# RenYurui/Global-Flow-Local-Attention

Measured on AMD Instinct MI355X. Metric: images/sec (fwd+bwd) PoseGenerator 256x176 attn_layer=2,3 -- feature-warping hot path, higher is better.
Workload: dtype f32 (FC products: 2-term f16 splits exact to 2^-24 on f16 MFMA, f32 accumulate)

## Files before the change

global_flow_local_attention_amd/_lib.py:

```python
import ctypes
import os
import subprocess

import torch

_PKG = os.path.dirname(os.path.abspath(__file__))
LIB_PATH = os.environ.get("GFLA_HIP_LIBRARY") or os.path.join(_PKG, "libgfla_hip.so")
_lib = None

_i64, _int, _ptr = ctypes.c_int64, ctypes.c_int, ctypes.c_void_p

_SIGNATURES = {
    "gfla_block_extractor_fwd": [_ptr] * 3 + [_i64] * 6 + [_int, _ptr],
    "gfla_block_extractor_bwd": [_ptr] * 5 + [_i64] * 6 + [_int, _ptr],
    "gfla_block_extractor_unfold_fwd": [_ptr] * 3 + [_i64] * 6 + [_int, _int, _ptr],
    "gfla_block_extractor_unfold_bwd": [_ptr] * 5 + [_i64] * 6 + [_int, _int, _ptr],
    "gfla_local_attn_reshape_fwd": [_ptr] * 2 + [_i64] * 3 + [_int, _ptr],
    "gfla_local_attn_reshape_bwd": [_ptr] * 2 + [_i64] * 3 + [_int, _ptr],
    "gfla_resample2d_fwd": [_ptr] * 3 + [_i64] * 6 + [_int, _int, _ptr],
    "gfla_resample2d_bwd": [_ptr] * 5 + [_i64] * 6 + [_int, _int, _int, _ptr],
    "gfla_local_attn_aggregate_fwd": [_ptr] * 5 + [_i64] * 6 + [_int, _int, _ptr],
    "gfla_local_attn_aggregate_bwd": [_ptr] * 7 + [_i64] * 6 + [_int, _int, _ptr],
    "gfla_local_attn_source_bwd": [_ptr] * 7 + [_i64] * 6 + [_int, _int, _ptr],
    "gfla_flow_warp_fwd": [_ptr] * 3 + [_i64] * 6 + [ctypes.c_double] * 4 + [_ptr],
    "gfla_flow_warp_bwd": [_ptr] * 5 + [_i64] * 6 + [ctypes.c_double] * 4 + [_ptr],
}
_SINGLE = {
    "gfla_max_cosine_fwd_f32": [_ptr] * 5 + [_i64] * 4 + [ctypes.c_double, _ptr],
    "gfla_max_cosine_fwd_f16": [_ptr] * 5 + [_i64] * 4 + [ctypes.c_double, _ptr],
    "gfla_max_cosine_fwd_bf16": [_ptr] * 5 + [_i64] * 4 + [ctypes.c_double, _ptr],
    "gfla_max_cosine_workspace_bytes": [_i64] * 3,
    "gfla_fc_tail_fwd_f32": [_ptr, _i64, _i64] + [_ptr] * 5 + [_i64] * 3 + [_int, ctypes.c_double, _ptr],
    "gfla_fc_tail_fwd_f64": [_ptr, _i64, _i64] + [_ptr] * 5 + [_i64] * 3 + [_int, ctypes.c_double, _ptr],
    "gfla_fc_tail_bwd_f32": [_ptr, _i64, _i64] + [_ptr] * 8 + [_i64] * 3 + [_int, ctypes.c_double, _ptr],
    "gfla_fc_tail_bwd_f64": [_ptr, _i64, _i64] + [_ptr] * 8 + [_i64] * 3 + [_int, ctypes.c_double, _ptr],
    "gfla_replicate_pad_bwd_f32": [_ptr] * 2 + [_i64] * 3 + [_int] * 4 + [_ptr],
    "gfla_replicate_pad_bwd_f64": [_ptr] * 2 + [_i64] * 3 + [_int] * 4 + [_ptr],
    "gfla_correctness_map_fwd_f32": [_ptr] * 5 + [_i64] * 3 + [ctypes.c_double] * 2 + [_ptr],
    "gfla_correctness_map_bwd_f32": [_ptr] * 9 + [_i64] * 3 + [ctypes.c_double] * 2 + [_ptr],
    "gfla_correctness_map_fwd_f16": [_ptr] * 5 + [_i64] * 3 + [ctypes.c_double] * 2 + [_ptr],
    "gfla_correctness_map_bwd_f16": [_ptr] * 9 + [_i64] * 3 + [ctypes.c_double] * 2 + [_ptr],
    "gfla_correctness_map_fwd_bf16": [_ptr] * 5 + [_i64] * 3 + [ctypes.c_double] * 2 + [_ptr],
    "gfla_correctness_map_bwd_bf16": [_ptr] * 9 + [_i64] * 3 + [ctypes.c_double] * 2 + [_ptr],
    "gfla_fc_supported": [_i64] * 3 + [_int, _int],
    "gfla_fc_workspace_bytes": [_i64] * 4 + [_int] * 3,
    "gfla_fc_forward_f32": [_ptr] * 9 + [_i64] * 4 + [_int, ctypes.c_double, _int, _ptr],
    "gfla_fc_backward_f32": [_ptr] * 12 + [_i64] * 4 + [_int, ctypes.c_double, _int, _int, _ptr],
    "gfla_fc_geometry": [_i64, _i64, _int, _int, _ptr],
    "gfla_fc_conv_fwd_f32": [_ptr, _ptr, _int, _ptr, _ptr] + [_i64] * 4 + [_int, _int, _ptr],
    "gfla_fc_conv_bwd_f32": [_ptr, _int, _ptr, _ptr, _ptr, _ptr] + [_i64] * 4 + [_int, _int, _ptr],
    "gfla_fc_tr_probe": [_ptr, _int, _ptr, _ptr, _ptr],
    "gfla_fc_wino_debug_buffer": [_ptr],
    "gfla_fc_kernel_f32": [_int, _ptr, _ptr] + [_i64] * 4 + [_int, _int, _ptr],
    "gfla_scatter_workspace_bytes": [_i64] * 3 + [_int],
    "gfla_aggregate_fwd_workspace_bytes": [_i64] * 3 + [_int],
    "gfla_aggregate_fwd_geometry": [_i64] * 6 + [_int, _ptr],
    "gfla_aggregate_bwd_supported": [_i64, _i64, _int],
    "gfla_big_plane_geometry": [_int] + [_i64] * 6 + [_int, _int, _ptr],
    "gfla_xcd_swizzle": [_i64, _i64],
    "gfla_local_attn_aggregate_fwd_ws_f32": [_ptr] * 6 + [_i64] * 6 + [_int, _int, _ptr],
    "gfla_local_attn_aggregate_fwd_ws_bf16": [_ptr] * 6 + [_i64] * 6 + [_int, _int, _ptr],
    "gfla_local_attn_aggregate_fwd_ws_f16": [_ptr] * 6 + [_i64] * 6 + [_int, _int, _ptr],
    "gfla_local_attn_aggregate_bwd_ws_f32": [_ptr] * 8 + [_i64] * 6 + [_int, _int, _ptr],
    "gfla_resample2d_bwd_ws_f32": [_ptr] * 6 + [_i64] * 6 + [_int, _int, _int, _ptr],
    "gfla_convert_multi": [_ptr, _ptr, _i64] * 4 + [_int, _ptr],
    "gfla_mask_blend_fwd_f32": [_ptr] * 6 + [_i64] * 3 + [_ptr],
    "gfla_mask_blend_fwd_bf16": [_ptr] * 6 + [_i64] * 3 + [_ptr],
    "gfla_mask_blend_bwd_f32": [_ptr] * 11 + [_i64] * 3 + [_ptr],
    "gfla_mask_blend_bwd_bf16": [_ptr] * 11 + [_i64] * 3 + [_ptr],
    "gfla_mask_blend_fwd_f16": [_ptr] * 6 + [_i64] * 3 + [_ptr],
    "gfla_mask_blend_bwd_f16": [_ptr] * 11 + [_i64] * 3 + [_ptr],
    "gfla_fc_forward_f16": [_ptr] * 9 + [_i64] * 4 + [_int, ctypes.c_double, _ptr],
    "gfla_gemm_f64_workspace_bytes": [_i64] * 3 + [_int],
    "gfla_gemm_f64": [_ptr] * 6 + [_i64] * 3 + [_int, _int, _ptr, _ptr],
    "gfla_affine_reg_workspace_bytes": [_i64] * 3 + [_int],
    "gfla_affine_reg_fwd_f32": [_ptr] * 3 + [_i64] * 3 + [_int, _ptr],
    "gfla_affine_reg_fwd_f64": [_ptr] * 3 + [_i64] * 3 + [_int, _ptr],
    "gfla_affine_reg_fwd_f16": [_ptr] * 3 + [_i64] * 3 + [_int, _ptr],
    "gfla_affine_reg_fwd_bf16": [_ptr] * 3 + [_i64] * 3 + [_int, _ptr],
    "gfla_affine_reg_bwd_f32": [_ptr] * 4 + [_i64] * 3 + [_int, _ptr],
    "gfla_affine_reg_bwd_f64": [_ptr] * 4 + [_i64] * 3 + [_int, _ptr],
    "gfla_affine_reg_bwd_f16": [_ptr] * 4 + [_i64] * 3 + [_int, _ptr],
    "gfla_affine_reg_bwd_bf16": [_ptr] * 4 + [_i64] * 3 + [_int, _ptr],
    "gfla_gram_l1_workspace_bytes": [_i64] * 3,
    "gfla_gram_l1_fwd_f32": [_ptr] * 5 + [_i64] * 3 + [_ptr],
    "gfla_gram_l1_fwd_f16": [_ptr] * 5 + [_i64] * 3 + [_ptr],
    "gfla_gram_l1_fwd_bf16": [_ptr] * 5 + [_i64] * 3 + [_ptr],
    "gfla_gram_l1_bwd_f32": [_ptr] * 4 + [_i64] * 3 + [_int, _ptr],
    "gfla_gram_l1_bwd_f16": [_ptr] * 4 + [_i64] * 3 + [_int, _ptr],
    "gfla_gram_l1_bwd_bf16": [_ptr] * 4 + [_i64] * 3 + [_int, _ptr],
}
_FWD_ONLY_BF16 = set()


def exported_symbols():
    names = ["gfla_abi_version", "gfla_status_string", "gfla_set_tuning", "gfla_path_count", "gfla_unfold_supported"]
    for base in _SIGNATURES:
        for sfx in ("f32", "f64", "bf16", "f16"):
            if sfx == "bf16" and base in _FWD_ONLY_BF16:
                continue
            names.append("%s_%s" % (base, sfx))
    return names + list(_SINGLE)


def build(force=False):
    cmd = ["make", "-C", os.path.join(_PKG, "csrc"), "-j8"]
    if force:
        cmd.append("-B")
    subprocess.check_call(cmd, stdout=subprocess.DEVNULL)
    return LIB_PATH


def lib():
    global _lib
    if _lib is None:
        if not os.path.exists(LIB_PATH):
            raise RuntimeError(
                "libgfla_hip.so is not built (%s). Run `python -c 'import __graft_entry__ as g; g.build()'` "
                "or `make -C global_flow_local_attention_amd/csrc`. There is no fallback path." % LIB_PATH)
        handle = ctypes.CDLL(LIB_PATH)
        handle.gfla_status_string.restype = ctypes.c_char_p
        handle.gfla_status_string.argtypes = [_int]
        handle.gfla_set_tuning.argtypes = [_int, _int]
        handle.gfla_path_count.argtypes = [_int]
        handle.gfla_path_count.restype = _i64
        handle.gfla_unfold_supported.argtypes = [_i64, _i64, _int, _int]
        for base, args in _SIGNATURES.items():
            for sfx in ("f32", "f64", "bf16", "f16"):
                if sfx == "bf16" and base in _FWD_ONLY_BF16:
                    continue
                fn = getattr(handle, "%s_%s" % (base, sfx))
                fn.argtypes = args
                fn.restype = _int
        for name, args in _SINGLE.items():
            fn = getattr(handle, name)
            fn.argtypes = args
            fn.restype = _i64 if (name.endswith("_bytes") or name == "gfla_xcd_swizzle") else _int
        _lib = handle
    return _lib


_SUFFIX = {torch.float32: "f32", torch.float64: "f64", torch.bfloat16: "bf16", torch.float16: "f16"}
HALF_TYPES = (torch.bfloat16, torch.float16)


def suffix(t, what, allow_bf16=True):
    try:
        sfx = _SUFFIX[t.dtype]
    except KeyError:
        raise TypeError("%s: unsupported dtype %s (float32, float64, bfloat16, float16)" % (what, t.dtype))
    if sfx == "bf16" and not allow_bf16:
        raise TypeError("%s: bfloat16 is forward-only in this library (use float32 for training)" % what)
    return sfx


def reduction_like(t):
    return torch.zeros(t.shape, dtype=torch.float32 if t.dtype in HALF_TYPES else t.dtype, device=t.device)


def scatter_workspace(ref_tensor, B, H, W, entries):
    n = lib().gfla_scatter_workspace_bytes(int(B), int(H), int(W), int(entries))
    return torch.empty(max(int(n), 16), dtype=torch.uint8, device=ref_tensor.device)


def aggregate_fwd(source, flow, logits, out, attn, k, apply_softmax):
    b, c, hs, ws = source.shape
    h, w = flow.shape[2], flow.shape[3]
    sfx = suffix(source, "local_attn_aggregate")
    tail = (b, c, hs, ws, h, w, int(k), 1 if apply_softmax else 0)
    if sfx in ("f32", "bf16", "f16"):
        n = lib().gfla_aggregate_fwd_workspace_bytes(int(b), int(h), int(w), int(k))
        scratch = torch.empty(max(int(n), 16), dtype=torch.uint8, device=source.device)
        call("gfla_local_attn_aggregate_fwd_ws_" + sfx, source, ptr(source), ptr(flow), ptr(logits), ptr(out), ptr(attn),
             ptr(scratch), *tail)
    else:
        call("gfla_local_attn_aggregate_fwd_" + sfx, source, ptr(source), ptr(flow), ptr(logits), ptr(out), ptr(attn), *tail)


def require_gpu(*tensors):
    for t in tensors:
        if t is not None and not t.is_cuda:
            raise NotImplementedError("GFLA ops run on the GPU only (got a %s tensor); there is no CPU path"
                                      % t.device.type)


def ptr(t):
    return None if t is None else ctypes.c_void_p(t.data_ptr())


class Unsupported(RuntimeError):
    """GFLA_ERR_UNSUPPORTED (-3): the arguments are valid but outside what this entry point's kernels take (nothing was
    launched).  Callers that have another way to the same result catch exactly this."""


def call(name, ref_tensor, *args):
    fn = getattr(lib(), name)
    with torch.cuda.device(ref_tensor.device):
        stream = ctypes.c_void_p(torch.cuda.current_stream(ref_tensor.device).cuda_stream)
        status = fn(*args, stream)
    if status != 0:
        err = Unsupported if status == -3 else RuntimeError
        raise err("%s failed: %s (status %d)" % (name, lib().gfla_status_string(status).decode(), status))


_CONVERT_FLAG = {(torch.bfloat16, torch.float32): 0, (torch.float32, torch.bfloat16): 1,
                 (torch.float16, torch.float32): 2, (torch.float32, torch.float16): 3}


def convert_many(tensors, dtype):
    out = list(tensors)
    todo = [i for i, t in enumerate(out) if t is not None and t.dtype != dtype]
    pair_ok = all(out[i].is_cuda and (out[i].dtype, dtype) in _CONVERT_FLAG for i in todo)
    if not todo or not pair_ok or len({out[i].dtype for i in todo}) != 1:
        return [None if t is None else t.to(dtype) for t in out]
    flag = _CONVERT_FLAG[(out[todo[0]].dtype, dtype)]
    for at in range(0, len(todo), 4):
        grp = todo[at:at + 4]
        srcs = [out[i].contiguous() for i in grp]
        dsts = [torch.empty(t.shape, dtype=dtype, device=t.device) for t in srcs]
        args = []
        for j in range(4):
            args += [ptr(srcs[j]), ptr(dsts[j]), srcs[j].numel()] if j < len(grp) else [None, None, 0]
        call("gfla_convert_multi", srcs[0], *args, flag)
        for i, d in zip(grp, dsts):
            out[i] = d
    return out


def unfold_supported(Hs, Ws, k, elem_size):
    return bool(lib().gfla_unfold_supported(int(Hs), int(Ws), int(k), int(elem_size)))


def set_tuning(key, value):
    return lib().gfla_set_tuning(int(key), int(value))


ABI_VERSION = 8
PATH_BE_BWD_LDS, PATH_BE_BWD_GLOBAL, PATH_FC_FWD_MODE0, PATH_FC_BWD_MODE0, PATH_BE_FWD_PIX = 0, 1, 2, 7, 12
PATH_BE_FWD_GPIX, PATH_BE_BWD_TILE, PATH_RS_FWD_BIG, PATH_RS_BWD1_TILE, PATH_RS_BWD2_BIG = 13, 14, 15, 16, 17
PATH_FC_FWD_MODE5, PATH_FC_BWD_MODE5 = 18, 19
PATH_GEMM_F64 = 20
PATH_FC_PACK_F16, PATH_COUNT = 21, 22


def fc_path(mode, backward=False):
    if int(mode) == 5:
        return PATH_FC_BWD_MODE5 if backward else PATH_FC_FWD_MODE5
    return (PATH_FC_BWD_MODE0 if backward else PATH_FC_FWD_MODE0) + int(mode)


def path_count(path):
    return int(lib().gfla_path_count(int(path)))
```

global_flow_local_attention_amd/csrc/fc_block.hip:

```cpp
#include "fc_gemm.h"

namespace gfla {

static int64_t align256(int64_t v) { return (v + 255) & ~(int64_t)255; }

enum { kAmaxSrc = 0, kAmaxTgt = 1, kAmaxW = 2, kAmaxZs = 3, kAmaxZt = 4, kAmaxSlots = 8 };

enum FcConv {
  kConvDirect,
  kConvDirect16,
  kConvWino32,
  kConvWino16,
};
enum FcWgrad {
  kWgradDirect32,
  kWgradDirect16,
  kWgradWino32,
  kWgradWino16,
};
static bool fc_wgrad_wino(FcWgrad w) { return w == kWgradWino32 || w == kWgradWino16; }

struct FcPlan {
  int split;
  bool scaled;
  FcConv fwd, dgrad;
  bool pack_wf, pack_wd;
  int pack_split;
  bool pack_uf, pack_ud;
  bool dgrads_together;
  FcWgrad wgrad;
  FcWgrad wgrad_both;
  bool wgrads_together;
  bool wgrad_x32;
  bool own_scatter;
};

static FcPlan fc_plan(int64_t B, int C, int H, int W, int k, int mode) {
  (void)C;
  FcPlan P;
  P.split = fc_base_mode(mode);
  P.scaled = P.split != 0 || mode == 5;
  P.fwd = mode == 4 ? kConvWino32 : mode == 5 ? (k == 5 ? kConvDirect16 : kConvWino16) : kConvDirect;
  P.dgrad = mode == 4 ? kConvWino32 : mode == 5 ? kConvDirect16 : kConvDirect;
  P.pack_wf = P.fwd == kConvDirect || P.fwd == kConvDirect16;
  P.pack_wd = P.dgrad == kConvDirect || P.dgrad == kConvDirect16;
  P.pack_split = P.dgrad == kConvDirect16 ? 2 : P.split;
  P.pack_uf = P.fwd == kConvWino32 || P.fwd == kConvWino16;
  P.pack_ud = P.dgrad == kConvWino32;
  P.dgrads_together = fc_is_wino(mode);
  P.wgrad_x32 = mode == 1 && k == 5;
  P.wgrad = fc_is_wino(mode) || P.wgrad_x32 ? (mode == 5 && k == 5 ? kWgradWino16 : kWgradWino32)
                                            : (P.split ? kWgradDirect16 : kWgradDirect32);
  P.wgrad_both = P.wgrad_x32 ? kWgradWino16 : P.wgrad;
  P.wgrads_together = tuning(21) != 2;
  const FcHalf hs = fc_half(H, W, k, true);
  P.own_scatter = tuning(46) != 1 && fc_scatter_own_rows(B, hs.Ho, hs.Wo) >= 1;
  return P;
}

struct FcLayout {
  FcPlan plan;
  FcHalf hs, ht;
  int nch_c, cpad, nt_d, KK, dw1_tiles;
  int64_t amax, xs, xt, gs, hid, wd_t, wd_s, gt, wf_t, wf_s, wu_ft, wu_fs, wu_dt, wu_ds, fwd_total;
  int64_t dzs, dzt, dw_s, dw_t, zero_bytes, zs_pk, zt_pk, dxs, dxt, b0p, dw1p, red, red_tmp, dwp, dwp2, x32, x32b, bwd_total;
};

static FcLayout fc_layout(int64_t B, int C, int H, int W, int k, int mode) {
  const bool wino = fc_is_wino(mode);
  FcLayout L;
  L.plan = fc_plan(B, C, H, W, k, mode);
  const FcPlan &P = L.plan;
  L.hs = fc_half(H, W, k, true);
  L.ht = fc_half(H, W, k, false);
  L.nch_c = (int)ceil_div(C, kFcChunk);
  L.cpad = L.nch_c * kFcChunk;
  L.nt_d = (int)ceil_div(C, kFcTN);
  L.KK = k * k;
  const int nch_h = kFcHidden / kFcChunk;
  int64_t o = 0;
  auto take = [&](int64_t bytes) {
    const int64_t at = o;
    o += align256(bytes);
    return at;
  };
  L.amax = take(kAmaxSlots * 4);
  L.xs = take(fc_packed_bytes(B, L.nch_c, L.hs.Sx, P.split));
  L.xt = take(fc_packed_bytes(B, L.nch_c, L.ht.Sx, P.split));
  L.gs = take(B * L.hs.Mg * kFcHidden * 4);
  L.hid = take(B * (int64_t)H * W * kFcHidden * 4);
  L.wd_t = take(P.pack_wd ? fc_wpack_bytes(L.nt_d, nch_h, k, P.pack_split) : 0);
  L.wd_s = take(P.pack_wd ? fc_wpack_bytes(L.nt_d, nch_h, k, P.pack_split) : 0);
  L.gt = take(B * L.ht.Mg * kFcHidden * 4);
  L.wf_t = take(P.pack_wd ? fc_wpack_bytes(1, L.nch_c, k, P.pack_split) : 0);
  L.wf_s = take(P.pack_wd ? fc_wpack_bytes(1, L.nch_c, k, P.pack_split) : 0);
  L.wu_ft = take(wino ? fc_wino_wpack_bytes(C, kFcHidden) : 0);
  L.wu_fs = take(wino ? fc_wino_wpack_bytes(C, kFcHidden) : 0);
  L.wu_dt = take(wino ? fc_wino_wpack_bytes(kFcHidden, C) : 0);
  L.wu_ds = take(wino ? fc_wino_wpack_bytes(kFcHidden, C) : 0);
  L.fwd_total = o;

  o = 0;
  L.dzs = take(B * L.hs.Sz * kFcHidden * 4);
  L.dzt = take(B * L.ht.Sz * kFcHidden * 4);
  L.dw_s = take((int64_t)L.KK * L.cpad * kFcHidden * 4);
  L.dw_t = take((int64_t)L.KK * L.cpad * kFcHidden * 4);
  L.zero_bytes = o;
  L.zs_pk = take(P.split ? fc_packed_bytes(B, nch_h, L.hs.Sz, P.split) : 0);
  L.zt_pk = take(P.split ? fc_packed_bytes(B, nch_h, L.ht.Sz, P.split) : 0);
  L.dxs = take(B * L.hs.Mdg * (int64_t)C * 4);
  L.dxt = take(B * L.ht.Mdg * (int64_t)C * 4);
  const int64_t tiles = ceil_div((int64_t)H * W, 64);
  L.b0p = take(B * tiles * kFcHidden * 4);
  int t = 1;
  while (B * t < 2 * kNumCU && t * 128 < H * W) t *= 2;
  L.dw1_tiles = t;
  L.dw1p = take(B * t * (32 * kFcHidden + 32) * 4);
  L.red = take((32 * kFcHidden + 32 + kFcHidden) * 4);
  L.red_tmp = take((int64_t)kFcRedTmpFloats * 4);
  const int64_t sp_s = fc_wgrad_splits(B, L.hs.M, L.cpad), sp_t = fc_wgrad_splits(B, L.ht.M, L.cpad);
  int64_t dwp = P.split == 0 ? (sp_s > sp_t ? sp_s : sp_t) * L.KK * L.cpad * kFcHidden * 4 : 0;
  if (fc_wgrad_wino(P.wgrad)) {
    const int64_t ws_s = fc_wino_wgrad_splits(B, L.hs.Ho, L.hs.Wo, L.cpad, k), ws_t = fc_wino_wgrad_splits(B, L.ht.Ho, L.ht.Wo, L.cpad, k);
    const int64_t w = (ws_s > ws_t ? ws_s : ws_t) * 36 * L.cpad * kFcHidden * 4;
    if (w > dwp) dwp = w;
  }
  L.dwp = take(dwp);
  L.dwp2 = take(dwp);
  const int64_t x32_s = fc_packed_bytes(B, L.nch_c, L.hs.Sx, 0), x32_t = fc_packed_bytes(B, L.nch_c, L.ht.Sx, 0);
  L.x32 = take(P.wgrad_x32 ? (x32_s > x32_t ? x32_s : x32_t) : 0);
  L.x32b = take(P.wgrad_x32 ? x32_t : 0);
  L.bwd_total = o;
  return L;
}

static int fc_args_ok(int64_t B, int64_t C, int64_t H, int64_t W, int k, int mode) {
  if (B < 0 || C <= 0 || H <= 0 || W <= 0 || k < 1) return GFLA_ERR_BAD_SHAPE;
  if (!fc_mode_ok(mode) || (k != 3 && k != 5)) return GFLA_ERR_UNSUPPORTED;
  if (B > 65535 || C > 4096 || H > 2048 || W > 2048) return GFLA_ERR_UNSUPPORTED;
  const FcHalf hs = fc_half((int)H, (int)W, k, true), ht = fc_half((int)H, (int)W, k, false);
  const int direct = mode == 5 ? 2 : mode;
  if (mode == 4) {
    if (!fc_wino_fits(hs.Mv, hs.Wo, hs.Wp, k) || !fc_wino_fits(hs.Md, hs.Wp, hs.Wp, k) ||
        !fc_wino_fits(ht.Mv, ht.Wo, ht.Wp, k) || !fc_wino_fits(ht.Md, ht.Wp, ht.Wp, k))
      return GFLA_ERR_UNSUPPORTED;
  } else if (mode == 5) {
    if (!fc_wino16_fits(hs.Mv, hs.Wo, hs.Wp, k) || !fc_wino16_fits(hs.Md, hs.Wp, hs.Wp, k) ||
        !fc_wino16_fits(ht.Mv, ht.Wo, ht.Wp, k) || !fc_wino16_fits(ht.Md, ht.Wp, ht.Wp, k))
      return GFLA_ERR_UNSUPPORTED;
  }
  if (mode != 4 && (!fc_conv_fits(hs.Wo, hs.Wp, k, direct) || !fc_conv_fits(hs.Wp, hs.Wp, k, direct) ||
                    !fc_conv_fits(ht.Wo, ht.Wp, k, direct) || !fc_conv_fits(ht.Wp, ht.Wp, k, direct)))
    return GFLA_ERR_UNSUPPORTED;
  if ((int64_t)64 * (W + 1) * 4 > 64 * 1024) return GFLA_ERR_UNSUPPORTED;
  return GFLA_OK;
}

#define GFLA_TRY(expr)           \
  do {                           \
    const int rc_ = (expr);      \
    if (rc_ != GFLA_OK) return rc_; \
  } while (0)

static int fc_pack_weight_sets(const FcLayout &L, const float *w0, unsigned char *ws, int C, int k, hipStream_t stream) {
  const FcPlan &P = L.plan;
  const uint32_t *a_w = reinterpret_cast<const uint32_t *>(ws + L.amax) + kAmaxW;
  if (P.pack_wf || P.pack_wd)
    GFLA_TRY(fc_pack_weights(w0, P.pack_split ? a_w : nullptr, P.pack_wf ? ws + L.wf_t : nullptr, P.pack_wf ? ws + L.wf_s : nullptr,
                             P.pack_wd ? ws + L.wd_t : nullptr, P.pack_wd ? ws + L.wd_s : nullptr, C, k, P.pack_split, stream));
  float *u_ft = reinterpret_cast<float *>(ws + L.wu_ft), *u_fs = reinterpret_cast<float *>(ws + L.wu_fs);
  if (P.fwd == kConvWino16) return fc_wino16_pack_weights(w0, a_w, u_ft, u_fs, C, k, stream);
  if (P.pack_uf || P.pack_ud)
    return fc_wino_pack_weights(w0, P.pack_uf ? u_ft : nullptr, P.pack_uf ? u_fs : nullptr,
                                P.pack_ud ? reinterpret_cast<float *>(ws + L.wu_dt) : nullptr,
                                P.pack_ud ? reinterpret_cast<float *>(ws + L.wu_ds) : nullptr, C, k, stream);
  return GFLA_OK;
}

static int fc_wino_jobs(const WnConvJob *jobs, int njobs, const uint32_t *const *amax, const uint32_t *amax_w, bool w16, int64_t B,
                        int nch, int k, hipStream_t stream) {
  if (!w16) return fc_wino_conv_jobs(jobs, njobs, B, nch, k, stream);
  Wn16ConvJob j16[2];
  for (int j = 0; j < njobs && j < 2; ++j)
    j16[j] = Wn16ConvJob{jobs[j].X, reinterpret_cast<const uint32_t *>(jobs[j].U), amax[j], jobs[j].out, jobs[j].out_bs, jobs[j].ldo,
                         jobs[j].n_valid, jobs[j].M, jobs[j].Wv, jobs[j].Wp, jobs[j].S};
  return fc_wino16_conv_jobs(j16, njobs, B, nch, k, amax_w, stream);
}

static int fc_fwd_convs(const FcLayout &L, const unsigned char *ws, float *out_s, float *out_t, int64_t B, int k,
                        hipStream_t stream) {
  const FcPlan &P = L.plan;
  const uint32_t *amax = reinterpret_cast<const uint32_t *>(ws + L.amax);
  WnConvJob jobs[2];
  const uint32_t *am[2];
  int n = 0;
  for (int h = 0; h < 2; ++h) {
    const bool src = h == 0;
    float *out = src ? out_s : out_t;
    if (!out) continue;
    const FcHalf &g = src ? L.hs : L.ht;
    const PackedDesc X = fc_desc_packed(ws + (src ? L.xs : L.xt), B, L.nch_c, g.Sx, P.split);
    const uint32_t *a_x = amax + (src ? kAmaxSrc : kAmaxTgt);
    const unsigned char *wf = ws + (src ? L.wf_s : L.wf_t);
    if (P.fwd == kConvDirect16) {
      GFLA_TRY(fc_conv_f32src(X, wf, fc_wpack_bytes(1, L.nch_c, k, 2) / 2, out, g.Mg * kFcHidden, kFcHidden, kFcHidden, B, L.nch_c,
                              g.Mv, g.Wo, g.Wp, k, a_x, amax + kAmaxW, stream));
    } else if (P.fwd == kConvDirect) {
      GFLA_TRY(fc_conv(X, wf, fc_wpack_bytes(1, L.nch_c, k, P.split) / fc_nsplit(P.split), out, g.Mg * kFcHidden, kFcHidden,
                       kFcHidden, B, L.nch_c, g.Mv, g.Wo, g.Wp, k, P.split, P.split ? a_x : nullptr,
                       P.split ? amax + kAmaxW : nullptr, stream));
    } else {
      jobs[n] = WnConvJob{X, reinterpret_cast<const float *>(ws + (src ? L.wu_fs : L.wu_ft)), out, g.Mg * kFcHidden, kFcHidden,
                          kFcHidden, g.Mv, g.Wo, g.Wp, g.Sx};
      am[n++] = a_x;
    }
  }
  return n ? fc_wino_jobs(jobs, n, am, amax + kAmaxW, P.fwd == kConvWino16, B, L.nch_c, k, stream) : GFLA_OK;
}

static int fc_dgrad_convs(const FcLayout &L, const unsigned char *ws, unsigned char *sc, bool want_s, bool want_t, int64_t B, int C,
                          int k, hipStream_t stream) {
  const FcPlan &P = L.plan;
  const uint32_t *amax = reinterpret_cast<const uint32_t *>(ws + L.amax);
  const int nch_h = kFcHidden / kFcChunk;
  WnConvJob jobs[2];
  int n = 0;
  for (int h = 0; h < 2; ++h) {
    const bool src = h == 0;
    if (!(src ? want_s : want_t)) continue;
    const FcHalf &g = src ? L.hs : L.ht;
    const float *dz = reinterpret_cast<const float *>(sc + (src ? L.dzs : L.dzt));
    float *dx = reinterpret_cast<float *>(sc + (src ? L.dxs : L.dxt));
    const uint32_t *a_z = amax + (src ? kAmaxZs : kAmaxZt);
    const unsigned char *wd = ws + (src ? L.wd_s : L.wd_t);
    if (P.dgrad == kConvDirect16) {
      GFLA_TRY(fc_conv_f32src(fc_desc_nhwc(dz, g.Sz, kFcHidden), wd, fc_wpack_bytes(L.nt_d, nch_h, k, 2) / 2, dx, g.Mdg * (int64_t)C,
                              C, C, B, nch_h, g.Md, g.Wp, g.Wp, k, a_z, amax + kAmaxW, stream));
    } else if (P.dgrad == kConvDirect) {
      const PackedDesc Z = P.split ? fc_desc_packed(sc + (src ? L.zs_pk : L.zt_pk), B, nch_h, g.Sz, P.split)
                                   : fc_desc_nhwc(dz, g.Sz, kFcHidden);
      GFLA_TRY(fc_conv(Z, wd, fc_wpack_bytes(L.nt_d, nch_h, k, P.split) / fc_nsplit(P.split), dx, g.Mdg * (int64_t)C, C, C, B,
                       nch_h, g.Md, g.Wp, g.Wp, k, P.split, P.split ? a_z : nullptr, P.split ? amax + kAmaxW : nullptr, stream));
    } else {
      jobs[n++] = WnConvJob{fc_desc_nhwc(dz, g.Sz, kFcHidden), reinterpret_cast<const float *>(ws + (src ? L.wu_ds : L.wu_dt)), dx,
                            g.Mdg * (int64_t)C, C, C, g.Md, g.Wp, g.Wp, g.Sz};
    }
  }
  return n ? fc_wino_conv_jobs(jobs, n, B, nch_h, k, stream) : GFLA_OK;
}

static PackedDesc fc_wgrad_x(const FcLayout &L, const unsigned char *ws, const unsigned char *sc, bool src, int64_t B) {
  const FcHalf &g = src ? L.hs : L.ht;
  if (L.plan.wgrad_x32) return fc_desc_packed(sc + (src ? L.x32 : L.x32b), B, L.nch_c, g.Sx, 0);
  return fc_desc_packed(ws + (src ? L.xs : L.xt), B, L.nch_c, g.Sx, L.plan.split);
}

static int fc_wgrad_half(const FcLayout &L, bool src, const unsigned char *ws, unsigned char *sc, int64_t B, int k,
                         hipStream_t stream) {
  const FcPlan &P = L.plan;
  const FcHalf &g = src ? L.hs : L.ht;
  const uint32_t *amax = reinterpret_cast<const uint32_t *>(ws + L.amax);
  const PackedDesc X = fc_wgrad_x(L, ws, sc, src, B);
  const float *dz = reinterpret_cast<const float *>(sc + (src ? L.dzs : L.dzt));
  float *part = reinterpret_cast<float *>(sc + (src ? L.dwp : L.dwp2));
  switch (P.wgrad) {
    case kWgradWino16: {
      const WwJob job{X, dz, part, g.Sz * kFcHidden, g.lead, g.Sx, g.Ho, g.Wo, g.Wp};
      const uint32_t *const ax[1] = {amax + (src ? kAmaxSrc : kAmaxTgt)}, *const az[1] = {amax + (src ? kAmaxZs : kAmaxZt)};
      return fc_wino16_wgrad_jobs(&job, 1, L.cpad, B, k, ax, az, stream);
    }
    case kWgradWino32:
      return fc_wino_wgrad(X, dz, g.Sz * kFcHidden, g.lead, part, L.cpad, B, g.Ho, g.Wo, g.Wp, g.Sx, k, stream);
    case kWgradDirect32:
      return fc_wgrad_f32(X, fc_desc_nhwc(dz, g.Sz, kFcHidden), g.lead, part, L.cpad, B, g.M, g.Wp, k, stream);
    default:
      return fc_wgrad(X, fc_desc_packed(sc + (src ? L.zs_pk : L.zt_pk), B, kFcHidden / kFcChunk, g.Sz, P.split), g.lead,
                      reinterpret_cast<float *>(sc + (src ? L.dw_s : L.dw_t)), L.cpad, B, g.M, g.Wp, k, P.split, stream);
  }
}

static int fc_wgrad_both(const FcLayout &L, const unsigned char *ws, unsigned char *sc, int64_t B, int k, hipStream_t stream) {
  const uint32_t *amax = reinterpret_cast<const uint32_t *>(ws + L.amax);
  const WwJob jobs[2] = {
      {fc_wgrad_x(L, ws, sc, true, B), reinterpret_cast<const float *>(sc + L.dzs), reinterpret_cast<float *>(sc + L.dwp),
       L.hs.Sz * kFcHidden, L.hs.lead, L.hs.Sx, L.hs.Ho, L.hs.Wo, L.hs.Wp},
      {fc_wgrad_x(L, ws, sc, false, B), reinterpret_cast<const float *>(sc + L.dzt), reinterpret_cast<float *>(sc + L.dwp2),
       L.ht.Sz * kFcHidden, L.ht.lead, L.ht.Sx, L.ht.Ho, L.ht.Wo, L.ht.Wp}};
  if (L.plan.wgrad_both == kWgradWino16) {
    const uint32_t *const ax[2] = {amax + kAmaxSrc, amax + kAmaxTgt}, *const az[2] = {amax + kAmaxZs, amax + kAmaxZt};
    return fc_wino16_wgrad_jobs(jobs, 2, L.cpad, B, k, ax, az, stream);
  }
  return fc_wino_wgrad_jobs(jobs, 2, L.cpad, B, k, stream);
}

static int fc_forward(const float *source, const float *target, const float *flow, const float *w0, const float *b0,
                      const float *w1, const float *b1, void *ws_, float *logits, int64_t B, int C, int H, int W,
                      int k, float slope, int mode_, hipStream_t stream, const uint16_t *source16 = nullptr,
                      const uint16_t *target16 = nullptr) {
  const bool f16 = source16 != nullptr;
  if (f16 ? !target16 : (!source || !target)) return GFLA_ERR_NULL_POINTER;
  if (!flow || !w0 || !w1 || !ws_ || !logits) return GFLA_ERR_NULL_POINTER;
  if (f16 && mode_ != 1) return GFLA_ERR_UNSUPPORTED;
  GFLA_TRY(fc_args_ok(B, C, H, W, k, mode_));
  if (B == 0) return GFLA_OK;
  note_path(mode_ == 5 ? GFLA_PATH_FC_FWD_MODE5 : GFLA_PATH_FC_FWD_MODE0 + mode_);
  const FcLayout L = fc_layout(B, C, H, W, k, mode_);
  const FcPlan &P = L.plan;
  unsigned char *ws = static_cast<unsigned char *>(ws_);
  uint32_t *amax = reinterpret_cast<uint32_t *>(ws + L.amax);
  if (P.scaled) {
    if (hipMemsetAsync(amax, 0, kAmaxSlots * 4, stream) != hipSuccess) return GFLA_ERR_LAUNCH;
    if (f16)
      GFLA_TRY(fc_maxabs(w0, (int64_t)kFcHidden * 2 * C * k * k, amax + kAmaxW, stream));
    else
      GFLA_TRY(fc_maxabs_multi(source, B * (int64_t)C * H * W, amax + kAmaxSrc, target, B * (int64_t)C * H * W, amax + kAmaxTgt,
                               w0, (int64_t)kFcHidden * 2 * C * k * k, amax + kAmaxW, stream));
  }
  GFLA_TRY(fc_pack_weight_sets(L, w0, ws, C, k, stream));
  if (f16)
    GFLA_TRY(fc_pack_act2_f16(source16, ws + L.xs, L.hs, target16, ws + L.xt, L.ht, B, C, H, W, stream));
  else
    GFLA_TRY(fc_pack_act2(source, P.split ? amax + kAmaxSrc : nullptr, ws + L.xs, L.hs, target, P.split ? amax + kAmaxTgt : nullptr,
                          ws + L.xt, L.ht, B, C, H, W, P.split, stream));
  float *gs = reinterpret_cast<float *>(ws + L.gs), *gt = reinterpret_cast<float *>(ws + L.gt);
  GFLA_TRY(fc_fwd_convs(L, ws, gs, gt, B, k, stream));
  return fc_sample_tail_fwd(gs, gt, flow, b0, w1, b1, reinterpret_cast<float *>(ws + L.hid), logits, B, H, W, k,
                            L.hs.Mg * kFcHidden, L.ht.Mg * kFcHidden, L.hs.Wo, L.ht.Wo, slope, stream);
}

struct FcHalfCall {
  int acc_x = 0;
  bool z_ready = false;
  bool dgrad_done = false;
  bool fold_later = false;
  bool wgrad_later = false;
  bool reduce = true;
};

static int fc_half_backward(const FcLayout &L, bool source, unsigned char *ws, unsigned char *sc, float *g_x, float *g_w0,
                            int64_t B, int C, int H, int W, int k, const FcHalfCall &call, hipStream_t stream) {
  const FcPlan &P = L.plan;
  const FcHalf &g = source ? L.hs : L.ht;
  uint32_t *amax = reinterpret_cast<uint32_t *>(ws + L.amax);
  uint32_t *a_z = amax + (source ? kAmaxZs : kAmaxZt);
  float *dz = reinterpret_cast<float *>(sc + (source ? L.dzs : L.dzt));
  if (P.split && !call.z_ready) {
    GFLA_TRY(fc_maxabs(dz, B * g.Sz * kFcHidden, a_z, stream));
    GFLA_TRY(fc_pack_z(dz, a_z, sc + (source ? L.zs_pk : L.zt_pk), B, g.Sz, kFcHidden, P.split, stream));
  }
  if (g_x && !call.dgrad_done) {
    if (P.dgrad == kConvDirect16) GFLA_TRY(fc_maxabs(dz, B * g.Sz * kFcHidden, a_z, stream));
    GFLA_TRY(fc_dgrad_convs(L, ws, sc, source, !source, B, C, k, stream));
    if (!call.fold_later)
      GFLA_TRY(fc_fold(reinterpret_cast<const float *>(sc + (source ? L.dxs : L.dxt)), g_x, B, C, H, W, g, g.Mdg * (int64_t)C,
                       call.acc_x, stream));
  }
  if (!g_w0) return GFLA_OK;
  if (P.wgrad_x32)
    GFLA_TRY(fc_unpack_act(ws + (source ? L.xs : L.xt), amax + (source ? kAmaxSrc : kAmaxTgt),
                           reinterpret_cast<float *>(sc + (source ? L.x32 : L.x32b)), B, L.nch_c, g.Sx, stream));
  if (!call.wgrad_later) {
    if (P.wgrad == kWgradWino16) GFLA_TRY(fc_maxabs(dz, B * g.Sz * kFcHidden, a_z, stream));
    GFLA_TRY(fc_wgrad_half(L, source, ws, sc, B, k, stream));
  }
  if (!call.reduce) return GFLA_OK;
  float *part = reinterpret_cast<float *>(sc + (source ? L.dwp : L.dwp2));
  if (fc_wgrad_wino(P.wgrad))
    return fc_wino_wgrad_reduce(part, fc_wino_wgrad_splits(B, g.Ho, g.Wo, L.cpad, k), g_w0, C, source ? C : 0, L.cpad, k, stream);
  if (P.wgrad == kWgradDirect32)
    return fc_wgrad_reduce(part, fc_wgrad_splits(B, g.M, L.cpad), g_w0, C, source ? C : 0, L.cpad, k, stream);
  return GFLA_OK;
}

static int fc_fold_both(const FcLayout &L, const unsigned char *sc, float *g_source, float *g_target, int acc_s, int64_t B, int C,
                        int H, int W, hipStream_t stream) {
  return fc_fold2(reinterpret_cast<const float *>(sc + L.dxs), g_source, L.hs, L.hs.Mdg * (int64_t)C, acc_s,
                  reinterpret_cast<const float *>(sc + L.dxt), g_target, L.ht, L.ht.Mdg * (int64_t)C, 0, B, C, H, W, stream);
}

static int fc_unpack_wgrad_both(const FcLayout &L, const unsigned char *ws, unsigned char *sc, float *g_w0, int C, int k,
                                hipStream_t stream) {
  const uint32_t *a = reinterpret_cast<const uint32_t *>(ws + L.amax);
  return fc_unpack_wgrad(reinterpret_cast<float *>(sc + L.dw_t), reinterpret_cast<float *>(sc + L.dw_s), a + kAmaxTgt, a + kAmaxSrc,
                         a + kAmaxZt, a + kAmaxZs, g_w0, C, L.cpad, k, stream);
}

static int fc_backward(void *ws_, const float *flow, const float *w1, const float *g_logits, void *scratch_,
                       float *g_source, float *g_target, float *g_flow, float *g_w0, float *g_b0, float *g_w1,
                       float *g_b1, int64_t B, int C, int H, int W, int k, float slope, int mode_, int flags,
                       hipStream_t stream) {
  if (!ws_ || !flow || !w1 || !g_logits || !scratch_) return GFLA_ERR_NULL_POINTER;
  GFLA_TRY(fc_args_ok(B, C, H, W, k, mode_));
  if (B == 0) return GFLA_OK;
  note_path(mode_ == 5 ? GFLA_PATH_FC_BWD_MODE5 : GFLA_PATH_FC_BWD_MODE0 + mode_);
  const FcLayout L = fc_layout(B, C, H, W, k, mode_);
  const FcPlan &P = L.plan;
  unsigned char *ws = static_cast<unsigned char *>(ws_), *sc = static_cast<unsigned char *>(scratch_);
  uint32_t *amax = reinterpret_cast<uint32_t *>(ws + L.amax);
  const float *hid = reinterpret_cast<const float *>(ws + L.hid);
  float *red_tmp = reinterpret_cast<float *>(sc + L.red_tmp);
  const float *gs = reinterpret_cast<const float *>(ws + L.gs);
  const bool need_s = g_source || g_w0, need_t = g_target || g_w0;
  float *dzs = need_s ? reinterpret_cast<float *>(sc + L.dzs) : nullptr;
  float *dzt = need_t ? reinterpret_cast<float *>(sc + L.dzt) : nullptr;
  float *b0p = g_b0 ? reinterpret_cast<float *>(sc + L.b0p) : nullptr;
  const int64_t tiles = ceil_div((int64_t)H * W, 64);
  const bool own = need_s && need_t && P.own_scatter;
  if (hipMemsetAsync(sc + (own ? L.dzt : 0), 0, L.zero_bytes - (own ? L.dzt : 0), stream) != hipSuccess) return GFLA_ERR_LAUNCH;
  if ((P.scaled || own) && hipMemsetAsync(amax + kAmaxZs, 0, 8, stream) != hipSuccess) return GFLA_ERR_LAUNCH;
  GFLA_TRY(fc_sample_tail_bwd(gs, flow, hid, w1, g_logits, own ? nullptr : dzs, dzt, g_flow, b0p, B, H, W, k, L.hs.Mg * kFcHidden,
                              L.hs.Wo, L.hs.Wp, L.ht.Wp, L.hs.Sz * kFcHidden, L.ht.Sz * kFcHidden, L.hs.lead, L.ht.lead, slope,
                              flags & GFLA_FC_ACCUMULATE_FLOW, stream, own ? amax + kAmaxZt : nullptr));
  if (own)
    GFLA_TRY(fc_sample_scatter_own(flow, dzt, dzs, amax + kAmaxZt, amax + kAmaxZs, B, H, W, k, L.hs.Ho, L.hs.Wo, L.hs.Wp, L.ht.Wp,
                                   L.hs.Sz * kFcHidden, L.ht.Sz * kFcHidden, L.hs.lead, L.ht.lead, L.hs.Sz, stream));
  const float *dw1p = nullptr;
  if (g_w1 || g_b1) {
    float *part = reinterpret_cast<float *>(sc + L.dw1p);
    GFLA_TRY(fc_dw1(hid, g_logits, part, B, H * W, L.KK, L.dw1_tiles, slope, stream));
    dw1p = part;
  }
  GFLA_TRY(fc_reduce_bias_w1(b0p, B * tiles, g_b0, dw1p, B * L.dw1_tiles, g_w1, g_b1, L.KK, red_tmp, stream));
  const int acc_s = (flags & GFLA_FC_ACCUMULATE_SOURCE) ? 1 : 0;
  const bool both_x = g_source && g_target;
  const bool dgrads_done = P.dgrads_together && both_x;
  if (dgrads_done) {
    if (P.dgrad == kConvDirect16 && !own)
      GFLA_TRY(fc_maxabs_multi(dzs, B * L.hs.Sz * kFcHidden, amax + kAmaxZs, dzt, B * L.ht.Sz * kFcHidden, amax + kAmaxZt, nullptr,
                               0, nullptr, stream));
    GFLA_TRY(fc_dgrad_convs(L, ws, sc, true, true, B, C, k, stream));
    GFLA_TRY(fc_fold_both(L, sc, g_source, g_target, acc_s, B, C, H, W, stream));
  }
  const bool defer = g_w0 && P.wgrad != kWgradDirect16;
  const bool wgrads_done = defer && fc_wgrad_wino(P.wgrad) && both_x && P.wgrads_together;
  const bool z_both = P.split != 0 && need_s && need_t;
  if (z_both) {
    if (!own)
      GFLA_TRY(fc_maxabs_multi(dzs, B * L.hs.Sz * kFcHidden, amax + kAmaxZs, dzt, B * L.ht.Sz * kFcHidden, amax + kAmaxZt, nullptr,
                               0, nullptr, stream));
    GFLA_TRY(fc_pack_z2(dzs, amax + kAmaxZs, sc + L.zs_pk, L.hs.Sz, dzt, amax + kAmaxZt, sc + L.zt_pk, L.ht.Sz, B, kFcHidden,
                        P.split, stream));
  }
  FcHalfCall call;
  call.z_ready = z_both;
  call.dgrad_done = dgrads_done;
  call.fold_later = both_x;
  call.wgrad_later = wgrads_done;
  call.reduce = !defer;
  if (need_s) {
    call.acc_x = acc_s;
    GFLA_TRY(fc_half_backward(L, true, ws, sc, g_source, g_w0, B, C, H, W, k, call, stream));
  }
  if (need_t) {
    call.acc_x = 0;
    GFLA_TRY(fc_half_backward(L, false, ws, sc, g_target, g_w0, B, C, H, W, k, call, stream));
  }
  if (both_x && !dgrads_done) GFLA_TRY(fc_fold_both(L, sc, g_source, g_target, acc_s, B, C, H, W, stream));
  if (wgrads_done) GFLA_TRY(fc_wgrad_both(L, ws, sc, B, k, stream));
  if (defer) {
    float *part_s = reinterpret_cast<float *>(sc + L.dwp), *part_t = reinterpret_cast<float *>(sc + L.dwp2);
    if (fc_wgrad_wino(P.wgrad))
      GFLA_TRY(fc_wino_wgrad_reduce2(part_s, fc_wino_wgrad_splits(B, L.hs.Ho, L.hs.Wo, L.cpad, k), part_t,
                                     fc_wino_wgrad_splits(B, L.ht.Ho, L.ht.Wo, L.cpad, k), g_w0, C, L.cpad, k, stream));
    else
      GFLA_TRY(fc_wgrad_reduce2(part_s, fc_wgrad_splits(B, L.hs.M, L.cpad), part_t, fc_wgrad_splits(B, L.ht.M, L.cpad), g_w0, C,
                                L.cpad, k, stream));
  }
  if (g_w0 && P.wgrad == kWgradDirect16) GFLA_TRY(fc_unpack_wgrad_both(L, ws, sc, g_w0, C, k, stream));
  return GFLA_OK;
}

}

extern "C" {
using namespace gfla;

int gfla_fc_supported(int64_t C, int64_t H, int64_t W, int kernel_size, int mode) {
  return fc_args_ok(1, C, H, W, kernel_size, mode) == GFLA_OK ? 1 : 0;
}

int64_t gfla_fc_workspace_bytes(int64_t B, int64_t C, int64_t H, int64_t W, int kernel_size, int mode, int which) {
  if (fc_args_ok(B, C, H, W, kernel_size, mode) != GFLA_OK) return -1;
  const FcLayout L = fc_layout(B, (int)C, (int)H, (int)W, kernel_size, mode);
  return which == 0 ? L.fwd_total : L.bwd_total;
}

int gfla_fc_forward_f32(const float *source, const float *target, const float *flow, const float *w0,
                        const float *b0, const float *w1, const float *b1, void *workspace, float *logits, int64_t B,
                        int64_t C, int64_t H, int64_t W, int kernel_size, double slope, int mode,
                        gfla_stream_t stream) {
  return fc_forward(source, target, flow, w0, b0, w1, b1, workspace, logits, B, (int)C, (int)H, (int)W, kernel_size,
                    (float)slope, mode, static_cast<hipStream_t>(stream));
}

int gfla_fc_forward_f16(const uint16_t *source, const uint16_t *target, const float *flow, const float *w0,
                        const float *b0, const float *w1, const float *b1, void *workspace, float *logits, int64_t B,
                        int64_t C, int64_t H, int64_t W, int kernel_size, double slope, gfla_stream_t stream) {
  return fc_forward(nullptr, nullptr, flow, w0, b0, w1, b1, workspace, logits, B, (int)C, (int)H, (int)W, kernel_size,
                    (float)slope, 1, static_cast<hipStream_t>(stream), source, target);
}

int gfla_fc_backward_f32(void *workspace, const float *flow, const float *w1, const float *grad_logits,
                         void *scratch, float *grad_source, float *grad_target, float *grad_flow, float *grad_w0,
                         float *grad_b0, float *grad_w1, float *grad_b1, int64_t B, int64_t C, int64_t H, int64_t W,
                         int kernel_size, double slope, int mode, int flags, gfla_stream_t stream) {
  return fc_backward(workspace, flow, w1, grad_logits, scratch, grad_source, grad_target, grad_flow, grad_w0, grad_b0,
                     grad_w1, grad_b1, B, (int)C, (int)H, (int)W, kernel_size, (float)slope, mode, flags,
                     static_cast<hipStream_t>(stream));
}


int gfla_fc_geometry(int64_t H, int64_t W, int kernel_size, int is_source, int64_t *out) {
  if (!out) return GFLA_ERR_NULL_POINTER;
  if (H <= 0 || W <= 0 || kernel_size < 1) return GFLA_ERR_BAD_SHAPE;
  const FcHalf g = fc_half((int)H, (int)W, kernel_size, is_source != 0);
  const int64_t v[13] = {g.Hp, g.Wp, g.Ho, g.Wo, g.pad_t, g.pad_l, g.M, g.Md, g.lead, g.Sx, g.Sz, g.Mg, g.Mdg};
  for (int i = 0; i < 13; ++i) out[i] = v[i];
  return GFLA_OK;
}

int gfla_fc_conv_fwd_f32(const float *x, const float *w0, int is_source, void *workspace, float *out, int64_t B,
                         int64_t C_, int64_t H_, int64_t W_, int kernel_size, int mode, gfla_stream_t stream_) {
  if (!x || !w0 || !workspace || !out) return GFLA_ERR_NULL_POINTER;
  const int C = (int)C_, H = (int)H_, W = (int)W_, k = kernel_size;
  GFLA_TRY(fc_args_ok(B, C, H, W, k, mode));
  if (B == 0) return GFLA_OK;
  hipStream_t stream = static_cast<hipStream_t>(stream_);
  const FcLayout L = fc_layout(B, C, H, W, k, mode);
  const FcPlan &P = L.plan;
  const FcHalf &g = is_source ? L.hs : L.ht;
  unsigned char *ws = static_cast<unsigned char *>(workspace);
  uint32_t *amax = reinterpret_cast<uint32_t *>(ws + L.amax);
  uint32_t *a_x = amax + (is_source ? kAmaxSrc : kAmaxTgt);
  if (hipMemsetAsync(amax, 0, kAmaxSlots * 4, stream) != hipSuccess) return GFLA_ERR_LAUNCH;
  if (P.scaled) {
    GFLA_TRY(fc_maxabs(x, B * (int64_t)C * H * W, a_x, stream));
    GFLA_TRY(fc_maxabs(w0, (int64_t)kFcHidden * 2 * C * k * k, amax + kAmaxW, stream));
  }
  GFLA_TRY(fc_pack_act(x, P.split ? a_x : nullptr, ws + (is_source ? L.xs : L.xt), B, C, H, W, g, P.split, stream));
  GFLA_TRY(fc_pack_weight_sets(L, w0, ws, C, k, stream));
  return fc_fwd_convs(L, ws, is_source ? out : nullptr, is_source ? nullptr : out, B, k, stream);
}

int gfla_fc_conv_bwd_f32(const float *z, int is_source, void *workspace, void *scratch, float *grad_x, float *grad_w0,
                         int64_t B, int64_t C_, int64_t H_, int64_t W_, int kernel_size, int mode,
                         gfla_stream_t stream_) {
  if (!z || !workspace || !scratch) return GFLA_ERR_NULL_POINTER;
  const int C = (int)C_, H = (int)H_, W = (int)W_, k = kernel_size;
  GFLA_TRY(fc_args_ok(B, C, H, W, k, mode));
  if (B == 0) return GFLA_OK;
  hipStream_t stream = static_cast<hipStream_t>(stream_);
  const FcLayout L = fc_layout(B, C, H, W, k, mode);
  const FcHalf &g = is_source ? L.hs : L.ht;
  unsigned char *ws = static_cast<unsigned char *>(workspace), *sc = static_cast<unsigned char *>(scratch);
  uint32_t *amax = reinterpret_cast<uint32_t *>(ws + L.amax);
  if (hipMemsetAsync(sc, 0, L.zero_bytes, stream) != hipSuccess) return GFLA_ERR_LAUNCH;
  if (hipMemsetAsync(amax + kAmaxZs, 0, 8, stream) != hipSuccess) return GFLA_ERR_LAUNCH;
  if (hipMemcpyAsync(sc + (is_source ? L.dzs : L.dzt), z, (size_t)(B * g.Sz * kFcHidden * 4), hipMemcpyDeviceToDevice,
                     stream) != hipSuccess)
    return GFLA_ERR_LAUNCH;
  const bool unpack = L.plan.wgrad == kWgradDirect16;
  if (grad_w0 && !unpack &&
      hipMemsetAsync(grad_w0, 0, (size_t)kFcHidden * 2 * C * k * k * 4, stream) != hipSuccess)
    return GFLA_ERR_LAUNCH;
  GFLA_TRY(fc_half_backward(L, is_source != 0, ws, sc, grad_x, grad_w0, B, C, H, W, k, FcHalfCall(), stream));
  if (grad_w0 && unpack) GFLA_TRY(fc_unpack_wgrad_both(L, ws, sc, grad_w0, C, k, stream));
  return GFLA_OK;
}

int gfla_fc_kernel_f32(int which, void *workspace, void *scratch, int64_t B, int64_t C_, int64_t H_, int64_t W_,
                       int kernel_size, int mode, gfla_stream_t stream_) {
  if (!workspace || !scratch) return GFLA_ERR_NULL_POINTER;
  if (which < 0 || which > 8 || (which > 5 && !fc_is_wino(mode))) return GFLA_ERR_BAD_SHAPE;
  const int C = (int)C_, H = (int)H_, W = (int)W_, k = kernel_size;
  GFLA_TRY(fc_args_ok(B, C, H, W, k, mode));
  if (B == 0) return GFLA_OK;
  hipStream_t stream = static_cast<hipStream_t>(stream_);
  const FcLayout L = fc_layout(B, C, H, W, k, mode);
  unsigned char *ws = static_cast<unsigned char *>(workspace), *sc = static_cast<unsigned char *>(scratch);
  const bool src = which == 6 || which == 7 || (which & 1) == 0, tgt = which > 5 || (which & 1) == 1;
  float *gs = reinterpret_cast<float *>(ws + L.gs), *gt = reinterpret_cast<float *>(ws + L.gt);
  switch (which) {
    case 0: case 1: case 6: return fc_fwd_convs(L, ws, src ? gs : nullptr, tgt ? gt : nullptr, B, k, stream);
    case 2: case 3: case 7: return fc_dgrad_convs(L, ws, sc, src, tgt, B, C, k, stream);
    case 4: case 5: return fc_wgrad_half(L, src, ws, sc, B, k, stream);
    default: return fc_wgrad_wino(L.plan.wgrad_both) ? fc_wgrad_both(L, ws, sc, B, k, stream) : GFLA_ERR_UNSUPPORTED;
  }
}

int gfla_fc_tr_probe(const int16_t *image, int n_halves, const int32_t *offsets, int16_t *out, gfla_stream_t stream) {
  if (!image || !offsets || !out) return GFLA_ERR_NULL_POINTER;
  return fc_tr_probe(image, n_halves, offsets, out, static_cast<hipStream_t>(stream));
}
}
```

global_flow_local_attention_amd/csrc/fc_conv.hip:

```cpp
#include "fc_conv_impl.h"

namespace gfla {

bool fc_conv_fits(int Wv, int Wp, int k, int mode) {
  return (int64_t)fc_nsplit(mode) * fc_conv_tile_pixels(kFcMinRowBlocks, Wv, Wp, k) * (mode ? 48 : 80) <= 156 * 1024;
}

int fc_conv(const PackedDesc &X, const void *wk, int64_t w_split_stride, float *out, int64_t out_bs, int ldo,
            int n_valid, int64_t B, int nch, int M, int Wv, int Wp, int k, int mode, const uint32_t *amax_x,
            const uint32_t *amax_w, hipStream_t stream) {
  if (!fc_mode_ok(mode) || (k != 3 && k != 5)) return GFLA_ERR_UNSUPPORTED;
  if (B > 65535 || B <= 0 || M <= 0) return B == 0 ? GFLA_OK : GFLA_ERR_UNSUPPORTED;
  if (Wv <= 0 || Wv > Wp || !fc_conv_fits(Wv, Wp, k, mode)) return GFLA_ERR_UNSUPPORTED;
  if (mode == 0)
    return fc_conv_mode<0>(X, wk, w_split_stride, out, out_bs, ldo, n_valid, B, nch, M, Wv, Wp, k, amax_x, amax_w, stream);
  if (mode == 1)
    return fc_conv_mode<1>(X, wk, w_split_stride, out, out_bs, ldo, n_valid, B, nch, M, Wv, Wp, k, amax_x, amax_w, stream);
  if (mode == 2)
    return fc_conv_mode<2>(X, wk, w_split_stride, out, out_bs, ldo, n_valid, B, nch, M, Wv, Wp, k, amax_x, amax_w, stream);
  return fc_conv_mode<3>(X, wk, w_split_stride, out, out_bs, ldo, n_valid, B, nch, M, Wv, Wp, k, amax_x, amax_w, stream);
}

}
```

global_flow_local_attention_amd/csrc/fc_conv_impl.h:

```cpp
#pragma once

#include "fc_mma.h"

namespace gfla {

constexpr int kFcMinRowBlocks = 2, kFcMaxRowBlocks = 8;
constexpr int kFcPrefetch = 8;

template <int MODE>
__device__ __forceinline__ void load_b_frags(Frag<MODE> (&fb)[Fc<MODE>::KB], const unsigned char *p, int64_t split_stride) {
  if constexpr (MODE == 0) {
    fb[0].v = *reinterpret_cast<const float4 *>(p);
    fb[1].v = *reinterpret_cast<const float4 *>(p + 32);
  } else {
#pragma unroll
    for (int sp = 0; sp < Fc<MODE>::NS; ++sp) fb[0].s[sp] = *reinterpret_cast<const f16x8 *>(p + sp * split_stride);
  }
}

typedef unsigned int u32x4 __attribute__((ext_vector_type(4)));

__device__ __forceinline__ void fc_prefetch_pieces(u32x4 (&pf)[kFcPrefetch], const unsigned char *src, int x_ps, int pix0,
                                                   int tmh) {
#pragma unroll
  for (int q = 0; q < kFcPrefetch; ++q)
    pf[q] = *reinterpret_cast<const u32x4 *>(src + (int64_t)min(pix0 + 64 * q, tmh - 1) * x_ps);
}

struct ConvTiling {
  int T, base, rem, heavy, per_ntile;
};

template <int MODE, int KS, int NMB, bool SRC32 = false>
__global__ __launch_bounds__(256, 2) void fc_conv_kernel(PackedDesc X, const unsigned char *__restrict__ Wk,
                                                        int64_t w_split_stride, float *__restrict__ out,
                                                        int64_t out_bs, int ldo, int n_valid, int M, int Wv, int Wp,
                                                        int nch, int tmh, ConvTiling tl,
                                                        const uint32_t *__restrict__ amax_x,
                                                        const uint32_t *__restrict__ amax_w) {
  using F = Fc<MODE>;
  constexpr int KK = KS * KS, PITCH = F::PITCH, STEPS = F::KB * NMB;
  extern __shared__ __attribute__((aligned(16))) unsigned char gfla_smem[];
  unsigned char *xs = gfla_smem;
  const int t = threadIdx.x, lane = t & 63, wave = t >> 6, l31 = lane & 31, kh = lane >> 5;
  int wid = blockIdx.x;
  const int ntile = wid / tl.per_ntile;
  wid -= ntile * tl.per_ntile;
  if (tl.per_ntile <= 2 * kNumCU && wid >= kNumCU) wid = tl.per_ntile - 1 - (wid - kNumCU);
  else if (tl.per_ntile <= kNumCU && (ntile & 1)) wid = tl.per_ntile - 1 - wid;
  int64_t b;
  int first, nblk;
  if (wid < tl.heavy) {
    b = wid / tl.rem;
    first = (wid - (int)b * tl.rem) * (tl.base + 1);
    nblk = tl.base + 1;
  } else {
    const int u = wid - tl.heavy, per = tl.T - tl.rem;
    b = u / per;
    first = tl.rem * (tl.base + 1) + (u - (int)b * per) * tl.base;
    nblk = tl.base;
  }
  const int m0 = first * 32;
  const int y0 = m0 / Wv, p0 = y0 * Wp + (m0 - y0 * Wv);
  const int64_t x_ss = X.split_stride, x_cs = X.chunk_stride;
  const int x_ps = X.pix_stride;
  const unsigned char *xg = X.base + b * X.batch_stride + (int64_t)p0 * x_ps;
  constexpr int64_t kWTile = (int64_t)kFcTN * F::REC;
  const unsigned char *wg = Wk + (int64_t)ntile * nch * KK * kWTile + (wave * 32 + l31) * F::REC + kh * 16;

  int a_off[NMB];
#pragma unroll
  for (int mb = 0; mb < NMB; ++mb) {
    const int r = min(m0 + mb * 32 + l31, M - 1);
    const int y = r / Wv;
    a_off[mb] = (y * Wp + (r - y * Wv) - p0) * PITCH;
  }

  f32x16 acc[NMB];
#pragma unroll
  for (int mb = 0; mb < NMB; ++mb)
#pragma unroll
    for (int r = 0; r < 16; ++r) acc[mb][r] = 0.f;

  static_assert(!SRC32 || MODE == 2, "float32 source: mode 2 arithmetic only");
  const int per = tmh * (SRC32 ? 4 : F::PIECES);
  const int x_total = SRC32 ? per : per * F::NS;
  const int xplane = tmh * PITCH;

  constexpr int PF = kFcPrefetch;
  constexpr bool kPrefetch = MODE == 0 || SRC32;
  const float sx32 = SRC32 ? fc_scale(amax_x) : 1.f;
  auto store_split = [&](unsigned char *dst8, u32x4 v) {
    uint32_t h01, l01, h23, l23;
    fc_split_pair(__uint_as_float(v[0]) * sx32, __uint_as_float(v[1]) * sx32, h01, l01);
    fc_split_pair(__uint_as_float(v[2]) * sx32, __uint_as_float(v[3]) * sx32, h23, l23);
    *reinterpret_cast<uint2 *>(dst8) = make_uint2(h01, h23);
    *reinterpret_cast<uint2 *>(dst8 + xplane) = make_uint2(l01, l23);
  };
  u32x4 pf[PF];
  const int pix0 = t >> 2;
  const unsigned char *pf_src = xg + (t & 3) * 16;
  unsigned char *pf_dst = xs + (size_t)pix0 * PITCH + (t & 3) * (SRC32 ? 8 : 16);
  const int x_first = kPrefetch ? min(x_total, 256 * PF) : 0;

  Frag<MODE> cur[F::KB], nxt[F::KB];
  load_b_frags<MODE>(cur, wg, w_split_stride);
  if constexpr (kPrefetch) fc_prefetch_pieces(pf, pf_src, x_ps, pix0, tmh);
  for (int cc = 0; cc < nch; ++cc) {
    __syncthreads();
    if constexpr (kPrefetch) {
#pragma unroll
      for (int q = 0; q < PF; ++q)
        if (pix0 + 64 * q < tmh) {
          if constexpr (SRC32) store_split(pf_dst + (size_t)q * 64 * PITCH, pf[q]);
          else *reinterpret_cast<u32x4 *>(pf_dst + (size_t)q * 64 * PITCH) = pf[q];
        }
    }
    if constexpr (SRC32) {
      const unsigned char *src = xg + (int64_t)cc * x_cs + (t & 3) * 16;
      for (int pix = pix0 + 64 * PF; pix < tmh; pix += 64)
        store_split(xs + (size_t)pix * PITCH + (t & 3) * 8, *reinterpret_cast<const u32x4 *>(src + (int64_t)pix * x_ps));
    } else if (x_first < x_total) {
      const unsigned char *src = xg + (int64_t)cc * x_cs;
      for (int base = x_first + t; base < x_total; base += 256 * 4) {
        uint4 v0 = make_uint4(0, 0, 0, 0), v1 = v0, v2 = v0, v3 = v0;
#define GFLA_X_SP(idx_) (((idx_) >= per) + ((idx_) >= 2 * per))
#define GFLA_X_REM(idx_) ((idx_)-GFLA_X_SP(idx_) * per)
#define GFLA_X_SRC(idx_) \
  (src + GFLA_X_SP(idx_) * x_ss + (int64_t)(GFLA_X_REM(idx_) / F::PIECES) * x_ps + (GFLA_X_REM(idx_) % F::PIECES) * 16)
#define GFLA_X_DST(idx_) \
  (xs + ((size_t)GFLA_X_SP(idx_) * tmh + GFLA_X_REM(idx_) / F::PIECES) * PITCH + (GFLA_X_REM(idx_) % F::PIECES) * 16)
        if (base < x_total) v0 = *reinterpret_cast<const uint4 *>(GFLA_X_SRC(base));
        if (base + 256 < x_total) v1 = *reinterpret_cast<const uint4 *>(GFLA_X_SRC(base + 256));
        if (base + 512 < x_total) v2 = *reinterpret_cast<const uint4 *>(GFLA_X_SRC(base + 512));
        if (base + 768 < x_total) v3 = *reinterpret_cast<const uint4 *>(GFLA_X_SRC(base + 768));
        if (base < x_total) *reinterpret_cast<uint4 *>(GFLA_X_DST(base)) = v0;
        if (base + 256 < x_total) *reinterpret_cast<uint4 *>(GFLA_X_DST(base + 256)) = v1;
        if (base + 512 < x_total) *reinterpret_cast<uint4 *>(GFLA_X_DST(base + 512)) = v2;
        if (base + 768 < x_total) *reinterpret_cast<uint4 *>(GFLA_X_DST(base + 768)) = v3;
#undef GFLA_X_SRC
#undef GFLA_X_DST
#undef GFLA_X_SP
#undef GFLA_X_REM
      }
    }
    __syncthreads();
    Frag<MODE> fa = load_frag<MODE>(xs + a_off[0], xplane, 0, kh);
#pragma unroll 1
    for (int tap = 0; tap < KK; ++tap) {
      {
        const int lin = cc * KK + tap + 1;
#pragma unroll
        for (int q = 0; q < F::KB; ++q) nxt[q] = cur[q];
        if (lin < nch * KK) load_b_frags<MODE>(nxt, wg + (int64_t)lin * kWTile, w_split_stride);
        if constexpr (kPrefetch)
          if (tap == 0 && cc + 1 < nch)
            fc_prefetch_pieces(pf, pf_src + (int64_t)(cc + 1) * x_cs, x_ps, pix0, tmh);
      }
      const int i = tap / KS, j = tap - i * KS;
      const unsigned char *xa = xs + (size_t)(i * Wp + j) * PITCH;
      const int tn = tap + 1 < KK ? tap + 1 : 0;
      const int in = tn / KS, jn = tn - in * KS;
      const unsigned char *xa_next = xs + (size_t)(in * Wp + jn) * PITCH;
#pragma unroll
      for (int st = 0; st < STEPS; ++st) {
        const int kb = st / NMB, mb = st % NMB;
        const Frag<MODE> fc = fa;
        if (st + 1 < STEPS)
          fa = load_frag<MODE>(xa + a_off[(st + 1) % NMB], xplane, (st + 1) / NMB, kh);
        else
          fa = load_frag<MODE>(xa_next + a_off[0], xplane, 0, kh);
        __builtin_amdgcn_sched_barrier(0);
        if (mb + 1 < NMB || nblk == NMB)
          acc[mb] = mma<MODE>(fc, cur[kb], acc[mb]);
      }
#pragma unroll
      for (int q = 0; q < F::KB; ++q) cur[q] = nxt[q];
    }
  }

  const float inv = MODE == 0 ? 1.f : fc_inv_scale(amax_x) * fc_inv_scale(amax_w);
  float *ob = out + b * out_bs;
  const int col = ntile * kFcTN + wave * 32 + l31;
  if (col < n_valid) {
#pragma unroll
    for (int mb = 0; mb < NMB; ++mb) {
      if (mb >= nblk) continue;
#pragma unroll
      for (int r = 0; r < 16; ++r) {
        const int m = m0 + mb * 32 + (r & 3) + 8 * (r >> 2) + 4 * kh;
        if (m < M) ob[(int64_t)m * ldo + col] = acc[mb][r] * inv;
      }
    }
  }
}



inline int fc_conv_tile_pixels(int mb, int Wv, int Wp, int k) {
  const int tm = 32 * mb;
  return tm + ((tm - 1) / Wv + 1) * (Wp - Wv) + (k - 1) * (Wp + 1);
}

inline int pick_conv_tiling(int M, int64_t B, int ntiles_n, int Wv, int Wp, int k, int mode, ConvTiling *tl) {
  const int ns = fc_nsplit(mode), pitch = mode ? 48 : 80;
  const int nb = (int)ceil_div(M, 32);
  const int forced = tuning(11);
  int64_t T = (2 * kNumCU) / (B * ntiles_n);
  if (T < 1) T = 1;
  if (T > nb) T = nb;
  if (ceil_div(nb, T) > kFcMaxRowBlocks) T = ceil_div(nb, kFcMaxRowBlocks);
  if (forced >= kFcMinRowBlocks && forced <= kFcMaxRowBlocks) T = ceil_div(nb, forced);
  for (;; ++T) {
    const int nmb = (int)ceil_div(nb, T);
    const int64_t lds = (int64_t)ns * fc_conv_tile_pixels(nmb < kFcMinRowBlocks ? kFcMinRowBlocks : nmb, Wv, Wp, k) * pitch;
    if (lds <= 156 * 1024) break;
    if (nmb <= kFcMinRowBlocks) return 0;
  }
  tl->T = (int)T;
  tl->base = nb / (int)T;
  tl->rem = nb % (int)T;
  tl->heavy = (int)B * tl->rem;
  tl->per_ntile = (int)(B * T);
  int nmb = tl->base + (tl->rem ? 1 : 0);
  if (nmb < kFcMinRowBlocks) {
    nmb = kFcMinRowBlocks;
  }
  return nmb;
}

template <int MODE, int KS, int NMB, bool SRC32 = false>
static int launch_conv(const PackedDesc &X, const void *wk, int64_t w_split_stride, float *out, int64_t out_bs,
                       int ldo, int n_valid, int64_t B, int nch, int M, int Wv, int Wp, const ConvTiling &tl,
                       const uint32_t *amax_x, const uint32_t *amax_w, hipStream_t stream) {
  using F = Fc<MODE>;
  const int tmh = fc_conv_tile_pixels(NMB, Wv, Wp, KS);
  const unsigned lds = (unsigned)(F::NS * tmh * F::PITCH);
  const int64_t wgs = (int64_t)tl.per_ntile * ceil_div(n_valid, kFcTN);
  if (wgs > 0x7fffffffLL) return GFLA_ERR_UNSUPPORTED;
  auto kern = fc_conv_kernel<MODE, KS, NMB, SRC32>;
  if (lds > 64 * 1024)
    (void)hipFuncSetAttribute(reinterpret_cast<const void *>(kern), hipFuncAttributeMaxDynamicSharedMemorySize, (int)lds);
  kern<<<dim3((unsigned)wgs), 256, lds, stream>>>(X, static_cast<const unsigned char *>(wk), w_split_stride, out, out_bs,
                                                  ldo, n_valid, M, Wv, Wp, nch, tmh, tl, amax_x, amax_w);
  return launch_status();
}

template <int MODE, int KS, bool SRC32 = false>
static int dispatch_conv(int nmb, const PackedDesc &X, const void *wk, int64_t wss, float *out, int64_t out_bs, int ldo,
                         int n_valid, int64_t B, int nch, int M, int Wv, int Wp, const ConvTiling &tl, const uint32_t *ax,
                         const uint32_t *aw, hipStream_t s) {
  switch (nmb) {
#define GFLA_CASE(N_) \
  case N_: return launch_conv<MODE, KS, N_, SRC32>(X, wk, wss, out, out_bs, ldo, n_valid, B, nch, M, Wv, Wp, tl, ax, aw, s)
    GFLA_CASE(2);
    GFLA_CASE(3);
    GFLA_CASE(4);
    GFLA_CASE(5);
    GFLA_CASE(6);
    GFLA_CASE(7);
    GFLA_CASE(8);
#undef GFLA_CASE
  }
  return GFLA_ERR_UNSUPPORTED;
}

template <int MODE>
int fc_conv_mode(const PackedDesc &X, const void *wk, int64_t w_split_stride, float *out, int64_t out_bs, int ldo,
                 int n_valid, int64_t B, int nch, int M, int Wv, int Wp, int k, const uint32_t *amax_x,
                 const uint32_t *amax_w, hipStream_t stream);

#define GFLA_DEFINE_FC_CONV_MODE(MODE_)                                                                               \
  template <>                                                                                                         \
  int fc_conv_mode<MODE_>(const PackedDesc &X, const void *wk, int64_t w_split_stride, float *out, int64_t out_bs,    \
                          int ldo, int n_valid, int64_t B, int nch, int M, int Wv, int Wp, int k,                     \
                          const uint32_t *amax_x, const uint32_t *amax_w, hipStream_t stream) {                       \
    ConvTiling tl;                                                                                                    \
    const int nmb = pick_conv_tiling(M, B, (int)ceil_div(n_valid, kFcTN), Wv, Wp, k, MODE_, &tl);                      \
    if (nmb == 0) return GFLA_ERR_UNSUPPORTED;                                                                        \
    if (k == 3)                                                                                                       \
      return dispatch_conv<MODE_, 3>(nmb, X, wk, w_split_stride, out, out_bs, ldo, n_valid, B, nch, M, Wv, Wp, tl,     \
                                     amax_x, amax_w, stream);                                                         \
    return dispatch_conv<MODE_, 5>(nmb, X, wk, w_split_stride, out, out_bs, ldo, n_valid, B, nch, M, Wv, Wp, tl,       \
                                   amax_x, amax_w, stream);                                                           \
  }

}
```

global_flow_local_attention_amd/csrc/fc_conv_m2.hip:

```cpp
#include "fc_conv_impl.h"

namespace gfla {
GFLA_DEFINE_FC_CONV_MODE(2)

int fc_conv_f32src(const PackedDesc &X32, const void *wk, int64_t w_split_stride, float *out, int64_t out_bs, int ldo,
                   int n_valid, int64_t B, int nch, int M, int Wv, int Wp, int k, const uint32_t *amax_x,
                   const uint32_t *amax_w, hipStream_t stream) {
  if ((k != 3 && k != 5) || !amax_x || !amax_w || X32.pix_stride < 64) return GFLA_ERR_UNSUPPORTED;
  if (B > 65535 || B <= 0 || M <= 0) return B == 0 ? GFLA_OK : GFLA_ERR_UNSUPPORTED;
  if (Wv <= 0 || Wv > Wp || !fc_conv_fits(Wv, Wp, k, 2)) return GFLA_ERR_UNSUPPORTED;
  ConvTiling tl;
  const int nmb = pick_conv_tiling(M, B, (int)ceil_div(n_valid, kFcTN), Wv, Wp, k, 2, &tl);
  if (nmb == 0) return GFLA_ERR_UNSUPPORTED;
  if (k == 3)
    return dispatch_conv<2, 3, true>(nmb, X32, wk, w_split_stride, out, out_bs, ldo, n_valid, B, nch, M, Wv, Wp, tl, amax_x, amax_w,
                                     stream);
  return dispatch_conv<2, 5, true>(nmb, X32, wk, w_split_stride, out, out_bs, ldo, n_valid, B, nch, M, Wv, Wp, tl, amax_x, amax_w,
                                   stream);
}
}
```

global_flow_local_attention_amd/csrc/fc_gemm.h:

```cpp
#pragma once

#include "gfla_common.h"

namespace gfla {

typedef float f32x16 __attribute__((ext_vector_type(16)));
typedef _Float16 f16x8 __attribute__((ext_vector_type(8)));
typedef short s16x4 __attribute__((ext_vector_type(4)));
typedef short s16x8 __attribute__((ext_vector_type(8)));

constexpr int kFcChunk = 16;
constexpr int kFcTN = 128;
constexpr int kFcHidden = 128;

template <int MODE>
struct Fc;
template <>
struct Fc<0> {
  static constexpr int NS = 1, ESZ = 4, REC = 64, PIECES = 4, PITCH = 80, KB = 2;
};
template <>
struct Fc<1> {
  static constexpr int NS = 1, ESZ = 2, REC = 32, PIECES = 2, PITCH = 48, KB = 1;
};
template <>
struct Fc<2> {
  static constexpr int NS = 2, ESZ = 2, REC = 32, PIECES = 2, PITCH = 48, KB = 1;
};
template <>
struct Fc<3> {
  static constexpr int NS = 3, ESZ = 2, REC = 32, PIECES = 2, PITCH = 48, KB = 1;
};

inline bool fc_is_wino(int mode) { return mode == 4 || mode == 5; }
inline int fc_base_mode(int mode) { return fc_is_wino(mode) ? 0 : mode; }
inline int fc_nsplit(int mode) { return mode == 0 ? 1 : mode; }
inline int fc_esz(int mode) { return mode == 0 ? 4 : 2; }
inline bool fc_mode_ok(int mode) { return mode >= 0 && mode <= 5; }

struct PackedDesc {
  const unsigned char *base;
  int64_t split_stride;
  int64_t batch_stride;
  int64_t chunk_stride;
  int pix_stride;
};

__host__ __device__ __forceinline__ int fc_scale_exp(uint32_t amax_bits) {
  const int eb = (int)((amax_bits >> 23) & 0xffu);
  if (eb == 0 || eb == 255) return 127;
  int se = 268 - eb;
  return se < 2 ? 2 : (se > 252 ? 252 : se);
}
__device__ __forceinline__ float fc_scale(const uint32_t *amax) {
  return amax ? __uint_as_float((uint32_t)fc_scale_exp(*amax) << 23) : 1.f;
}
__device__ __forceinline__ float fc_inv_scale(const uint32_t *amax) {
  return amax ? __uint_as_float((uint32_t)(254 - fc_scale_exp(*amax)) << 23) : 1.f;
}

typedef _Float16 fc_f16x2 __attribute__((ext_vector_type(2)));
typedef float fc_f32x2 __attribute__((ext_vector_type(2)));
__device__ __forceinline__ void fc_split_pair(float v0, float v1, uint32_t &hi, uint32_t &lo) {
  asm("" : "+v"(v0));
  asm("" : "+v"(v1));
  hi = __builtin_bit_cast(uint32_t, __builtin_convertvector(fc_f32x2{v0, v1}, fc_f16x2));
  float r0, r1;
  asm("v_fma_mix_f32 %0, %1, 1.0, -%2 op_sel_hi:[0,0,1]" : "=v"(r0) : "v"(v0), "v"(hi));
  asm("v_fma_mix_f32 %0, %1, 1.0, -%2 op_sel:[0,0,1] op_sel_hi:[0,0,1]" : "=v"(r1) : "v"(v1), "v"(hi));
  lo = __builtin_bit_cast(uint32_t, __builtin_convertvector(fc_f32x2{r0, r1}, fc_f16x2));
}

struct FcHalf {
  int Hp, Wp;
  int Ho, Wo;
  int pad_t, pad_l, pad_b, pad_r;
  int M;
  int Mv;
  int Md;
  int lead;
  int64_t Sx;
  int64_t Sz;
  int64_t Mg;
  int64_t Mdg;
};

inline int64_t round_up(int64_t v, int64_t m) { return (v + m - 1) / m * m; }

inline FcHalf fc_half(int H, int W, int k, bool source) {
  FcHalf g;
  const int lo = k / 2, hi = k - 1 - lo;
  if (source) {
    g.pad_t = g.pad_l = g.pad_b = g.pad_r = k - 1;
  } else {
    g.pad_t = g.pad_l = lo;
    g.pad_b = g.pad_r = hi;
  }
  g.Hp = H + g.pad_t + g.pad_b;
  g.Wp = W + g.pad_l + g.pad_r;
  g.Ho = g.Hp - k + 1;
  g.Wo = g.Wp - k + 1;
  g.M = g.Ho * g.Wp;
  g.Mv = g.Ho * g.Wo;
  g.Md = g.Hp * g.Wp;
  g.lead = (k - 1) * (g.Wp + 1);
  g.Mg = round_up(g.Mv, 16);
  g.Mdg = round_up(g.Md, 16);
  g.Sx = round_up((int64_t)g.Md + 256 + (255 / g.Wo + 1) * (k - 1) + 16, 16);
  const int64_t need_w = g.lead + round_up(g.M, 64) + 64;
  const int64_t need_d = (int64_t)g.Md + 256 + g.lead;
  g.Sz = round_up((need_w > need_d ? need_w : need_d) + 16, 16);
  return g;
}

int fc_maxabs(const float *x, int64_t n, uint32_t *slot, hipStream_t stream);
int fc_maxabs_multi(const float *x0, int64_t n0, uint32_t *slot0, const float *x1, int64_t n1, uint32_t *slot1,
                    const float *x2, int64_t n2, uint32_t *slot2, hipStream_t stream);
int fc_pack_act(const float *src, const uint32_t *amax, void *out, int64_t B, int C, int H, int W, const FcHalf &g,
                int mode, hipStream_t stream);
int fc_pack_act2(const float *src_s, const uint32_t *amax_s, void *out_s, const FcHalf &gs, const float *src_t,
                 const uint32_t *amax_t, void *out_t, const FcHalf &gt, int64_t B, int C, int H, int W, int mode,
                 hipStream_t stream);
int fc_pack_z(const float *z, const uint32_t *amax, void *out, int64_t B, int64_t S, int Cz, int mode,
              hipStream_t stream);
int fc_pack_z2(const float *z_s, const uint32_t *amax_s, void *out_s, int64_t S_s, const float *z_t, const uint32_t *amax_t,
               void *out_t, int64_t S_t, int64_t B, int Cz, int mode, hipStream_t stream);
int fc_pack_act2_f16(const uint16_t *src_s, void *out_s, const FcHalf &gs, const uint16_t *src_t, void *out_t,
                     const FcHalf &gt, int64_t B, int C, int H, int W, hipStream_t stream);
int fc_unpack_act(const void *x16, const uint32_t *amax, float *x32, int64_t B, int nch, int64_t S, hipStream_t stream);
int fc_pack_weights(const float *w0, const uint32_t *amax, void *wf_t, void *wf_s, void *wd_t, void *wd_s, int C,
                    int k, int mode, hipStream_t stream);
int fc_conv(const PackedDesc &X, const void *wk, int64_t w_split_stride, float *out, int64_t out_bs, int ldo,
            int n_valid, int64_t B, int nch, int M, int Wv, int Wp, int k, int mode, const uint32_t *amax_x,
            const uint32_t *amax_w, hipStream_t stream);
int fc_conv_f32src(const PackedDesc &X32, const void *wk, int64_t w_split_stride, float *out, int64_t out_bs, int ldo,
                   int n_valid, int64_t B, int nch, int M, int Wv, int Wp, int k, const uint32_t *amax_x,
                   const uint32_t *amax_w, hipStream_t stream);
bool fc_conv_fits(int Wv, int Wp, int k, int mode);
int fc_wgrad(const PackedDesc &X, const PackedDesc &Y, int64_t y_lead, float *dwacc, int cpad, int64_t B, int Mk,
             int Wp, int k, int mode, hipStream_t stream);
int fc_wgrad_splits(int64_t B, int Mk, int cpad);
int fc_wgrad_f32(const PackedDesc &X, const PackedDesc &Y, int64_t y_lead, float *part, int cpad, int64_t B, int Mk,
                 int Wp, int k, hipStream_t stream);
int fc_wgrad_reduce(const float *part, int nsplit, float *grad_w0, int C, int c_off, int cpad, int k,
                    hipStream_t stream);
int fc_wgrad_reduce2(const float *part_s, int nsplit_s, const float *part_t, int nsplit_t, float *grad_w0, int C, int cpad,
                     int k, hipStream_t stream);
int fc_unpack_wgrad(const float *dw_t, const float *dw_s, const uint32_t *amax_xt, const uint32_t *amax_xs,
                    const uint32_t *amax_zt, const uint32_t *amax_zs, float *grad_w0, int C, int cpad, int k,
                    hipStream_t stream);
PackedDesc fc_desc_packed(const void *base, int64_t B, int nch, int64_t S, int mode);
PackedDesc fc_desc_nhwc(const float *base, int64_t S, int Cz);
int64_t fc_packed_bytes(int64_t B, int nch, int64_t S, int mode);
int64_t fc_wpack_bytes(int ntiles, int nch, int k, int mode);
int fc_tr_probe(const short *image, int n_halves, const int *offsets, short *out, hipStream_t stream);

int64_t fc_wino_wpack_bytes(int n_in, int n_out);
int fc_wino_pack_weights(const float *w0, float *u_ft, float *u_fs, float *u_dt, float *u_ds, int C, int k,
                         hipStream_t stream);
bool fc_wino_fits(int M, int Wv, int Wp, int k);
struct WnConvJob {
  PackedDesc X;
  const float *U;
  float *out;
  int64_t out_bs;
  int ldo, n_valid, M, Wv, Wp;
  int64_t S;
};
int fc_wino_conv_jobs(const WnConvJob *jobs, int njobs, int64_t B, int nch, int k, hipStream_t stream);
int fc_wino_conv(const PackedDesc &X, const float *U, float *out, int64_t out_bs, int ldo, int n_valid, int64_t B, int nch,
                 int M, int Wv, int Wp, int64_t S, int k, hipStream_t stream);
int fc_wino_wgrad_splits(int64_t B, int Ho, int Wo, int cpad, int k);
struct WwJob {
  PackedDesc X;
  const float *Z;
  float *part;
  int64_t z_bs, z_lead, SX;
  int Ho, Wo, Wp;
};
int fc_wino_wgrad_jobs(const WwJob *jobs, int njobs, int cpad, int64_t B, int k, hipStream_t stream);
int fc_wino16_wgrad_jobs(const WwJob *jobs, int njobs, int cpad, int64_t B, int k, const uint32_t *const *amax_x,
                         const uint32_t *const *amax_z, hipStream_t stream);
int fc_wino_wgrad(const PackedDesc &X, const float *Z, int64_t z_bs, int64_t z_lead, float *part, int cpad, int64_t B, int Ho,
                  int Wo, int Wp, int64_t SX, int k, hipStream_t stream);
int fc_wino_wgrad_reduce(float *part, int nsplit, float *grad_w0, int C, int c_off, int cpad, int k, hipStream_t stream);
int fc_wino_wgrad_reduce2(float *part_s, int nsplit_s, float *part_t, int nsplit_t, float *grad_w0, int C, int cpad, int k,
                          hipStream_t stream);

struct Wn16ConvJob {
  PackedDesc X;
  const uint32_t *U;
  const uint32_t *amax_x;
  float *out;
  int64_t out_bs;
  int ldo, n_valid, M, Wv, Wp;
  int64_t S;
};
int fc_wino16_pack_weights(const float *w0, const uint32_t *amax_w, float *u_ft, float *u_fs, int C, int k, hipStream_t stream);
bool fc_wino16_fits(int M, int Wv, int Wp, int k);
int fc_wino16_conv_jobs(const Wn16ConvJob *jobs, int njobs, int64_t B, int nch, int k, const uint32_t *amax_w,
                        hipStream_t stream);

int fc_sample_tail_fwd(const float *gs, const float *gt, const float *flow, const float *b0, const float *w1,
                       const float *b1, float *hid, float *logits, int64_t B, int H, int W, int k, int64_t gs_bs,
                       int64_t gt_bs, int wps, int wpt, float slope, hipStream_t stream);
int fc_sample_tail_bwd(const float *gs, const float *flow, const float *hid, const float *w1, const float *g_logits,
                       float *dzs, float *dzt, float *gflow, float *b0_partials, int64_t B, int H, int W, int k,
                       int64_t gs_bs, int wps, int wpz, int wpt, int64_t zs_bs, int64_t zt_bs, int lead_s, int lead_t,
                       float slope, int acc_flow, hipStream_t stream, uint32_t *amax_d = nullptr);
int fc_scatter_own_rows(int64_t B, int Ho, int Wo);
int fc_sample_scatter_own(const float *flow, const float *dzt, float *dzs, const uint32_t *amax_d, uint32_t *amax_out,
                          int64_t B, int H, int W, int k, int Ho, int Wo, int wpz, int wpt, int64_t zs_bs, int64_t zt_bs,
                          int lead_s, int lead_t, int64_t Sz, hipStream_t stream);
int fc_dw1(const float *hid, const float *g_logits, float *partials, int64_t B, int HW, int KK, int tiles_per_sample,
           float slope, hipStream_t stream);
int fc_fold(const float *dxpad, float *grad, int64_t B, int C, int H, int W, const FcHalf &g, int64_t dx_bs,
            int accumulate, hipStream_t stream);
int fc_fold2(const float *dx_s, float *grad_s, const FcHalf &gs, int64_t dxs_bs, int acc_s, const float *dx_t, float *grad_t,
             const FcHalf &gt, int64_t dxt_bs, int acc_t, int64_t B, int C, int H, int W, hipStream_t stream);
constexpr int kFcRedTmpFloats = 32 * (32 * kFcHidden + 32 + kFcHidden);
int fc_reduce_rows(const float *partials, float *out, int64_t rows, int cols, float scale, float *tmp,
                   hipStream_t stream);
int fc_reduce_bias_w1(const float *b0_partials, int64_t rows_b0, float *g_b0, const float *dw1_partials, int64_t rows_w1,
                      float *g_w1, float *g_b1, int KK, float *tmp, hipStream_t stream);

}
```

global_flow_local_attention_amd/csrc/fc_wino16.hip:

```cpp
#include "fc_wino_shared.h"

namespace gfla {

__global__ __launch_bounds__(256) void fc_wino16_pack_w_kernel(const float *__restrict__ w0, WnPackJobs jobs, int C,
                                                               const uint32_t *__restrict__ amax_w) {
  constexpr int KS = 3;
  const WnPackJob jb = jobs.j[blockIdx.y];
  const int nch = (jb.n_in + kFcChunk - 1) / kFcChunk, ntn = (jb.n_out + kWnN - 1) / kWnN;
  const int64_t idx = (int64_t)blockIdx.x * 256 + threadIdx.x;
  if (!jb.U || idx >= (int64_t)ntn * kWnN * nch * kFcChunk) return;
  const float su = wn16_pow2(wn16_scale_exp(*amax_w, kWn16HeadW));
  const int co = (int)(idx % (ntn * kWnN)), ci = (int)(idx / (ntn * kWnN));
  float w[KS][KS];
#pragma unroll
  for (int i = 0; i < KS; ++i)
#pragma unroll
    for (int j = 0; j < KS; ++j) {
      float v = 0.f;
      if (ci < jb.n_in && co < jb.n_out) v = w0[(((int64_t)co * 2 * C + jb.c_off + ci) * KS + i) * KS + j];
      w[i][j] = v * su;
    }
  float t[6][KS];
#pragma unroll
  for (int j = 0; j < KS; ++j) {
    float col[KS], o[6];
#pragma unroll
    for (int i = 0; i < KS; ++i) col[i] = w[i][j];
    wn_g<KS>(col, o);
#pragma unroll
    for (int a = 0; a < 6; ++a) t[a][j] = o[a];
  }
  const int ntile = co / kWnN, n = co % kWnN;
  const int step = ci >> 3, g = (ci >> 2) & 1, c4 = ci & 3;
  uint32_t *dst = reinterpret_cast<uint32_t *>(jb.U) + ((((int64_t)ntile * 2 * nch + step) * kWnXi * 2 + g) * kWnN + n) * 4 + c4;
#pragma unroll
  for (int a = 0; a < 6; ++a) {
    float o[6];
    wn_g<KS>(t[a], o);
#pragma unroll
    for (int e = 0; e < 6; ++e) dst[(int64_t)(a * 6 + e) * 2 * kWnN * 4] = wn16_split(o[e]);
  }
}

int fc_wino16_pack_weights(const float *w0, const uint32_t *amax_w, float *u_ft, float *u_fs, int C, int k, hipStream_t stream) {
  if (k != 3) return GFLA_ERR_UNSUPPORTED;
  WnPackJobs jobs;
  jobs.j[0] = WnPackJob{u_ft, 0, 0, C, kFcHidden};
  jobs.j[1] = WnPackJob{u_fs, C, 0, C, kFcHidden};
  const dim3 grid((unsigned)ceil_div(ceil_div(kFcHidden, kWnN) * kWnN * ceil_div(C, kFcChunk) * kFcChunk, 256), 2);
  fc_wino16_pack_w_kernel<<<grid, 256, 0, stream>>>(w0, jobs, C, amax_w);
  return launch_status();
}

struct Wn16KArgs {
  PackedDesc X;
  const uint32_t *U;
  const uint32_t *amax_x;
  float *out;
  int64_t out_bs;
  int ldo, n_valid, Ho, Wv, Wp;
  WnGeo geo;
  int ntn;
  int64_t total_groups, S;
};

template <int M>
struct WnAT;
template <>
struct WnAT<2> {
  static constexpr float v[2][6] = {{1.f, 1.f, 1.f, 1.f, 1.f, 0.f}, {0.f, 1.f, -1.f, 2.f, -0.5f, 1.f}};
};
template <>
struct WnAT<4> {
  static constexpr float v[4][6] = {{1.f, 1.f, 1.f, 1.f, 1.f, 0.f},
                                    {0.f, 1.f, -1.f, 2.f, -0.5f, 0.f},
                                    {0.f, 1.f, 1.f, 4.f, 0.25f, 0.f},
                                    {0.f, 1.f, -1.f, 8.f, -0.125f, 1.f}};
};

template <int PG_>
struct PgTag { static constexpr int value = PG_; };

extern unsigned long long *g_wino_stamps;
template <int KS, bool DB = true, int DBG = 0>
__global__ __launch_bounds__(kWnThreads, 2) void fc_wino16_conv_kernel(Wn16KArgs a0, Wn16KArgs a1, unsigned n0, int nch,
                                                                      const uint32_t *__restrict__ amax_w,
                                                                      unsigned long long *stamps) {
  unsigned long long tk0 = 0, t_first = 0, t_second = 0, t_bar = 0, t_pro = 0, t_epi = 0;
  if constexpr (DBG & 16) tk0 = __builtin_amdgcn_s_memtime();
  auto stamp = [&](unsigned long long &slot) {
    if constexpr (DBG & 16) {
      __builtin_amdgcn_s_waitcnt(0);
      const unsigned long long n = __builtin_amdgcn_s_memtime();
      slot += n - tk0;
      tk0 = n;
    }
  };
  constexpr int M = Wn<KS>::M, PITCH = Wn<KS>::PITCH, NP = 9;
  const bool second = blockIdx.x >= n0;
#define GFLA_PICK(f) (second ? a1.f : a0.f)
  PackedDesc X;
  X.base = GFLA_PICK(X.base), X.split_stride = 0, X.batch_stride = GFLA_PICK(X.batch_stride);
  X.chunk_stride = GFLA_PICK(X.chunk_stride), X.pix_stride = GFLA_PICK(X.pix_stride);
  const uint32_t *__restrict__ U = GFLA_PICK(U);
  const uint32_t *__restrict__ amax_x = GFLA_PICK(amax_x);
  float *__restrict__ out = GFLA_PICK(out);
  const int64_t out_bs = GFLA_PICK(out_bs), total_groups = GFLA_PICK(total_groups), S = GFLA_PICK(S);
  const int ldo = GFLA_PICK(ldo), n_valid = GFLA_PICK(n_valid), Ho = GFLA_PICK(Ho), Wv = GFLA_PICK(Wv), Wp = GFLA_PICK(Wp);
  const int ntn = GFLA_PICK(ntn);
  WnGeo geo;
  geo.TH = GFLA_PICK(geo.TH), geo.TW = GFLA_PICK(geo.TW), geo.ngroups = GFLA_PICK(geo.ngroups), geo.span = GFLA_PICK(geo.span);
  geo.tpg = GFLA_PICK(geo.tpg);
#undef GFLA_PICK
  extern __shared__ __attribute__((aligned(16))) unsigned char gfla_smem[];
  uint32_t *vbuf = reinterpret_cast<uint32_t *>(gfla_smem);
  unsigned char *raw = gfla_smem + 2 * kWnVFloats * 4;
  const int raw_bytes = (geo.span * PITCH + 15) & ~15;
  const int t = threadIdx.x, lane = t & 63, wave = t >> 6, nblk = wave & 1, pg = (wave >> 1) & 3, xh = wave >> 2;
  const int g = lane >> 5, l31 = lane & 31;
  const int ex = wn16_scale_exp(*amax_x, kWn16HeadX), ew = wn16_scale_exp(*amax_w, kWn16HeadW);
  const float sx = wn16_pow2(ex), inv_x = wn16_pow2(254 - ex), inv_w = wn16_pow2(254 - ew);
  const int64_t x = blockIdx.x - (second ? n0 : 0u);
  const int xcd = (int)(x & 7);
  const int64_t slot = x >> 3;
  const int ntile = (int)(slot % ntn);
  const int64_t glin = (slot / ntn) * 8 + xcd;
  if (glin >= total_groups) return;
  const int64_t b = glin / geo.ngroups;
  const int grp = (int)(glin - b * geo.ngroups);
  const int ntiles = geo.TH * geo.TW;
  const int tile0 = grp * geo.tpg;
  const int ty_first = tile0 / geo.TW;
  const int p0 = M * ty_first * Wp;
  const int64_t avail = S - p0;

  const int tl = (t & 255) >> 3, c8 = t & 7;
  int toff;
  {
    const int tau = min(tile0 + min(tl, geo.tpg - 1), ntiles - 1);
    const int ty = tau / geo.TW, tx = tau - ty * geo.TW;
    toff = ((M * ty * Wp + M * tx) - p0) * PITCH + c8 * 4;
  }
  const int vpos = xh * 18 * 256 + (c8 >> 2) * 128 + tl * 4 + (c8 & 3);

  const unsigned char *xg = X.base + b * X.batch_stride + (int64_t)p0 * X.pix_stride;

  f32x16 acc[NP];
#pragma unroll
  for (int p = 0; p < NP; ++p)
#pragma unroll
    for (int i = 0; i < 16; ++i) acc[p][i] = 0.f;

  const int npieces = geo.span * 4;
  u32x4w pf[kWnPF];
  auto piece_off = [&](int q) -> unsigned {
    const int pix = q >> 2;
    return (unsigned)min((int64_t)pix, avail - 1) * (unsigned)X.pix_stride + (unsigned)(q & 3) * 16u;
  };
  auto piece_store = [&](int q, u32x4w v, int cc) {
    const int pix = q >> 2;
    float f[4];
#pragma unroll
    for (int e = 0; e < 4; ++e) f[e] = pix >= avail ? 0.f : __uint_as_float(v[e]) * sx;
    float2 *d = reinterpret_cast<float2 *>(raw + (DB ? (cc & 1) * raw_bytes : 0) + pix * PITCH + (q & 3) * 16);
    d[0] = make_float2(f[0], f[1]);
    d[1] = make_float2(f[2], f[3]);
  };
  auto prefetch = [&](int cc) {
    const unsigned char *base = xg + (int64_t)cc * X.chunk_stride;
#pragma unroll
    for (int i = 0; i < kWnPF; ++i) pf[i] = *reinterpret_cast<const u32x4w *>(base + piece_off(min(t + kWnThreads * i, npieces - 1)));
  };
  auto commit = [&](int cc) {
#pragma unroll
    for (int i = 0; i < kWnPF; ++i) {
      piece_store(min(t + kWnThreads * i, npieces - 1), pf[i], cc);
    }
    const unsigned char *base = xg + (int64_t)cc * X.chunk_stride;
    for (int q = t + kWnThreads * kWnPF; q < npieces; q += kWnThreads)
      piece_store(q, *reinterpret_cast<const u32x4w *>(base + piece_off(q)), cc);
  };

  const int nsteps = 2 * nch;
  const unsigned ub_wave = __builtin_amdgcn_readfirstlane((unsigned)((((unsigned)ntile * nsteps) * kWnXi + NP * pg) * 2 * kWnN + nblk * 32));
  const u32x4w *ub = reinterpret_cast<const u32x4w *>(U) + ub_wave + g * kWnN + l31;
  u32x4w bf[NP];
  auto load_b = [&](int step, int p) { return ub[((unsigned)step * kWnXi + p) * 2 * kWnN]; };

  auto transform = [&](auto half_tag, int step) {
    constexpr int HALF = decltype(half_tag)::value;
    const unsigned char *src = raw + (DB ? ((step >> 1) & 1) * raw_bytes : 0) + toff + (step & 1) * 32;
    uint32_t *dst = vbuf + (step & 1) * kWnVFloats + vpos;
    __builtin_amdgcn_s_setprio(3);
    float tm[3][6];
#pragma unroll
    for (int jp = 0; jp < 3; ++jp) {
      f32x2v d[6], o[3];
#pragma unroll
      for (int i = 0; i < 6; ++i)
        d[i] = f32x2v{*reinterpret_cast<const float *>(src + (i * Wp + 2 * jp) * PITCH),
                      *reinterpret_cast<const float *>(src + (i * Wp + 2 * jp + 1) * PITCH)};
      wn_bt3<HALF, f32x2v>(d, o);
#pragma unroll
      for (int r = 0; r < 3; ++r) tm[r][2 * jp] = o[r][0], tm[r][2 * jp + 1] = o[r][1];
    }
#pragma unroll
    for (int r = 0; r < 3; ++r) {
      float o[6];
      wn_bt_pk(tm[r], o);
#pragma unroll
      for (int e = 0; e < 6; ++e) dst[(r * 6 + e) * 256] = (DBG & 32) ? (uint32_t)__float_as_uint(o[e]) : wn16_split(o[e]);
    }
    __builtin_amdgcn_s_setprio(0);
  };

  auto multiply = [&](int s, int sn) {
    const u32x4w *va = reinterpret_cast<const u32x4w *>(vbuf + (s & 1) * kWnVFloats + (NP * pg) * 256 + g * 128 + l31 * 4);
    u32x4w ra[2][2];
    auto read_pair = [&](int p, int sl) {
      ra[sl][0] = va[p * 64];
      if (p + 1 < NP) ra[sl][1] = va[(p + 1) * 64];
    };
    auto swapped = [](u32x4w w) {
      u32x4w r;
#pragma unroll
      for (int e = 0; e < 4; ++e) r[e] = __builtin_amdgcn_alignbit(w[e], w[e], 16);
      return r;
    };
    read_pair(0, 0);
#pragma unroll
    for (int p = 0; p < NP; p += 2) {
      const int sl = (p >> 1) & 1;
      if (p + 2 < NP) read_pair(p + 2, sl ^ 1);
      __builtin_amdgcn_sched_barrier(0);
      const f16x8 a0v = __builtin_bit_cast(f16x8, ra[sl][0]);
      const f16x8 b0v = __builtin_bit_cast(f16x8, bf[p]), b0s = __builtin_bit_cast(f16x8, swapped(bf[p]));
      if (p + 1 < NP) {
        const f16x8 a1v = __builtin_bit_cast(f16x8, ra[sl][1]);
        const f16x8 b1v = __builtin_bit_cast(f16x8, bf[p + 1]), b1s = __builtin_bit_cast(f16x8, swapped(bf[p + 1]));
        acc[p] = __builtin_amdgcn_mfma_f32_32x32x16_f16(a0v, b0v, acc[p], 0, 0, 0);
        acc[p + 1] = __builtin_amdgcn_mfma_f32_32x32x16_f16(a1v, b1v, acc[p + 1], 0, 0, 0);
        acc[p] = __builtin_amdgcn_mfma_f32_32x32x16_f16(a0v, b0s, acc[p], 0, 0, 0);
        acc[p + 1] = __builtin_amdgcn_mfma_f32_32x32x16_f16(a1v, b1s, acc[p + 1], 0, 0, 0);
        if constexpr (!(DBG & 4)) {
          bf[p] = load_b(sn, p);
          bf[p + 1] = load_b(sn, p + 1);
        }
      } else {
        acc[p] = __builtin_amdgcn_mfma_f32_32x32x16_f16(a0v, b0v, acc[p], 0, 0, 0);
        acc[p] = __builtin_amdgcn_mfma_f32_32x32x16_f16(a0v, b0s, acc[p], 0, 0, 0);
        if constexpr (!(DBG & 4)) bf[p] = load_b(sn, p);
      }
      __builtin_amdgcn_sched_barrier(0);
    }
  };

  prefetch(0);
  commit(0);
#pragma unroll
  for (int p = 0; p < NP; ++p) bf[p] = load_b(0, p);
  __syncthreads();
  if (xh == 0) transform(Half0{}, 0);
  else transform(Half1{}, 0);
  __syncthreads();

  stamp(t_pro);
  for (int s = 0; s < nsteps; ++s) {
    const int cc = s >> 1;
    const int sn = min(s + 1, nsteps - 1);
    const bool stage_next = !(s & 1) && cc + 1 < nch;
    constexpr bool kT = !(DBG & 1), kM = !(DBG & 2), kS = !(DBG & 8);
    if (xh == 0) {
      if constexpr (kM) multiply(s, sn);
      __builtin_amdgcn_sched_barrier(0);
      stamp(t_first);
      if (kS && stage_next) {
        prefetch(cc + 1);
        if constexpr (kT) transform(Half0{}, s + 1);
        if constexpr (DB) commit(cc + 1);
      } else {
        if constexpr (kT) transform(Half0{}, s + 1);
      }
      stamp(t_second);
    } else {
      if (kS && stage_next) {
        prefetch(cc + 1);
        if constexpr (kT) transform(Half1{}, s + 1);
        if constexpr (DB) commit(cc + 1);
      } else {
        if constexpr (kT) transform(Half1{}, s + 1);
      }
      __builtin_amdgcn_sched_barrier(0);
      stamp(t_first);
      if constexpr (kM) multiply(s, sn);
      stamp(t_second);
    }
    __syncthreads();
    stamp(t_bar);
    if constexpr (!DB) {
      if (stage_next) {
        commit(cc + 1);
        __syncthreads();
      }
    }
  }

  float4 *xch = reinterpret_cast<float4 *>(gfla_smem);
  constexpr int MM4 = M * M / 4;
  const int col = ntile * kWnN + nblk * 32 + l31;
  float *ob = out + b * out_bs + col;
  auto partial = [&](auto pg_tag, int i, float (&part)[M * M]) {
    constexpr int PG = decltype(pg_tag)::value;
#pragma unroll
    for (int e = 0; e < M * M; ++e) part[e] = 0.f;
#pragma unroll
    for (int a = 0; a < 6; ++a) {
      constexpr int first = NP * PG, last = NP * PG + NP - 1;
      const int e0 = a * 6 > first ? 0 : first - a * 6, e1 = a * 6 + 5 < last ? 5 : last - a * 6;
      if (a * 6 + 5 < first || a * 6 > last) continue;
      float tj[M];
#pragma unroll
      for (int j = 0; j < M; ++j) {
        float sacc = 0.f;
#pragma unroll
        for (int e = 0; e < 6; ++e)
          if (e >= e0 && e <= e1 && WnAT<M>::v[j][e] != 0.f) sacc = fmaf(WnAT<M>::v[j][e], acc[a * 6 + e - first][i], sacc);
        tj[j] = sacc;
      }
#pragma unroll
      for (int ii = 0; ii < M; ++ii)
        if (WnAT<M>::v[ii][a] != 0.f) {
#pragma unroll
          for (int j = 0; j < M; ++j) part[ii * M + j] = fmaf(WnAT<M>::v[ii][a], tj[j], part[ii * M + j]);
        }
    }
  };
  constexpr int QPR = M == 2 ? 4 : 1;
  auto finish = [&](auto pg_tag) {
    constexpr int PG = decltype(pg_tag)::value;
#pragma unroll
    for (int q0 = 0; q0 < 4; q0 += QPR) {
      float part[QPR][4][M * M];
#pragma unroll
      for (int qq = 0; qq < QPR; ++qq)
#pragma unroll
        for (int r = 0; r < 4; ++r) partial(pg_tag, 4 * (q0 + qq) + r, part[qq][r]);
      if constexpr (!(DBG & 256)) __syncthreads();
#pragma unroll
      for (int qq = 0; qq < QPR; ++qq) {
        const int qd = q0 + qq;
        if (PG != qd && !(DBG & 256)) {
          const int w3 = (PG - qd - 1) & 3;
          float4 *dst = xch + (((qq * 3 + w3) * 2 + nblk) * 4 * MM4) * 64 + lane;
#pragma unroll
          for (int r = 0; r < 4; ++r)
#pragma unroll
            for (int c4 = 0; c4 < MM4; ++c4)
              dst[(r * MM4 + c4) * 64] = make_float4(part[qq][r][4 * c4], part[qq][r][4 * c4 + 1], part[qq][r][4 * c4 + 2],
                                                     part[qq][r][4 * c4 + 3]);
        }
      }
      if constexpr (!(DBG & 256)) __syncthreads();
#pragma unroll
      for (int qq = 0; qq < QPR; ++qq) {
        const int qd = q0 + qq;
        if (PG != qd) continue;
#pragma unroll
        for (int w3 = 0; w3 < ((DBG & 256) ? 0 : 3); ++w3) {
          const float4 *srcp = xch + (((qq * 3 + w3) * 2 + nblk) * 4 * MM4) * 64 + lane;
#pragma unroll
          for (int r = 0; r < 4; ++r)
#pragma unroll
            for (int c4 = 0; c4 < MM4; ++c4) {
              const float4 v = srcp[(r * MM4 + c4) * 64];
              part[qq][r][4 * c4] += v.x, part[qq][r][4 * c4 + 1] += v.y, part[qq][r][4 * c4 + 2] += v.z, part[qq][r][4 * c4 + 3] += v.w;
            }
        }
#pragma unroll
        for (int r = 0; r < 4; ++r) {
          const int slot_ = 8 * qd + 4 * g + r, tau = tile0 + slot_;
          if (slot_ >= geo.tpg || tau >= ntiles || col >= n_valid) continue;
          const int ty = tau / geo.TW, tx = tau - ty * geo.TW;
#pragma unroll
          for (int i = 0; i < M; ++i) {
            const int yo = M * ty + i;
            if (yo >= Ho) continue;
#pragma unroll
            for (int j = 0; j < M; ++j) {
              const int xo = M * tx + j;
              if (xo < Wv && (!(DBG & 128) || part[qq][r][i * M + j] == 1.2345f))
                ob[(int64_t)(yo * Wv + xo) * ldo] = (part[qq][r][i * M + j] * inv_x) * inv_w;
            }
          }
        }
      }
    }
  };
  if constexpr (DBG & 64) {
    float keep = 0.f;
#pragma unroll
    for (int p = 0; p < NP; ++p)
#pragma unroll
      for (int i = 0; i < 16; ++i) keep += acc[p][i];
    if (keep == 1.2345f) ob[0] = keep * inv_x * inv_w;
    return;
  }
  if (pg == 0) finish(PgTag<0>{});
  else if (pg == 1) finish(PgTag<1>{});
  else if (pg == 2) finish(PgTag<2>{});
  else finish(PgTag<3>{});
  if constexpr (DBG & 16) {
    stamp(t_epi);
    if (stamps && lane == 0) {
      unsigned long long *o = stamps + ((int64_t)blockIdx.x * 8 + wave) * 6;
      o[0] = t_pro, o[1] = t_first, o[2] = t_second, o[3] = t_bar, o[4] = t_epi, o[5] = (unsigned long long)xh;
    }
  }
}

static unsigned wn16_lds_bytes(int k, const WnGeo &g, bool double_raw) {
  const int m = k == 5 ? 2 : 4;
  const unsigned raw = k == 5 ? wn_raw_bytes<5>(g) : wn_raw_bytes<3>(g);
  const unsigned main_loop = (unsigned)(2 * kWnVFloats * 4) + (double_raw ? 2u : 1u) * raw;
  const unsigned exchange = (unsigned)(3 * 2 * 4 * m * m * 64 * 4) * (m == 2 ? 4u : 1u);
  return main_loop > exchange ? main_loop : exchange;
}

static int wn16_launch(const Wn16ConvJob *jobs, int njobs, int64_t B, int nch, const uint32_t *amax_w, hipStream_t stream) {
  Wn16KArgs a[2];
  int64_t wgs[2] = {0, 0};
  bool db = tuning(21) != 1;
  unsigned lds = 0;
  for (int j = 0; j < njobs; ++j) db = db && wn16_lds_bytes(3, wn_geometry<3>(jobs[j].M, jobs[j].Wv, jobs[j].Wp), true) <= kWnLdsLimit;
  for (int j = 0; j < 2; ++j) {
    const Wn16ConvJob &J = jobs[j < njobs ? j : 0];
    const WnGeo g = wn_geometry<3>(J.M, J.Wv, J.Wp);
    const int ntn = (int)ceil_div(J.n_valid, kWnN);
    const int64_t groups = B * g.ngroups;
    a[j] = Wn16KArgs{J.X, J.U, J.amax_x, J.out, J.out_bs, J.ldo, J.n_valid, J.M / J.Wv, J.Wv, J.Wp, g, ntn, groups, J.S};
    if (j < njobs) {
      wgs[j] = ceil_div(groups, 8) * 8 * ntn;
      lds = std::max(lds, wn16_lds_bytes(3, g, db));
    }
  }
  if (wgs[0] + wgs[1] > 0x7fffffffLL || lds > kWnLdsLimit) return GFLA_ERR_UNSUPPORTED;
  auto kern = db ? fc_wino16_conv_kernel<3, true> : fc_wino16_conv_kernel<3, false>;
  (void)hipFuncSetAttribute(reinterpret_cast<const void *>(kern), hipFuncAttributeMaxDynamicSharedMemorySize, (int)lds);
  kern<<<dim3((unsigned)(wgs[0] + wgs[1])), kWnThreads, lds, stream>>>(a[0], a[1], (unsigned)wgs[0], nch, amax_w,
                                                                         db ? g_wino_stamps : nullptr);
  return launch_status();
}

bool fc_wino16_fits(int M, int Wv, int Wp, int k) {
  if (!fc_wino_fits(M, Wv, Wp, k)) return false;
  const WnGeo g = k == 5 ? wn_geometry<5>(M, Wv, Wp) : wn_geometry<3>(M, Wv, Wp);
  return wn16_lds_bytes(k, g, false) <= kWnLdsLimit;
}

int fc_wino16_conv_jobs(const Wn16ConvJob *jobs, int njobs, int64_t B, int nch, int k, const uint32_t *amax_w, hipStream_t stream) {
  if (B <= 0 || njobs <= 0) return GFLA_OK;
  if (njobs > 2 || !amax_w || k != 3) return GFLA_ERR_UNSUPPORTED;
  for (int j = 0; j < njobs; ++j)
    if (!jobs[j].amax_x || !fc_wino16_fits(jobs[j].M, jobs[j].Wv, jobs[j].Wp, k)) return GFLA_ERR_UNSUPPORTED;
  if (njobs == 2 && tuning(21) == 2) {
    const int st = fc_wino16_conv_jobs(jobs, 1, B, nch, k, amax_w, stream);
    return st != GFLA_OK ? st : fc_wino16_conv_jobs(jobs + 1, 1, B, nch, k, amax_w, stream);
  }
  return wn16_launch(jobs, njobs, B, nch, amax_w, stream);
}

}
```

global_flow_local_attention_amd/fc_mfma.py:

```python
import ctypes

import torch
from torch.autograd import Function

from . import _lib

MODES = (0, 1, 2, 3, 4, 5)
DEFAULT_MODE = 5
MODE_NAMES = {0: "f32 MFMA, direct convolution", 1: "one f16 term per operand (exact for bf16 values), f32 accumulate",
              2: "two f16 terms per operand, f32 accumulate", 3: "three f16 terms per operand, f32 accumulate",
              4: "f32 MFMA, Winograd-domain convolutions F(2x2,5x5) / F(4x4,3x3)",
              5: "two f16 terms per operand on f16 MFMA, f32 accumulate: direct kernels (k5 convolutions, data gradients) + "
                 "Winograd domain F(2x2,5x5) / F(4x4,3x3) (k3 forward, k5 weight gradient)"}


def supported(C, H, W, k, mode=DEFAULT_MODE):
    return bool(_lib.lib().gfla_fc_supported(int(C), int(H), int(W), int(k), int(mode)))


def resolve_mode(C, H, W, k, mode=None):
    mode = DEFAULT_MODE if mode is None else int(mode)
    if mode not in MODES:
        return None
    if supported(C, H, W, k, mode):
        return mode
    if mode == 5 and supported(C, H, W, k, 4):
        return 4
    if mode in (4, 5) and supported(C, H, W, k, 0):
        return 0
    return None


def workspace_bytes(B, C, H, W, k, mode, which):
    n = _lib.lib().gfla_fc_workspace_bytes(int(B), int(C), int(H), int(W), int(k), int(mode), int(which))
    if n < 0:
        raise ValueError("fc_mfma: unsupported shape B=%d C=%d %dx%d k=%d mode=%d" % (B, C, H, W, k, mode))
    return n


def geometry(H, W, k, is_source):
    out = (ctypes.c_int64 * 13)()
    rc = _lib.lib().gfla_fc_geometry(int(H), int(W), int(k), 1 if is_source else 0, ctypes.cast(out, ctypes.c_void_p))
    if rc != 0:
        raise ValueError("gfla_fc_geometry: status %d" % rc)
    names = ("Hp", "Wp", "Ho", "Wo", "pad_t", "pad_l", "M", "Md", "lead", "Sx", "Sz", "Mg", "Mdg")
    return dict(zip(names, (int(v) for v in out)))


def _check(source, target, flow, w0, w1, k):
    _lib.require_gpu(source, target, flow, w0, w1)
    B, C, H, W = source.shape
    if tuple(target.shape) != (B, C, H, W) or tuple(flow.shape) != (B, 2, H, W):
        raise ValueError("fc_mfma: source %s, target %s and flow %s must share B, C (features) and H, W" %
                         (tuple(source.shape), tuple(target.shape), tuple(flow.shape)))
    if tuple(w0.shape) != (128, 2 * C, k, k) or tuple(w1.shape[:2]) != (k * k, 128):
        raise ValueError("fc_mfma: weights %s / %s do not belong to an ExtractorAttn(%d, %d)" %
                         (tuple(w0.shape), tuple(w1.shape), C, k))
    for t in (source, target, flow, w0, w1):
        if t.dtype != torch.float32:
            raise TypeError("fc_mfma: float32 only (got %s)" % t.dtype)


def _f32c(t):
    return None if t is None else t.detach().float().contiguous()


def forward_call(source, target, flow, w0, b0, w1, b1, k, slope, mode):
    B, C, H, W = source.shape
    w0c, w1c, b0c, b1c = _f32c(w0), _f32c(w1).reshape(k * k, 128), _f32c(b0), _f32c(b1)
    ws = torch.empty(workspace_bytes(B, C, H, W, k, mode, 0), dtype=torch.uint8, device=source.device)
    logits = torch.empty((B, k * k, H, W), dtype=torch.float32, device=source.device)
    P = _lib.ptr
    if source.dtype == torch.float16:
        assert mode == 1, "gfla_fc_forward_f16 feeds the mode-1 backward"
        _lib.call("gfla_fc_forward_f16", source, P(source), P(target), P(flow), P(w0c), P(b0c), P(w1c), P(b1c), P(ws), P(logits),
                  B, C, H, W, k, float(slope))
    else:
        _lib.call("gfla_fc_forward_f32", source, P(source), P(target), P(flow), P(w0c), P(b0c), P(w1c), P(b1c), P(ws), P(logits),
                  B, C, H, W, k, float(slope), mode)
    return logits, ws, w1c


def backward_call(ws, flow, w1c, g_logits, dims, w_shapes, need, flags=0, g_source=None, g_flow=None):
    B, C, H, W, k, slope, mode = dims
    w0_shape, w1_shape, has_b0, has_b1 = w_shapes
    dev = flow.device
    g_logits = g_logits.contiguous()

    def new(shape, wanted):
        return torch.empty(shape, dtype=torch.float32, device=dev) if wanted else None

    g = (new((B, C, H, W), need[0]) if g_source is None else g_source, new((B, C, H, W), need[1]),
         new((B, 2, H, W), need[2]) if g_flow is None else g_flow, new(w0_shape, need[3]), new((128,), need[4] and has_b0),
         new(w1_shape, need[5]), new((k * k,), need[6] and has_b1))
    scratch = torch.empty(workspace_bytes(B, C, H, W, k, mode, 1), dtype=torch.uint8, device=dev)
    _lib.call("gfla_fc_backward_f32", flow, _lib.ptr(ws), _lib.ptr(flow), _lib.ptr(w1c), _lib.ptr(g_logits),
              _lib.ptr(scratch), *[_lib.ptr(t) for t in g], B, C, H, W, k, slope, mode, flags)
    return g


def aggregate_backward_f32(source, flow, attn, g_out, g_source, g_flow, g_logits, k, apply_softmax=True):
    b, c, hs, ws = source.shape
    h, w = flow.shape[2:]
    table = _lib.scatter_workspace(source, b, h, w, (k + 1) ** 2) if g_source is not None else None
    _lib.call("gfla_local_attn_aggregate_bwd_ws_f32", source, _lib.ptr(source), _lib.ptr(flow), _lib.ptr(attn), _lib.ptr(g_out),
              _lib.ptr(g_source), _lib.ptr(g_flow), _lib.ptr(g_logits), _lib.ptr(table), b, c, hs, ws, h, w, k,
              1 if apply_softmax else 0)


class FcMfmaFunction(Function):
    @staticmethod
    def forward(ctx, source, target, flow, w0, b0, w1, b1, kernel_size, slope, mode):
        k, mode = int(kernel_size), int(mode)
        _check(source, target, flow, w0, w1, k)
        source, target, flow = source.contiguous(), target.contiguous(), flow.contiguous()
        logits, ws, w1c = forward_call(source, target, flow, w0, b0, w1, b1, k, slope, mode)
        ctx.save_for_backward(flow, w1c, ws)
        ctx.dims = tuple(source.shape) + (k, float(slope), mode)
        ctx.w_shapes = (w0.shape, w1.shape, b0 is not None, b1 is not None)
        return logits

    @staticmethod
    def backward(ctx, g_logits):
        flow, w1c, ws = ctx.saved_tensors
        return backward_call(ws, flow, w1c, g_logits, ctx.dims, ctx.w_shapes, ctx.needs_input_grad) + (None, None, None)
```

include/gfla_hip.h:

```cpp
#ifndef GFLA_HIP_H_
#define GFLA_HIP_H_

#include <stdint.h>

#ifdef __cplusplus
extern "C" {
#endif

typedef enum gfla_status {
  GFLA_OK = 0,
  GFLA_ERR_NULL_POINTER = -1,
  GFLA_ERR_BAD_SHAPE = -2,
  GFLA_ERR_UNSUPPORTED = -3,
  GFLA_ERR_LAUNCH = -4
} gfla_status;

typedef void *gfla_stream_t;

#define GFLA_ABI_VERSION 8
int gfla_abi_version(void);
const char *gfla_status_string(int status);

int gfla_set_tuning(int key, int value);

enum gfla_path {
  GFLA_PATH_BE_BWD_LDS = 0,
  GFLA_PATH_BE_BWD_GLOBAL = 1,
  GFLA_PATH_FC_FWD_MODE0 = 2,
  GFLA_PATH_FC_FWD_MODE1 = 3,
  GFLA_PATH_FC_FWD_MODE2 = 4,
  GFLA_PATH_FC_FWD_MODE3 = 5,
  GFLA_PATH_FC_FWD_MODE4 = 6,
  GFLA_PATH_FC_BWD_MODE0 = 7,
  GFLA_PATH_FC_BWD_MODE1 = 8,
  GFLA_PATH_FC_BWD_MODE2 = 9,
  GFLA_PATH_FC_BWD_MODE3 = 10,
  GFLA_PATH_FC_BWD_MODE4 = 11,
  GFLA_PATH_BE_FWD_PIX = 12,
  GFLA_PATH_BE_FWD_GPIX = 13,
  GFLA_PATH_BE_BWD_TILE = 14,
  GFLA_PATH_RS_FWD_BIG = 15,
  GFLA_PATH_RS_BWD1_TILE = 16,
  GFLA_PATH_RS_BWD2_BIG = 17,
  GFLA_PATH_FC_FWD_MODE5 = 18,
  GFLA_PATH_FC_BWD_MODE5 = 19,
  GFLA_PATH_GEMM_F64 = 20,
  GFLA_PATH_FC_PACK_F16 = 21,
  GFLA_PATH_COUNT = 22
};
int64_t gfla_path_count(int path);

int gfla_big_plane_geometry(int op, int64_t B, int64_t C, int64_t Hs, int64_t Ws, int64_t H, int64_t W, int span,
                            int elem_size, int64_t *out);
int64_t gfla_xcd_swizzle(int64_t block, int64_t nwg);

#define GFLA_DECL_BLOCK_EXTRACTOR(SFX, T)                                                          \
  int gfla_block_extractor_fwd_##SFX(const T *source, const T *flow, T *out, int64_t B, int64_t C, \
                                     int64_t Hs, int64_t Ws, int64_t Hf, int64_t Wf,               \
                                     int kernel_size, gfla_stream_t stream);
GFLA_DECL_BLOCK_EXTRACTOR(f32, float)
GFLA_DECL_BLOCK_EXTRACTOR(f64, double)
GFLA_DECL_BLOCK_EXTRACTOR(bf16, uint16_t)
GFLA_DECL_BLOCK_EXTRACTOR(f16, uint16_t)
#undef GFLA_DECL_BLOCK_EXTRACTOR

#define GFLA_DECL_BLOCK_EXTRACTOR_BWD(SFX, T)                                                      \
  int gfla_block_extractor_bwd_##SFX(const T *source, const T *flow, const T *grad_out,            \
                                     T *grad_source, T *grad_flow, int64_t B, int64_t C,           \
                                     int64_t Hs, int64_t Ws, int64_t Hf, int64_t Wf,               \
                                     int kernel_size, gfla_stream_t stream);
GFLA_DECL_BLOCK_EXTRACTOR_BWD(f32, float)
GFLA_DECL_BLOCK_EXTRACTOR_BWD(f64, double)
#undef GFLA_DECL_BLOCK_EXTRACTOR_BWD

int gfla_unfold_supported(int64_t Hs, int64_t Ws, int kernel_size, int elem_size);
#define GFLA_DECL_UNFOLD_FWD(SFX, T)                                                               \
  int gfla_block_extractor_unfold_fwd_##SFX(const T *source, const T *flow, T *out_unfold,         \
                                            int64_t B, int64_t C, int64_t Hs, int64_t Ws,          \
                                            int64_t Hf, int64_t Wf, int kernel_size, int layout,   \
                                            gfla_stream_t stream);
GFLA_DECL_UNFOLD_FWD(f32, float)
GFLA_DECL_UNFOLD_FWD(f64, double)
GFLA_DECL_UNFOLD_FWD(bf16, uint16_t)
GFLA_DECL_UNFOLD_FWD(f16, uint16_t)
#undef GFLA_DECL_UNFOLD_FWD

#define GFLA_DECL_UNFOLD_BWD(SFX, T)                                                               \
  int gfla_block_extractor_unfold_bwd_##SFX(const T *source, const T *flow, const T *grad_unfold,  \
                                            T *grad_source, T *grad_flow, int64_t B, int64_t C,    \
                                            int64_t Hs, int64_t Ws, int64_t Hf, int64_t Wf,        \
                                            int kernel_size, int layout, gfla_stream_t stream);
GFLA_DECL_UNFOLD_BWD(f32, float)
GFLA_DECL_UNFOLD_BWD(f64, double)
#undef GFLA_DECL_UNFOLD_BWD

#define GFLA_DECL_RESHAPE(SFX, T)                                                                  \
  int gfla_local_attn_reshape_fwd_##SFX(const T *in, T *out, int64_t B, int64_t H, int64_t W,      \
                                        int kernel_size, gfla_stream_t stream);                    \
  int gfla_local_attn_reshape_bwd_##SFX(const T *grad_out, T *grad_in, int64_t B, int64_t H,       \
                                        int64_t W, int kernel_size, gfla_stream_t stream);
GFLA_DECL_RESHAPE(f32, float)
GFLA_DECL_RESHAPE(f64, double)
GFLA_DECL_RESHAPE(bf16, uint16_t)
GFLA_DECL_RESHAPE(f16, uint16_t)
#undef GFLA_DECL_RESHAPE

#define GFLA_RESAMPLE_TRUNC_COMPAT 1
#define GFLA_RESAMPLE_OVERWRITE_IN1 2
#define GFLA_DECL_RESAMPLE_FWD(SFX, T)                                                             \
  int gfla_resample2d_fwd_##SFX(const T *in1, const T *in2, T *out, int64_t B, int64_t C,          \
                                int64_t Hi, int64_t Wi, int64_t H, int64_t W, int kernel_size,     \
                                int dilation, gfla_stream_t stream);
GFLA_DECL_RESAMPLE_FWD(f32, float)
GFLA_DECL_RESAMPLE_FWD(f64, double)
GFLA_DECL_RESAMPLE_FWD(bf16, uint16_t)
GFLA_DECL_RESAMPLE_FWD(f16, uint16_t)
#undef GFLA_DECL_RESAMPLE_FWD

#define GFLA_DECL_RESAMPLE_BWD(SFX, T)                                                             \
  int gfla_resample2d_bwd_##SFX(const T *in1, const T *in2, const T *grad_out, T *grad_in1,        \
                                T *grad_in2, int64_t B, int64_t C, int64_t Hi, int64_t Wi,         \
                                int64_t H, int64_t W, int kernel_size, int dilation,               \
                                int trunc_compat, gfla_stream_t stream);
GFLA_DECL_RESAMPLE_BWD(f32, float)
GFLA_DECL_RESAMPLE_BWD(f64, double)
#undef GFLA_DECL_RESAMPLE_BWD

#define GFLA_DECL_AGGREGATE_FWD(SFX, T)                                                            \
  int gfla_local_attn_aggregate_fwd_##SFX(const T *source, const T *flow, const T *logits, T *out, \
                                          T *attn_out, int64_t B, int64_t C, int64_t Hs,           \
                                          int64_t Ws, int64_t H, int64_t W, int kernel_size,       \
                                          int apply_softmax, gfla_stream_t stream);
GFLA_DECL_AGGREGATE_FWD(f32, float)
GFLA_DECL_AGGREGATE_FWD(f64, double)
GFLA_DECL_AGGREGATE_FWD(bf16, uint16_t)
GFLA_DECL_AGGREGATE_FWD(f16, uint16_t)
#undef GFLA_DECL_AGGREGATE_FWD

int64_t gfla_aggregate_fwd_workspace_bytes(int64_t B, int64_t H, int64_t W, int kernel_size);
int gfla_aggregate_bwd_supported(int64_t Hs, int64_t Ws, int elem_size);
int gfla_aggregate_fwd_geometry(int64_t B, int64_t C, int64_t Hs, int64_t Ws, int64_t H, int64_t W, int kernel_size,
                                int64_t *out);
int gfla_local_attn_aggregate_fwd_ws_f32(const float *source, const float *flow, const float *logits, float *out,
                                         float *attn_out, void *workspace, int64_t B, int64_t C, int64_t Hs,
                                         int64_t Ws, int64_t H, int64_t W, int kernel_size, int apply_softmax,
                                         gfla_stream_t stream);
int gfla_local_attn_aggregate_fwd_ws_bf16(const uint16_t *source, const uint16_t *flow, const uint16_t *logits,
                                          uint16_t *out, uint16_t *attn_out, void *workspace, int64_t B, int64_t C,
                                          int64_t Hs, int64_t Ws, int64_t H, int64_t W, int kernel_size,
                                          int apply_softmax, gfla_stream_t stream);
int gfla_local_attn_aggregate_fwd_ws_f16(const uint16_t *source, const uint16_t *flow, const uint16_t *logits,
                                         uint16_t *out, uint16_t *attn_out, void *workspace, int64_t B, int64_t C,
                                         int64_t Hs, int64_t Ws, int64_t H, int64_t W, int kernel_size,
                                         int apply_softmax, gfla_stream_t stream);

#define GFLA_DECL_AGGREGATE_BWD(SFX, T)                                                            \
  int gfla_local_attn_aggregate_bwd_##SFX(const T *source, const T *flow, const T *attn,           \
                                          const T *grad_out, T *grad_source, T *grad_flow,         \
                                          T *grad_logits, int64_t B, int64_t C, int64_t Hs,        \
                                          int64_t Ws, int64_t H, int64_t W, int kernel_size,       \
                                          int apply_softmax, gfla_stream_t stream);
GFLA_DECL_AGGREGATE_BWD(f32, float)
GFLA_DECL_AGGREGATE_BWD(f64, double)
#undef GFLA_DECL_AGGREGATE_BWD


int gfla_block_extractor_bwd_bf16(const uint16_t *source, const uint16_t *flow, const uint16_t *grad_out,
                                  uint16_t *grad_source, float *grad_flow, int64_t B, int64_t C, int64_t Hs, int64_t Ws,
                                  int64_t Hf, int64_t Wf, int kernel_size, gfla_stream_t stream);
int gfla_block_extractor_unfold_bwd_bf16(const uint16_t *source, const uint16_t *flow, const uint16_t *grad_unfold,
                                         uint16_t *grad_source, float *grad_flow, int64_t B, int64_t C, int64_t Hs,
                                         int64_t Ws, int64_t Hf, int64_t Wf, int kernel_size, int layout,
                                         gfla_stream_t stream);
int gfla_local_attn_aggregate_bwd_bf16(const uint16_t *source, const uint16_t *flow, const uint16_t *attn,
                                       const uint16_t *grad_out, uint16_t *grad_source, float *grad_flow,
                                       float *grad_logits, int64_t B, int64_t C, int64_t Hs, int64_t Ws, int64_t H,
                                       int64_t W, int kernel_size, int apply_softmax, gfla_stream_t stream);
int gfla_local_attn_source_bwd_bf16(const uint16_t *source, const uint16_t *flow, const uint16_t *grad_unfold,
                                    const uint16_t *attn, const uint16_t *grad_out, uint16_t *grad_source,
                                    float *grad_flow, int64_t B, int64_t C, int64_t Hs, int64_t Ws, int64_t H,
                                    int64_t W, int kernel_size, int layout, gfla_stream_t stream);
int gfla_resample2d_bwd_bf16(const uint16_t *in1, const uint16_t *in2, const uint16_t *grad_out, uint16_t *grad_in1,
                             float *grad_in2, int64_t B, int64_t C, int64_t Hi, int64_t Wi, int64_t H, int64_t W,
                             int kernel_size, int dilation, int trunc_compat, gfla_stream_t stream);

#define GFLA_DECL_BWD16(SFX, T)                                                                                        \
  int gfla_block_extractor_bwd_##SFX(const T *source, const T *flow, const T *grad_out, T *grad_source, float *grad_flow, \
                                     int64_t B, int64_t C, int64_t Hs, int64_t Ws, int64_t Hf, int64_t Wf,               \
                                     int kernel_size, gfla_stream_t stream);                                             \
  int gfla_block_extractor_unfold_bwd_##SFX(const T *source, const T *flow, const T *grad_unfold, T *grad_source,        \
                                            float *grad_flow, int64_t B, int64_t C, int64_t Hs, int64_t Ws, int64_t Hf,  \
                                            int64_t Wf, int kernel_size, int layout, gfla_stream_t stream);              \
  int gfla_local_attn_aggregate_bwd_##SFX(const T *source, const T *flow, const T *attn, const T *grad_out,             \
                                          T *grad_source, float *grad_flow, float *grad_logits, int64_t B, int64_t C,    \
                                          int64_t Hs, int64_t Ws, int64_t H, int64_t W, int kernel_size,                 \
                                          int apply_softmax, gfla_stream_t stream);                                      \
  int gfla_local_attn_source_bwd_##SFX(const T *source, const T *flow, const T *grad_unfold, const T *attn,             \
                                       const T *grad_out, T *grad_source, float *grad_flow, int64_t B, int64_t C,        \
                                       int64_t Hs, int64_t Ws, int64_t H, int64_t W, int kernel_size, int layout,        \
                                       gfla_stream_t stream);                                                            \
  int gfla_resample2d_bwd_##SFX(const T *in1, const T *in2, const T *grad_out, T *grad_in1, float *grad_in2, int64_t B, \
                                int64_t C, int64_t Hi, int64_t Wi, int64_t H, int64_t W, int kernel_size, int dilation,  \
                                int trunc_compat, gfla_stream_t stream);
GFLA_DECL_BWD16(f16, uint16_t)
#undef GFLA_DECL_BWD16

int64_t gfla_scatter_workspace_bytes(int64_t B, int64_t H, int64_t W, int patch_entries);
int gfla_local_attn_aggregate_bwd_ws_f32(const float *source, const float *flow, const float *attn,
                                         const float *grad_out, float *grad_source, float *grad_flow,
                                         float *grad_logits, void *workspace, int64_t B, int64_t C, int64_t Hs,
                                         int64_t Ws, int64_t H, int64_t W, int kernel_size, int apply_softmax,
                                         gfla_stream_t stream);
int gfla_resample2d_bwd_ws_f32(const float *in1, const float *in2, const float *grad_out, float *grad_in1,
                               float *grad_in2, void *workspace, int64_t B, int64_t C, int64_t Hi, int64_t Wi,
                               int64_t H, int64_t W, int kernel_size, int dilation, int trunc_compat,
                               gfla_stream_t stream);

#define GFLA_DECL_SOURCE_BWD(SFX, T)                                                               \
  int gfla_local_attn_source_bwd_##SFX(const T *source, const T *flow, const T *grad_unfold,       \
                                       const T *attn, const T *grad_out, T *grad_source,           \
                                       T *grad_flow, int64_t B, int64_t C, int64_t Hs, int64_t Ws, \
                                       int64_t H, int64_t W, int kernel_size, int layout,          \
                                       gfla_stream_t stream);
GFLA_DECL_SOURCE_BWD(f32, float)
GFLA_DECL_SOURCE_BWD(f64, double)
#undef GFLA_DECL_SOURCE_BWD

#define GFLA_DECL_FC_TAIL(SFX, T)                                                                    \
  int gfla_fc_tail_fwd_##SFX(const T *hs, int64_t hs_sb, int64_t hs_so, const T *ht, const T *b0,   \
                             const T *w1, const T *b1, T *logits, int64_t B, int64_t Hc, int64_t HW, \
                             int KK, double slope, gfla_stream_t stream);                           \
  int gfla_fc_tail_bwd_##SFX(const T *hs, int64_t hs_sb, int64_t hs_so, const T *ht, const T *b0,   \
                             const T *w1, const T *g_logits, T *g_hs, T *g_ht, T *act,              \
                             T *bias_partials, int64_t B, int64_t Hc, int64_t HW, int KK,           \
                             double slope, gfla_stream_t stream);
GFLA_DECL_FC_TAIL(f32, float)
GFLA_DECL_FC_TAIL(f64, double)
#undef GFLA_DECL_FC_TAIL

#define GFLA_FC_ACCUMULATE_SOURCE 1
#define GFLA_FC_ACCUMULATE_FLOW 2
int gfla_fc_supported(int64_t C, int64_t H, int64_t W, int kernel_size, int mode);
int64_t gfla_fc_workspace_bytes(int64_t B, int64_t C, int64_t H, int64_t W, int kernel_size, int mode,
                                int which);
int gfla_fc_forward_f32(const float *source, const float *target, const float *flow, const float *w0,
                        const float *b0, const float *w1, const float *b1, void *workspace, float *logits,
                        int64_t B, int64_t C, int64_t H, int64_t W, int kernel_size, double slope, int mode,
                        gfla_stream_t stream);
int gfla_fc_backward_f32(void *workspace, const float *flow, const float *w1, const float *grad_logits,
                         void *scratch, float *grad_source, float *grad_target, float *grad_flow, float *grad_w0,
                         float *grad_b0, float *grad_w1, float *grad_b1, int64_t B, int64_t C, int64_t H,
                         int64_t W, int kernel_size, double slope, int mode, int flags, gfla_stream_t stream);
int gfla_fc_forward_f16(const uint16_t *source, const uint16_t *target, const float *flow, const float *w0,
                        const float *b0, const float *w1, const float *b1, void *workspace, float *logits,
                        int64_t B, int64_t C, int64_t H, int64_t W, int kernel_size, double slope, gfla_stream_t stream);
int gfla_fc_geometry(int64_t H, int64_t W, int kernel_size, int is_source, int64_t *out);
int gfla_fc_conv_fwd_f32(const float *x, const float *w0, int is_source, void *workspace, float *out, int64_t B,
                         int64_t C, int64_t H, int64_t W, int kernel_size, int mode, gfla_stream_t stream);
int gfla_fc_conv_bwd_f32(const float *z, int is_source, void *workspace, void *scratch, float *grad_x,
                         float *grad_w0, int64_t B, int64_t C, int64_t H, int64_t W, int kernel_size, int mode,
                         gfla_stream_t stream);
int gfla_fc_kernel_f32(int which, void *workspace, void *scratch, int64_t B, int64_t C, int64_t H, int64_t W,
                       int kernel_size, int mode, gfla_stream_t stream);
int gfla_fc_tr_probe(const int16_t *image, int n_halves, const int32_t *offsets, int16_t *out,
                     gfla_stream_t stream);
int gfla_fc_wino_debug_buffer(void *buffer);

int gfla_replicate_pad_bwd_f32(const float *grad_padded, float *grad_in, int64_t planes, int64_t H,
                               int64_t W, int pad_left, int pad_right, int pad_top, int pad_bottom,
                               gfla_stream_t stream);
int gfla_replicate_pad_bwd_f64(const double *grad_padded, double *grad_in, int64_t planes, int64_t H,
                               int64_t W, int pad_left, int pad_right, int pad_top, int pad_bottom,
                               gfla_stream_t stream);

int64_t gfla_gemm_f64_workspace_bytes(int64_t M, int64_t N, int64_t K, int split_k);
int gfla_gemm_f64(double *c, const int64_t *c_view, const double *a, const int64_t *a_view, const double *b,
                  const int64_t *b_view, int64_t M, int64_t N, int64_t K, int beta, int split_k, void *workspace,
                  gfla_stream_t stream);

int64_t gfla_max_cosine_workspace_bytes(int64_t B, int64_t Ns, int64_t Nt);
int gfla_max_cosine_fwd_f32(const float *source, const float *target, void *workspace, float *out_max,
                            int32_t *out_idx, int64_t B, int64_t C, int64_t Ns, int64_t Nt, double eps,
                            gfla_stream_t stream);
int gfla_max_cosine_fwd_f16(const uint16_t *source, const uint16_t *target, void *workspace, float *out_max,
                            int32_t *out_idx, int64_t B, int64_t C, int64_t Ns, int64_t Nt, double eps,
                            gfla_stream_t stream);
int gfla_max_cosine_fwd_bf16(const uint16_t *source, const uint16_t *target, void *workspace, float *out_max,
                             int32_t *out_idx, int64_t B, int64_t C, int64_t Ns, int64_t Nt, double eps,
                             gfla_stream_t stream);

int gfla_correctness_map_fwd_f32(const float *warped, const float *target, const float *best,
                                 float *loss_map, float *stats, int64_t B, int64_t C, int64_t N,
                                 double eps_cos, double eps, gfla_stream_t stream);
int gfla_correctness_map_bwd_f32(const float *warped, const float *target, const float *best,
                                 const float *stats, const float *loss_map, const float *grad_map,
                                 float *grad_warped, float *grad_target, float *grad_best, int64_t B,
                                 int64_t C, int64_t N, double eps_cos, double eps, gfla_stream_t stream);
int gfla_correctness_map_fwd_f16(const float *warped, const uint16_t *target, const float *best,
                                 float *loss_map, float *stats, int64_t B, int64_t C, int64_t N,
                                 double eps_cos, double eps, gfla_stream_t stream);
int gfla_correctness_map_bwd_f16(const float *warped, const uint16_t *target, const float *best,
                                 const float *stats, const float *loss_map, const float *grad_map,
                                 float *grad_warped, uint16_t *grad_target, float *grad_best, int64_t B,
                                 int64_t C, int64_t N, double eps_cos, double eps, gfla_stream_t stream);
int gfla_correctness_map_fwd_bf16(const float *warped, const uint16_t *target, const float *best,
                                 float *loss_map, float *stats, int64_t B, int64_t C, int64_t N,
                                 double eps_cos, double eps, gfla_stream_t stream);
int gfla_correctness_map_bwd_bf16(const float *warped, const uint16_t *target, const float *best,
                                 const float *stats, const float *loss_map, const float *grad_map,
                                 float *grad_warped, uint16_t *grad_target, float *grad_best, int64_t B,
                                 int64_t C, int64_t N, double eps_cos, double eps, gfla_stream_t stream);

int gfla_convert_multi(const void *src0, void *dst0, int64_t n0, const void *src1, void *dst1, int64_t n1, const void *src2,
                       void *dst2, int64_t n2, const void *src3, void *dst3, int64_t n3, int to_bf16, gfla_stream_t stream);
#define GFLA_CONVERT_F16_TO_F32 2
#define GFLA_CONVERT_F32_TO_F16 3

int gfla_mask_blend_fwd_f32(const float *out, const float *attn_p, const float *attn_r, const float *mask_p,
                            const float *mask_r, float *y, int64_t B, int64_t C, int64_t HW, gfla_stream_t stream);
int gfla_mask_blend_fwd_bf16(const uint16_t *out, const uint16_t *attn_p, const uint16_t *attn_r, const uint16_t *mask_p,
                             const uint16_t *mask_r, uint16_t *y, int64_t B, int64_t C, int64_t HW, gfla_stream_t stream);
int gfla_mask_blend_bwd_f32(const float *out, const float *attn_p, const float *attn_r, const float *mask_p,
                            const float *mask_r, const float *grad_y, float *g_out, float *g_attn_p, float *g_attn_r,
                            float *g_mask_p, float *g_mask_r, int64_t B, int64_t C, int64_t HW, gfla_stream_t stream);
int gfla_mask_blend_bwd_bf16(const uint16_t *out, const uint16_t *attn_p, const uint16_t *attn_r, const uint16_t *mask_p,
                             const uint16_t *mask_r, const uint16_t *grad_y, uint16_t *g_out, uint16_t *g_attn_p,
                             uint16_t *g_attn_r, float *g_mask_p, float *g_mask_r, int64_t B, int64_t C, int64_t HW,
                             gfla_stream_t stream);
int gfla_mask_blend_fwd_f16(const uint16_t *out, const uint16_t *attn_p, const uint16_t *attn_r, const uint16_t *mask_p,
                            const uint16_t *mask_r, uint16_t *y, int64_t B, int64_t C, int64_t HW, gfla_stream_t stream);
int gfla_mask_blend_bwd_f16(const uint16_t *out, const uint16_t *attn_p, const uint16_t *attn_r, const uint16_t *mask_p,
                            const uint16_t *mask_r, const uint16_t *grad_y, uint16_t *g_out, uint16_t *g_attn_p,
                            uint16_t *g_attn_r, float *g_mask_p, float *g_mask_r, int64_t B, int64_t C, int64_t HW,
                            gfla_stream_t stream);

int64_t gfla_affine_reg_workspace_bytes(int64_t B, int64_t H, int64_t W, int k);
int gfla_affine_reg_fwd_f32(const float *flow, void *workspace, float *loss, int64_t B, int64_t H, int64_t W, int k,
                            gfla_stream_t stream);
int gfla_affine_reg_fwd_f64(const double *flow, void *workspace, double *loss, int64_t B, int64_t H, int64_t W, int k,
                            gfla_stream_t stream);
int gfla_affine_reg_fwd_f16(const uint16_t *flow, void *workspace, float *loss, int64_t B, int64_t H, int64_t W, int k,
                            gfla_stream_t stream);
int gfla_affine_reg_fwd_bf16(const uint16_t *flow, void *workspace, float *loss, int64_t B, int64_t H, int64_t W, int k,
                             gfla_stream_t stream);
int gfla_affine_reg_bwd_f32(const float *flow, const float *grad_loss, void *workspace, float *grad_flow, int64_t B,
                            int64_t H, int64_t W, int k, gfla_stream_t stream);
int gfla_affine_reg_bwd_f64(const double *flow, const double *grad_loss, void *workspace, double *grad_flow, int64_t B,
                            int64_t H, int64_t W, int k, gfla_stream_t stream);
int gfla_affine_reg_bwd_f16(const uint16_t *flow, const float *grad_loss, void *workspace, uint16_t *grad_flow, int64_t B,
                            int64_t H, int64_t W, int k, gfla_stream_t stream);
int gfla_affine_reg_bwd_bf16(const uint16_t *flow, const float *grad_loss, void *workspace, uint16_t *grad_flow, int64_t B,
                             int64_t H, int64_t W, int k, gfla_stream_t stream);

int64_t gfla_gram_l1_workspace_bytes(int64_t B, int64_t C, int64_t N);
int gfla_gram_l1_fwd_f32(const float *x, const float *y, void *workspace, float *diff, float *loss, int64_t B, int64_t C,
                         int64_t N, gfla_stream_t stream);
int gfla_gram_l1_fwd_f16(const uint16_t *x, const uint16_t *y, void *workspace, float *diff, float *loss, int64_t B,
                         int64_t C, int64_t N, gfla_stream_t stream);
int gfla_gram_l1_fwd_bf16(const uint16_t *x, const uint16_t *y, void *workspace, float *diff, float *loss, int64_t B,
                          int64_t C, int64_t N, gfla_stream_t stream);
int gfla_gram_l1_bwd_f32(const float *feat, const float *diff, const float *grad_loss, float *grad_feat, int64_t B,
                         int64_t C, int64_t N, int negate, gfla_stream_t stream);
int gfla_gram_l1_bwd_f16(const uint16_t *feat, const float *diff, const float *grad_loss, uint16_t *grad_feat, int64_t B,
                         int64_t C, int64_t N, int negate, gfla_stream_t stream);
int gfla_gram_l1_bwd_bf16(const uint16_t *feat, const float *diff, const float *grad_loss, uint16_t *grad_feat, int64_t B,
                          int64_t C, int64_t N, int negate, gfla_stream_t stream);

int gfla_flow_warp_fwd_f32(const float *source, const float *flow, float *out, int64_t B, int64_t C, int64_t Hs, int64_t Ws,
                           int64_t H, int64_t W, double gx, double gy, double mx, double my, gfla_stream_t stream);
int gfla_flow_warp_fwd_f64(const double *source, const double *flow, double *out, int64_t B, int64_t C, int64_t Hs,
                           int64_t Ws, int64_t H, int64_t W, double gx, double gy, double mx, double my,
                           gfla_stream_t stream);
int gfla_flow_warp_fwd_f16(const uint16_t *source, const float *flow, float *out, int64_t B, int64_t C, int64_t Hs,
                           int64_t Ws, int64_t H, int64_t W, double gx, double gy, double mx, double my,
                           gfla_stream_t stream);
int gfla_flow_warp_fwd_bf16(const uint16_t *source, const float *flow, float *out, int64_t B, int64_t C, int64_t Hs,
                            int64_t Ws, int64_t H, int64_t W, double gx, double gy, double mx, double my,
                            gfla_stream_t stream);
int gfla_flow_warp_bwd_f32(const float *source, const float *flow, const float *grad_out, float *grad_source,
                           float *grad_flow, int64_t B, int64_t C, int64_t Hs, int64_t Ws, int64_t H, int64_t W, double gx,
                           double gy, double mx, double my, gfla_stream_t stream);
int gfla_flow_warp_bwd_f64(const double *source, const double *flow, const double *grad_out, double *grad_source,
                           double *grad_flow, int64_t B, int64_t C, int64_t Hs, int64_t Ws, int64_t H, int64_t W, double gx,
                           double gy, double mx, double my, gfla_stream_t stream);
int gfla_flow_warp_bwd_f16(const uint16_t *source, const float *flow, const float *grad_out, float *grad_source,
                           float *grad_flow, int64_t B, int64_t C, int64_t Hs, int64_t Ws, int64_t H, int64_t W, double gx,
                           double gy, double mx, double my, gfla_stream_t stream);
int gfla_flow_warp_bwd_bf16(const uint16_t *source, const float *flow, const float *grad_out, float *grad_source,
                            float *grad_flow, int64_t B, int64_t C, int64_t Hs, int64_t Ws, int64_t H, int64_t W, double gx,
                            double gy, double mx, double my, gfla_stream_t stream);

#ifdef __cplusplus
}
#endif
#endif
```

Measured before the change: 9642.

## Replace Winograd f16 forward with paired direct-f16 convolution launching both halves

```diff
diff --git a/global_flow_local_attention_amd/_lib.py b/global_flow_local_attention_amd/_lib.py
--- a/global_flow_local_attention_amd/_lib.py
+++ b/global_flow_local_attention_amd/_lib.py
@@ -47,6 +47,8 @@
     "gfla_fc_forward_f32": [_ptr] * 9 + [_i64] * 4 + [_int, ctypes.c_double, _int, _ptr],
     "gfla_fc_backward_f32": [_ptr] * 12 + [_i64] * 4 + [_int, ctypes.c_double, _int, _int, _ptr],
     "gfla_fc_geometry": [_i64, _i64, _int, _int, _ptr],
+    "gfla_fc_conv_tiling": [_i64] * 4 + [_int, _int, _ptr],
+    "gfla_fc_map_offsets": [_i64] * 4 + [_int, _int, _ptr],
     "gfla_fc_conv_fwd_f32": [_ptr, _ptr, _int, _ptr, _ptr] + [_i64] * 4 + [_int, _int, _ptr],
     "gfla_fc_conv_bwd_f32": [_ptr, _int, _ptr, _ptr, _ptr, _ptr] + [_i64] * 4 + [_int, _int, _ptr],
     "gfla_fc_tr_probe": [_ptr, _int, _ptr, _ptr, _ptr],
diff --git a/global_flow_local_attention_amd/csrc/fc_block.hip b/global_flow_local_attention_amd/csrc/fc_block.hip
--- a/global_flow_local_attention_amd/csrc/fc_block.hip
+++ b/global_flow_local_attention_amd/csrc/fc_block.hip
@@ -1,3 +1,6 @@
+#include <algorithm>
+
+#include "fc_conv_tiling.h"
 #include "fc_gemm.h"
 
 namespace gfla {
@@ -10,7 +13,6 @@
   kConvDirect,
   kConvDirect16,
   kConvWino32,
-  kConvWino16,
 };
 enum FcWgrad {
   kWgradDirect32,
@@ -28,6 +30,7 @@
   int pack_split;
   bool pack_uf, pack_ud;
   bool dgrads_together;
+  bool fwd_pair, dgrad_pair;
   FcWgrad wgrad;
   FcWgrad wgrad_both;
   bool wgrads_together;
@@ -40,14 +43,16 @@
   FcPlan P;
   P.split = fc_base_mode(mode);
   P.scaled = P.split != 0 || mode == 5;
-  P.fwd = mode == 4 ? kConvWino32 : mode == 5 ? (k == 5 ? kConvDirect16 : kConvWino16) : kConvDirect;
+  P.fwd = mode == 4 ? kConvWino32 : mode == 5 ? kConvDirect16 : kConvDirect;
   P.dgrad = mode == 4 ? kConvWino32 : mode == 5 ? kConvDirect16 : kConvDirect;
   P.pack_wf = P.fwd == kConvDirect || P.fwd == kConvDirect16;
   P.pack_wd = P.dgrad == kConvDirect || P.dgrad == kConvDirect16;
   P.pack_split = P.dgrad == kConvDirect16 ? 2 : P.split;
-  P.pack_uf = P.fwd == kConvWino32 || P.fwd == kConvWino16;
+  P.pack_uf = P.fwd == kConvWino32;
   P.pack_ud = P.dgrad == kConvWino32;
   P.dgrads_together = fc_is_wino(mode);
+  P.fwd_pair = P.fwd == kConvDirect16 && k == 3;
+  P.dgrad_pair = P.dgrad == kConvDirect16 && k == 3;
   P.wgrad_x32 = mode == 1 && k == 5;
   P.wgrad = fc_is_wino(mode) || P.wgrad_x32 ? (mode == 5 && k == 5 ? kWgradWino16 : kWgradWino32)
                                             : (P.split ? kWgradDirect16 : kWgradDirect32);
@@ -145,8 +150,8 @@
         !fc_wino_fits(ht.Mv, ht.Wo, ht.Wp, k) || !fc_wino_fits(ht.Md, ht.Wp, ht.Wp, k))
       return GFLA_ERR_UNSUPPORTED;
   } else if (mode == 5) {
-    if (!fc_wino16_fits(hs.Mv, hs.Wo, hs.Wp, k) || !fc_wino16_fits(hs.Md, hs.Wp, hs.Wp, k) ||
-        !fc_wino16_fits(ht.Mv, ht.Wo, ht.Wp, k) || !fc_wino16_fits(ht.Md, ht.Wp, ht.Wp, k))
+    if (!fc_wino_fits(hs.Mv, hs.Wo, hs.Wp, k) || !fc_wino_fits(hs.Md, hs.Wp, hs.Wp, k) ||
+        !fc_wino_fits(ht.Mv, ht.Wo, ht.Wp, k) || !fc_wino_fits(ht.Md, ht.Wp, ht.Wp, k))
       return GFLA_ERR_UNSUPPORTED;
   }
   if (mode != 4 && (!fc_conv_fits(hs.Wo, hs.Wp, k, direct) || !fc_conv_fits(hs.Wp, hs.Wp, k, direct) ||
@@ -169,7 +174,6 @@
     GFLA_TRY(fc_pack_weights(w0, P.pack_split ? a_w : nullptr, P.pack_wf ? ws + L.wf_t : nullptr, P.pack_wf ? ws + L.wf_s : nullptr,
                              P.pack_wd ? ws + L.wd_t : nullptr, P.pack_wd ? ws + L.wd_s : nullptr, C, k, P.pack_split, stream));
   float *u_ft = reinterpret_cast<float *>(ws + L.wu_ft), *u_fs = reinterpret_cast<float *>(ws + L.wu_fs);
-  if (P.fwd == kConvWino16) return fc_wino16_pack_weights(w0, a_w, u_ft, u_fs, C, k, stream);
   if (P.pack_uf || P.pack_ud)
     return fc_wino_pack_weights(w0, P.pack_uf ? u_ft : nullptr, P.pack_uf ? u_fs : nullptr,
                                 P.pack_ud ? reinterpret_cast<float *>(ws + L.wu_dt) : nullptr,
@@ -177,23 +181,20 @@
   return GFLA_OK;
 }
 
-static int fc_wino_jobs(const WnConvJob *jobs, int njobs, const uint32_t *const *amax, const uint32_t *amax_w, bool w16, int64_t B,
-                        int nch, int k, hipStream_t stream) {
-  if (!w16) return fc_wino_conv_jobs(jobs, njobs, B, nch, k, stream);
-  Wn16ConvJob j16[2];
-  for (int j = 0; j < njobs && j < 2; ++j)
-    j16[j] = Wn16ConvJob{jobs[j].X, reinterpret_cast<const uint32_t *>(jobs[j].U), amax[j], jobs[j].out, jobs[j].out_bs, jobs[j].ldo,
-                         jobs[j].n_valid, jobs[j].M, jobs[j].Wv, jobs[j].Wp, jobs[j].S};
-  return fc_wino16_conv_jobs(j16, njobs, B, nch, k, amax_w, stream);
+static int fc_direct16_jobs(const ConvJobArgs *jobs, int njobs, bool pair, int64_t B, int nch, int k, const uint32_t *amax_w,
+                            hipStream_t stream) {
+  if (pair || njobs == 1) return fc_conv_f32src_jobs(jobs, njobs, B, nch, k, amax_w, stream);
+  for (int j = 0; j < njobs; ++j) GFLA_TRY(fc_conv_f32src_jobs(jobs + j, 1, B, nch, k, amax_w, stream));
+  return GFLA_OK;
 }
 
 static int fc_fwd_convs(const FcLayout &L, const unsigned char *ws, float *out_s, float *out_t, int64_t B, int k,
-                        hipStream_t stream) {
+                        hipStream_t stream, bool force_pair = false) {
   const FcPlan &P = L.plan;
   const uint32_t *amax = reinterpret_cast<const uint32_t *>(ws + L.amax);
   WnConvJob jobs[2];
-  const uint32_t *am[2];
-  int n = 0;
+  ConvJobArgs direct[2];
+  int n = 0, nd = 0;
   for (int h = 0; h < 2; ++h) {
     const bool src = h == 0;
     float *out = src ? out_s : out_t;
@@ -203,8 +204,8 @@
     const uint32_t *a_x = amax + (src ? kAmaxSrc : kAmaxTgt);
     const unsigned char *wf = ws + (src ? L.wf_s : L.wf_t);
     if (P.fwd == kConvDirect16) {
-      GFLA_TRY(fc_conv_f32src(X, wf, fc_wpack_bytes(1, L.nch_c, k, 2) / 2, out, g.Mg * kFcHidden, kFcHidden, kFcHidden, B, L.nch_c,
-                              g.Mv, g.Wo, g.Wp, k, a_x, amax + kAmaxW, stream));
+      direct[nd++] = ConvJobArgs{X, wf, fc_wpack_bytes(1, L.nch_c, k, 2) / 2, out, g.Mg * kFcHidden, kFcHidden, kFcHidden, g.Mv, g.Wo,
+                                 g.Wp, a_x};
     } else if (P.fwd == kConvDirect) {
       GFLA_TRY(fc_conv(X, wf, fc_wpack_bytes(1, L.nch_c, k, P.split) / fc_nsplit(P.split), out, g.Mg * kFcHidden, kFcHidden,
                        kFcHidden, B, L.nch_c, g.Mv, g.Wo, g.Wp, k, P.split, P.split ? a_x : nullptr,
@@ -212,19 +213,21 @@
     } else {
       jobs[n] = WnConvJob{X, reinterpret_cast<const float *>(ws + (src ? L.wu_fs : L.wu_ft)), out, g.Mg * kFcHidden, kFcHidden,
                           kFcHidden, g.Mv, g.Wo, g.Wp, g.Sx};
-      am[n++] = a_x;
+      ++n;
     }
   }
-  return n ? fc_wino_jobs(jobs, n, am, amax + kAmaxW, P.fwd == kConvWino16, B, L.nch_c, k, stream) : GFLA_OK;
+  if (nd) return fc_direct16_jobs(direct, nd, P.fwd_pair || force_pair, B, L.nch_c, k, amax + kAmaxW, stream);
+  return n ? fc_wino_conv_jobs(jobs, n, B, L.nch_c, k, stream) : GFLA_OK;
 }
 
 static int fc_dgrad_convs(const FcLayout &L, const unsigned char *ws, unsigned char *sc, bool want_s, bool want_t, int64_t B, int C,
-                          int k, hipStream_t stream) {
+                          int k, hipStream_t stream, bool force_pair = false) {
   const FcPlan &P = L.plan;
   const uint32_t *amax = reinterpret_cast<const uint32_t *>(ws + L.amax);
   const int nch_h = kFcHidden / kFcChunk;
   WnConvJob jobs[2];
-  int n = 0;
+  ConvJobArgs direct[2];
+  int n = 0, nd = 0;
   for (int h = 0; h < 2; ++h) {
     const bool src = h == 0;
     if (!(src ? want_s : want_t)) continue;
@@ -234,8 +237,8 @@
     const uint32_t *a_z = amax + (src ? kAmaxZs : kAmaxZt);
     const unsigned char *wd = ws + (src ? L.wd_s : L.wd_t);
     if (P.dgrad == kConvDirect16) {
-      GFLA_TRY(fc_conv_f32src(fc_desc_nhwc(dz, g.Sz, kFcHidden), wd, fc_wpack_bytes(L.nt_d, nch_h, k, 2) / 2, dx, g.Mdg * (int64_t)C,
-                              C, C, B, nch_h, g.Md, g.Wp, g.Wp, k, a_z, amax + kAmaxW, stream));
+      direct[nd++] = ConvJobArgs{fc_desc_nhwc(dz, g.Sz, kFcHidden), wd, fc_wpack_bytes(L.nt_d, nch_h, k, 2) / 2, dx, g.Mdg * (int64_t)C, C,
+                                 C, g.Md, g.Wp, g.Wp, a_z};
     } else if (P.dgrad == kConvDirect) {
       const PackedDesc Z = P.split ? fc_desc_packed(sc + (src ? L.zs_pk : L.zt_pk), B, nch_h, g.Sz, P.split)
                                    : fc_desc_nhwc(dz, g.Sz, kFcHidden);
@@ -246,6 +249,7 @@
                             g.Mdg * (int64_t)C, C, C, g.Md, g.Wp, g.Wp, g.Sz};
     }
   }
+  if (nd) return fc_direct16_jobs(direct, nd, P.dgrad_pair || force_pair, B, nch_h, k, amax + kAmaxW, stream);
   return n ? fc_wino_conv_jobs(jobs, n, B, nch_h, k, stream) : GFLA_OK;
 }
 
@@ -479,6 +483,47 @@
   return fc_args_ok(1, C, H, W, kernel_size, mode) == GFLA_OK ? 1 : 0;
 }
 
+int gfla_fc_conv_tiling(int64_t B, int64_t C, int64_t H, int64_t W, int kernel_size, int dgrad, int64_t *out) {
+  if (!out) return GFLA_ERR_NULL_POINTER;
+  GFLA_TRY(fc_args_ok(B, C, H, W, kernel_size, 5));
+  if (B <= 0) return GFLA_ERR_BAD_SHAPE;
+  const int k = kernel_size;
+  const FcHalf hs = fc_half((int)H, (int)W, k, true), ht = fc_half((int)H, (int)W, k, false);
+  const int nt = dgrad ? (int)ceil_div(C, kFcTN) : 1;
+  const ConvShape sh[2] = {dgrad ? ConvShape{hs.Md, hs.Wp, hs.Wp, nt} : ConvShape{hs.Mv, hs.Wo, hs.Wp, nt},
+                           dgrad ? ConvShape{ht.Md, ht.Wp, ht.Wp, nt} : ConvShape{ht.Mv, ht.Wo, ht.Wp, nt}};
+  ConvTiling tl[2];
+  int rounds = 0, slots = 0;
+  const int nmb = pick_conv_tiling2(sh, B, k, 2, tl, &rounds, &slots);
+  if (nmb == 0) return GFLA_ERR_UNSUPPORTED;
+  int64_t lds = 0;
+  for (int j = 0; j < 2; ++j) lds = std::max(lds, fc_conv_lds_bytes(nmb, sh[j].Wv, sh[j].Wp, k, 2));
+  int64_t *o = out;
+  *o++ = nmb, *o++ = rounds, *o++ = slots, *o++ = lds, *o++ = nt, *o++ = kFcMaxRowBlocks, *o++ = kFcConvLdsLimit, *o++ = 0;
+  for (int j = 0; j < 2; ++j) *o++ = ceil_div(sh[j].M, 32), *o++ = tl[j].T, *o++ = tl[j].base, *o++ = tl[j].rem;
+  for (int j = 0; j < 2; ++j) {
+    ConvTiling t1;
+    const int n1 = pick_conv_tiling(sh[j].M, B, nt, sh[j].Wv, sh[j].Wp, k, 2, &t1);
+    if (n1 == 0) return GFLA_ERR_UNSUPPORTED;
+    *o++ = n1, *o++ = t1.T, *o++ = t1.base, *o++ = t1.rem, *o++ = fc_conv_lds_bytes(n1, sh[j].Wv, sh[j].Wp, k, 2);
+  }
+  ConvSeg seg[4];
+  const int ntn[2] = {nt, nt};
+  const int64_t wgs = fc_conv_segments(tl, ntn, 2, B, nmb, seg);
+  if (wgs <= 0) return GFLA_ERR_UNSUPPORTED;
+  out[7] = wgs;
+  for (int a = 0; a < 4; ++a) *o++ = seg[a].end, *o++ = seg[a].job, *o++ = seg[a].nblk, *o++ = seg[a].per, *o++ = seg[a].first0;
+  return GFLA_OK;
+}
+
+int gfla_fc_map_offsets(int64_t B, int64_t C, int64_t H, int64_t W, int kernel_size, int mode, int64_t *out) {
+  if (!out) return GFLA_ERR_NULL_POINTER;
+  GFLA_TRY(fc_args_ok(B, C, H, W, kernel_size, mode));
+  const FcLayout L = fc_layout(B, (int)C, (int)H, (int)W, kernel_size, mode);
+  out[0] = L.gs, out[1] = L.gt, out[2] = L.dxs, out[3] = L.dxt;
+  return GFLA_OK;
+}
+
 int64_t gfla_fc_workspace_bytes(int64_t B, int64_t C, int64_t H, int64_t W, int kernel_size, int mode, int which) {
   if (fc_args_ok(B, C, H, W, kernel_size, mode) != GFLA_OK) return -1;
   const FcLayout L = fc_layout(B, (int)C, (int)H, (int)W, kernel_size, mode);
@@ -571,13 +616,15 @@
 int gfla_fc_kernel_f32(int which, void *workspace, void *scratch, int64_t B, int64_t C_, int64_t H_, int64_t W_,
                        int kernel_size, int mode, gfla_stream_t stream_) {
   if (!workspace || !scratch) return GFLA_ERR_NULL_POINTER;
-  if (which < 0 || which > 8 || (which > 5 && !fc_is_wino(mode))) return GFLA_ERR_BAD_SHAPE;
+  if (which < 0 || which > 10 || (which > 5 && !fc_is_wino(mode)) || (which > 8 && mode != 5)) return GFLA_ERR_BAD_SHAPE;
   const int C = (int)C_, H = (int)H_, W = (int)W_, k = kernel_size;
   GFLA_TRY(fc_args_ok(B, C, H, W, k, mode));
   if (B == 0) return GFLA_OK;
   hipStream_t stream = static_cast<hipStream_t>(stream_);
   const FcLayout L = fc_layout(B, C, H, W, k, mode);
   unsigned char *ws = static_cast<unsigned char *>(workspace), *sc = static_cast<unsigned char *>(scratch);
+  if (which == 9) return fc_fwd_convs(L, ws, reinterpret_cast<float *>(ws + L.gs), reinterpret_cast<float *>(ws + L.gt), B, k, stream, true);
+  if (which == 10) return fc_dgrad_convs(L, ws, sc, true, true, B, C, k, stream, true);
   const bool src = which == 6 || which == 7 || (which & 1) == 0, tgt = which > 5 || (which & 1) == 1;
   float *gs = reinterpret_cast<float *>(ws + L.gs), *gt = reinterpret_cast<float *>(ws + L.gt);
   switch (which) {
diff --git a/global_flow_local_attention_amd/csrc/fc_conv.hip b/global_flow_local_attention_amd/csrc/fc_conv.hip
--- a/global_flow_local_attention_amd/csrc/fc_conv.hip
+++ b/global_flow_local_attention_amd/csrc/fc_conv.hip
@@ -3,7 +3,7 @@
 namespace gfla {
 
 bool fc_conv_fits(int Wv, int Wp, int k, int mode) {
-  return (int64_t)fc_nsplit(mode) * fc_conv_tile_pixels(kFcMinRowBlocks, Wv, Wp, k) * (mode ? 48 : 80) <= 156 * 1024;
+  return fc_conv_lds_bytes(kFcMinRowBlocks, Wv, Wp, k, mode) <= kFcConvLdsLimit;
 }
 
 int fc_conv(const PackedDesc &X, const void *wk, int64_t w_split_stride, float *out, int64_t out_bs, int ldo,
diff --git a/global_flow_local_attention_amd/csrc/fc_conv_impl.h b/global_flow_local_attention_amd/csrc/fc_conv_impl.h
--- a/global_flow_local_attention_amd/csrc/fc_conv_impl.h
+++ b/global_flow_local_attention_amd/csrc/fc_conv_impl.h
@@ -1,10 +1,12 @@
 #pragma once
 
+#include <utility>
+
+#include "fc_conv_tiling.h"
 #include "fc_mma.h"
 
 namespace gfla {
 
-constexpr int kFcMinRowBlocks = 2, kFcMaxRowBlocks = 8;
 constexpr int kFcPrefetch = 8;
 
 template <int MODE>
@@ -27,39 +29,49 @@
     pf[q] = *reinterpret_cast<const u32x4 *>(src + (int64_t)min(pix0 + 64 * q, tmh - 1) * x_ps);
 }
 
-struct ConvTiling {
-  int T, base, rem, heavy, per_ntile;
+struct ConvJob {
+  PackedDesc X;
+  const unsigned char *Wk;
+  int64_t w_split_stride;
+  float *out;
+  int64_t out_bs;
+  const uint32_t *amax_x;
+  int ldo, n_valid, M, Wv, Wp;
+  int tmh;
+  ConvTiling tl;
 };
+struct ConvJobs {
+  ConvJob job[2];
+  ConvSeg seg[4];
+  int total, B, nch;
+  const uint32_t *amax_w;
+};
 
 template <int MODE, int KS, int NMB, bool SRC32 = false>
-__global__ __launch_bounds__(256, 2) void fc_conv_kernel(PackedDesc X, const unsigned char *__restrict__ Wk,
-                                                        int64_t w_split_stride, float *__restrict__ out,
-                                                        int64_t out_bs, int ldo, int n_valid, int M, int Wv, int Wp,
-                                                        int nch, int tmh, ConvTiling tl,
-                                                        const uint32_t *__restrict__ amax_x,
-                                                        const uint32_t *__restrict__ amax_w) {
+__global__ __launch_bounds__(256, 2) void fc_conv_kernel(ConvJobs jobs) {
   using F = Fc<MODE>;
   constexpr int KK = KS * KS, PITCH = F::PITCH, STEPS = F::KB * NMB;
   extern __shared__ __attribute__((aligned(16))) unsigned char gfla_smem[];
   unsigned char *xs = gfla_smem;
   const int t = threadIdx.x, lane = t & 63, wave = t >> 6, l31 = lane & 31, kh = lane >> 5;
   int wid = blockIdx.x;
-  const int ntile = wid / tl.per_ntile;
-  wid -= ntile * tl.per_ntile;
-  if (tl.per_ntile <= 2 * kNumCU && wid >= kNumCU) wid = tl.per_ntile - 1 - (wid - kNumCU);
-  else if (tl.per_ntile <= kNumCU && (ntile & 1)) wid = tl.per_ntile - 1 - wid;
-  int64_t b;
-  int first, nblk;
-  if (wid < tl.heavy) {
-    b = wid / tl.rem;
-    first = (wid - (int)b * tl.rem) * (tl.base + 1);
-    nblk = tl.base + 1;
-  } else {
-    const int u = wid - tl.heavy, per = tl.T - tl.rem;
-    b = u / per;
-    first = tl.rem * (tl.base + 1) + (u - (int)b * per) * tl.base;
-    nblk = tl.base;
-  }
+  if (jobs.total <= 2 * kNumCU && wid >= kNumCU) wid = jobs.total - 1 - (wid - kNumCU);
+  const int si = (wid >= jobs.seg[0].end) + (wid >= jobs.seg[1].end) + (wid >= jobs.seg[2].end);
+  const ConvSeg sg = jobs.seg[si];
+  if (si) wid -= jobs.seg[si - 1].end;
+  const ConvJob &J = jobs.job[sg.job];
+  const PackedDesc X = J.X;
+  const unsigned char *__restrict__ Wk = J.Wk;
+  float *__restrict__ out = J.out;
+  const int64_t w_split_stride = J.w_split_stride, out_bs = J.out_bs;
+  const int ldo = J.ldo, n_valid = J.n_valid, M = J.M, Wv = J.Wv, Wp = J.Wp, tmh = J.tmh, nch = jobs.nch;
+  const uint32_t *__restrict__ amax_x = J.amax_x, *__restrict__ amax_w = jobs.amax_w;
+  const int per_ntile = jobs.B * sg.per;
+  const int ntile = wid / per_ntile;
+  wid -= ntile * per_ntile;
+  const int64_t b = wid / sg.per;
+  const int first = sg.first0 + (wid - (int)b * sg.per) * sg.nblk;
+  const int nblk = sg.nblk;
   const int m0 = first * 32;
   const int y0 = m0 / Wv, p0 = y0 * Wp + (m0 - y0 * Wv);
   const int64_t x_ss = X.split_stride, x_cs = X.chunk_stride;
@@ -171,7 +183,7 @@
         else
           fa = load_frag<MODE>(xa_next + a_off[0], xplane, 0, kh);
         __builtin_amdgcn_sched_barrier(0);
-        if (mb + 1 < NMB || nblk == NMB)
+        if (mb + 2 < NMB || mb < nblk)
           acc[mb] = mma<MODE>(fc, cur[kb], acc[mb]);
       }
 #pragma unroll
@@ -197,62 +209,34 @@
 
 
 
-inline int fc_conv_tile_pixels(int mb, int Wv, int Wp, int k) {
-  const int tm = 32 * mb;
-  return tm + ((tm - 1) / Wv + 1) * (Wp - Wv) + (k - 1) * (Wp + 1);
-}
-
-inline int pick_conv_tiling(int M, int64_t B, int ntiles_n, int Wv, int Wp, int k, int mode, ConvTiling *tl) {
-  const int ns = fc_nsplit(mode), pitch = mode ? 48 : 80;
-  const int nb = (int)ceil_div(M, 32);
-  const int forced = tuning(11);
-  int64_t T = (2 * kNumCU) / (B * ntiles_n);
-  if (T < 1) T = 1;
-  if (T > nb) T = nb;
-  if (ceil_div(nb, T) > kFcMaxRowBlocks) T = ceil_div(nb, kFcMaxRowBlocks);
-  if (forced >= kFcMinRowBlocks && forced <= kFcMaxRowBlocks) T = ceil_div(nb, forced);
-  for (;; ++T) {
-    const int nmb = (int)ceil_div(nb, T);
-    const int64_t lds = (int64_t)ns * fc_conv_tile_pixels(nmb < kFcMinRowBlocks ? kFcMinRowBlocks : nmb, Wv, Wp, k) * pitch;
-    if (lds <= 156 * 1024) break;
-    if (nmb <= kFcMinRowBlocks) return 0;
-  }
-  tl->T = (int)T;
-  tl->base = nb / (int)T;
-  tl->rem = nb % (int)T;
-  tl->heavy = (int)B * tl->rem;
-  tl->per_ntile = (int)(B * T);
-  int nmb = tl->base + (tl->rem ? 1 : 0);
-  if (nmb < kFcMinRowBlocks) {
-    nmb = kFcMinRowBlocks;
-  }
-  return nmb;
-}
-
 template <int MODE, int KS, int NMB, bool SRC32 = false>
-static int launch_conv(const PackedDesc &X, const void *wk, int64_t w_split_stride, float *out, int64_t out_bs,
-                       int ldo, int n_valid, int64_t B, int nch, int M, int Wv, int Wp, const ConvTiling &tl,
-                       const uint32_t *amax_x, const uint32_t *amax_w, hipStream_t stream) {
+static int launch_conv(ConvJobs &jobs, int njobs, hipStream_t stream) {
   using F = Fc<MODE>;
-  const int tmh = fc_conv_tile_pixels(NMB, Wv, Wp, KS);
+  ConvTiling tl[2];
+  int ntn[2], tmh = 0;
+  for (int j = 0; j < njobs; ++j) {
+    ConvJob &J = jobs.job[j];
+    J.tmh = fc_conv_tile_pixels(NMB, J.Wv, J.Wp, KS);
+    if (J.tmh > tmh) tmh = J.tmh;
+    tl[j] = J.tl;
+    ntn[j] = (int)ceil_div(J.n_valid, kFcTN);
+  }
+  const int64_t wgs = fc_conv_segments(tl, ntn, njobs, jobs.B, NMB, jobs.seg);
+  if (wgs <= 0) return GFLA_ERR_UNSUPPORTED;
+  jobs.total = (int)wgs;
   const unsigned lds = (unsigned)(F::NS * tmh * F::PITCH);
-  const int64_t wgs = (int64_t)tl.per_ntile * ceil_div(n_valid, kFcTN);
-  if (wgs > 0x7fffffffLL) return GFLA_ERR_UNSUPPORTED;
   auto kern = fc_conv_kernel<MODE, KS, NMB, SRC32>;
   if (lds > 64 * 1024)
     (void)hipFuncSetAttribute(reinterpret_cast<const void *>(kern), hipFuncAttributeMaxDynamicSharedMemorySize, (int)lds);
-  kern<<<dim3((unsigned)wgs), 256, lds, stream>>>(X, static_cast<const unsigned char *>(wk), w_split_stride, out, out_bs,
-                                                  ldo, n_valid, M, Wv, Wp, nch, tmh, tl, amax_x, amax_w);
+  kern<<<dim3((unsigned)wgs), 256, lds, stream>>>(jobs);
   return launch_status();
 }
 
 template <int MODE, int KS, bool SRC32 = false>
-static int dispatch_conv(int nmb, const PackedDesc &X, const void *wk, int64_t wss, float *out, int64_t out_bs, int ldo,
-                         int n_valid, int64_t B, int nch, int M, int Wv, int Wp, const ConvTiling &tl, const uint32_t *ax,
-                         const uint32_t *aw, hipStream_t s) {
+static int dispatch_conv(int nmb, ConvJobs &jobs, int njobs, hipStream_t s) {
   switch (nmb) {
 #define GFLA_CASE(N_) \
-  case N_: return launch_conv<MODE, KS, N_, SRC32>(X, wk, wss, out, out_bs, ldo, n_valid, B, nch, M, Wv, Wp, tl, ax, aw, s)
+  case N_: return launch_conv<MODE, KS, N_, SRC32>(jobs, njobs, s)
     GFLA_CASE(2);
     GFLA_CASE(3);
     GFLA_CASE(4);
@@ -265,6 +249,17 @@
   return GFLA_ERR_UNSUPPORTED;
 }
 
+inline ConvJobs fc_conv_one_job(const PackedDesc &X, const void *wk, int64_t w_split_stride, float *out, int64_t out_bs, int ldo,
+                                int n_valid, int64_t B, int nch, int M, int Wv, int Wp, const ConvTiling &tl,
+                                const uint32_t *amax_x, const uint32_t *amax_w) {
+  ConvJobs jobs = {};
+  jobs.job[0] = ConvJob{X, static_cast<const unsigned char *>(wk), w_split_stride, out, out_bs, amax_x, ldo, n_valid, M, Wv, Wp, 0, tl};
+  jobs.B = (int)B;
+  jobs.nch = nch;
+  jobs.amax_w = amax_w;
+  return jobs;
+}
+
 template <int MODE>
 int fc_conv_mode(const PackedDesc &X, const void *wk, int64_t w_split_stride, float *out, int64_t out_bs, int ldo,
                  int n_valid, int64_t B, int nch, int M, int Wv, int Wp, int k, const uint32_t *amax_x,
@@ -278,11 +273,10 @@
     ConvTiling tl;                                                                                                    \
     const int nmb = pick_conv_tiling(M, B, (int)ceil_div(n_valid, kFcTN), Wv, Wp, k, MODE_, &tl);                      \
     if (nmb == 0) return GFLA_ERR_UNSUPPORTED;                                                                        \
-    if (k == 3)                                                                                                       \
-      return dispatch_conv<MODE_, 3>(nmb, X, wk, w_split_stride, out, out_bs, ldo, n_valid, B, nch, M, Wv, Wp, tl,     \
-                                     amax_x, amax_w, stream);                                                         \
-    return dispatch_conv<MODE_, 5>(nmb, X, wk, w_split_stride, out, out_bs, ldo, n_valid, B, nch, M, Wv, Wp, tl,       \
-                                   amax_x, amax_w, stream);                                                           \
-  }
-
-}
+    ConvJobs jobs = fc_conv_one_job(X, wk, w_split_stride, out, out_bs, ldo, n_valid, B, nch, M, Wv, Wp, tl, amax_x,   \
+                                    amax_w);                                                                          \
+    if (k == 3) return dispatch_conv<MODE_, 3>(nmb, jobs, 1, stream);                                                  \
+    return dispatch_conv<MODE_, 5>(nmb, jobs, 1, stream);                                                              \
+  }
+
+}
diff --git a/global_flow_local_attention_amd/csrc/fc_conv_m2.hip b/global_flow_local_attention_amd/csrc/fc_conv_m2.hip
--- a/global_flow_local_attention_amd/csrc/fc_conv_m2.hip
+++ b/global_flow_local_attention_amd/csrc/fc_conv_m2.hip
@@ -3,19 +3,41 @@
 namespace gfla {
 GFLA_DEFINE_FC_CONV_MODE(2)
 
+int fc_conv_f32src_jobs(const ConvJobArgs *args, int njobs, int64_t B, int nch, int k, const uint32_t *amax_w,
+                        hipStream_t stream) {
+  if (!args || njobs < 1 || njobs > 2 || (k != 3 && k != 5) || !amax_w) return GFLA_ERR_UNSUPPORTED;
+  if (B > 65535 || B <= 0) return B == 0 ? GFLA_OK : GFLA_ERR_UNSUPPORTED;
+  ConvJobs jobs = {};
+  ConvShape sh[2];
+  for (int j = 0; j < njobs; ++j) {
+    const ConvJobArgs &a = args[j];
+    if (!a.amax_x || a.X.pix_stride < 64 || a.M <= 0) return GFLA_ERR_UNSUPPORTED;
+    if (a.Wv <= 0 || a.Wv > a.Wp || !fc_conv_fits(a.Wv, a.Wp, k, 2)) return GFLA_ERR_UNSUPPORTED;
+    jobs.job[j] = ConvJob{a.X, static_cast<const unsigned char *>(a.wk), a.w_split_stride, a.out, a.out_bs, a.amax_x, a.ldo,
+                          a.n_valid, a.M, a.Wv, a.Wp, 0, ConvTiling{}};
+    sh[j] = ConvShape{a.M, a.Wv, a.Wp, (int)ceil_div(a.n_valid, kFcTN)};
+  }
+  jobs.B = (int)B;
+  jobs.nch = nch;
+  jobs.amax_w = amax_w;
+  int nmb;
+  if (njobs == 1) {
+    nmb = pick_conv_tiling(sh[0].M, B, sh[0].ntiles_n, sh[0].Wv, sh[0].Wp, k, 2, &jobs.job[0].tl);
+  } else {
+    ConvTiling tl[2];
+    nmb = pick_conv_tiling2(sh, B, k, 2, tl, nullptr, nullptr);
+    jobs.job[0].tl = tl[0];
+    jobs.job[1].tl = tl[1];
+  }
+  if (nmb == 0) return GFLA_ERR_UNSUPPORTED;
+  if (k == 3) return dispatch_conv<2, 3, true>(nmb, jobs, njobs, stream);
+  return dispatch_conv<2, 5, true>(nmb, jobs, njobs, stream);
+}
+
 int fc_conv_f32src(const PackedDesc &X32, const void *wk, int64_t w_split_stride, float *out, int64_t out_bs, int ldo,
                    int n_valid, int64_t B, int nch, int M, int Wv, int Wp, int k, const uint32_t *amax_x,
                    const uint32_t *amax_w, hipStream_t stream) {
-  if ((k != 3 && k != 5) || !amax_x || !amax_w || X32.pix_stride < 64) return GFLA_ERR_UNSUPPORTED;
-  if (B > 65535 || B <= 0 || M <= 0) return B == 0 ? GFLA_OK : GFLA_ERR_UNSUPPORTED;
-  if (Wv <= 0 || Wv > Wp || !fc_conv_fits(Wv, Wp, k, 2)) return GFLA_ERR_UNSUPPORTED;
-  ConvTiling tl;
-  const int nmb = pick_conv_tiling(M, B, (int)ceil_div(n_valid, kFcTN), Wv, Wp, k, 2, &tl);
-  if (nmb == 0) return GFLA_ERR_UNSUPPORTED;
-  if (k == 3)
-    return dispatch_conv<2, 3, true>(nmb, X32, wk, w_split_stride, out, out_bs, ldo, n_valid, B, nch, M, Wv, Wp, tl, amax_x, amax_w,
-                                     stream);
-  return dispatch_conv<2, 5, true>(nmb, X32, wk, w_split_stride, out, out_bs, ldo, n_valid, B, nch, M, Wv, Wp, tl, amax_x, amax_w,
-                                   stream);
+  const ConvJobArgs a{X32, wk, w_split_stride, out, out_bs, ldo, n_valid, M, Wv, Wp, amax_x};
+  return fc_conv_f32src_jobs(&a, 1, B, nch, k, amax_w, stream);
 }
 }
diff --git a/global_flow_local_attention_amd/csrc/fc_conv_tiling.h b/global_flow_local_attention_amd/csrc/fc_conv_tiling.h
--- /dev/null
+++ b/global_flow_local_attention_amd/csrc/fc_conv_tiling.h
@@ -0,0 +1,146 @@
+#pragma once
+
+#include "fc_gemm.h"
+
+namespace gfla {
+
+constexpr int kFcMinRowBlocks = 2, kFcMaxRowBlocks = 8;
+constexpr int64_t kFcConvLdsLimit = 156 * 1024;
+constexpr int64_t kFcConvLdsPerCU = 160 * 1024;
+
+struct ConvTiling {
+  int T, base, rem, heavy, per_ntile;
+};
+
+struct ConvShape {
+  int M, Wv, Wp;
+  int ntiles_n;
+};
+
+struct ConvSeg {
+  int end;
+  int job;
+  int nblk;
+  int per;
+  int first0;
+};
+
+inline int64_t fc_conv_segments(const ConvTiling *tl, const int *ntn, int njobs, int64_t B, int nmb, ConvSeg *seg) {
+  ConvSeg run[4];
+  int nrun = 0;
+  for (int j = 0; j < njobs; ++j) {
+    const ConvTiling &t = tl[j];
+    const int64_t per_b = B * ntn[j];
+    const int light = t.T - t.rem;
+    if (t.base + (t.rem ? 1 : 0) > nmb || t.base + 2 < nmb || t.base < 1) return 0;
+    if (per_b * t.T > 0x3fffffffLL) return 0;
+    if (t.rem) run[nrun++] = ConvSeg{(int)(per_b * t.rem), j, t.base + 1, t.rem, 0};
+    if (light) run[nrun++] = ConvSeg{(int)(per_b * light), j, t.base, light, t.rem * (t.base + 1)};
+  }
+  for (int a = 1; a < nrun; ++a)
+    for (int c = a; c > 0 && run[c].nblk > run[c - 1].nblk; --c) {
+      const ConvSeg tmp = run[c];
+      run[c] = run[c - 1];
+      run[c - 1] = tmp;
+    }
+  int64_t wgs = 0;
+  for (int a = 0; a < 4; ++a) {
+    if (a < nrun) {
+      wgs += run[a].end;
+      seg[a] = run[a];
+      seg[a].end = (int)wgs;
+    } else {
+      seg[a] = ConvSeg{0x7fffffff, 0, 0, 1, 0};
+    }
+  }
+  return wgs > 0x7fffffffLL ? 0 : wgs;
+}
+
+inline int fc_conv_tile_pixels(int mb, int Wv, int Wp, int k) {
+  const int tm = 32 * mb;
+  return tm + ((tm - 1) / Wv + 1) * (Wp - Wv) + (k - 1) * (Wp + 1);
+}
+inline int64_t fc_conv_lds_bytes(int mb, int Wv, int Wp, int k, int mode) {
+  return (int64_t)fc_nsplit(mode) * fc_conv_tile_pixels(mb, Wv, Wp, k) * (mode ? 48 : 80);
+}
+
+inline void fc_conv_set_tiling(ConvTiling *tl, int nb, int64_t T, int64_t B) {
+  tl->T = (int)T;
+  tl->base = nb / (int)T;
+  tl->rem = nb % (int)T;
+  tl->heavy = (int)B * tl->rem;
+  tl->per_ntile = (int)(B * T);
+}
+
+inline int pick_conv_tiling(int M, int64_t B, int ntiles_n, int Wv, int Wp, int k, int mode, ConvTiling *tl) {
+  const int nb = (int)ceil_div(M, 32);
+  const int forced = tuning(11);
+  int64_t T = (2 * kNumCU) / (B * ntiles_n);
+  if (T < 1) T = 1;
+  if (T > nb) T = nb;
+  if (ceil_div(nb, T) > kFcMaxRowBlocks) T = ceil_div(nb, kFcMaxRowBlocks);
+  if (forced >= kFcMinRowBlocks && forced <= kFcMaxRowBlocks) T = ceil_div(nb, forced);
+  for (;; ++T) {
+    const int nmb = (int)ceil_div(nb, T);
+    if (fc_conv_lds_bytes(nmb < kFcMinRowBlocks ? kFcMinRowBlocks : nmb, Wv, Wp, k, mode) <= kFcConvLdsLimit) break;
+    if (nmb <= kFcMinRowBlocks) return 0;
+  }
+  fc_conv_set_tiling(tl, nb, T, B);
+  const int nmb = tl->base + (tl->rem ? 1 : 0);
+  return nmb < kFcMinRowBlocks ? kFcMinRowBlocks : nmb;
+}
+
+inline int pick_conv_tiling2(const ConvShape *sh, int64_t B, int k, int mode, ConvTiling *tl, int *rounds, int *slots) {
+  int nb[2];
+  for (int j = 0; j < 2; ++j) nb[j] = (int)ceil_div(sh[j].M, 32);
+  int best_n = 0, best_slots = 0;
+  int64_t best_rounds = 0, best_T[2] = {0, 0};
+  for (int n = kFcMaxRowBlocks; n >= kFcMinRowBlocks; --n) {
+    int64_t lds = 0;
+    for (int j = 0; j < 2; ++j) {
+      const int64_t l = fc_conv_lds_bytes(n, sh[j].Wv, sh[j].Wp, k, mode);
+      if (l > lds) lds = l;
+    }
+    if (lds > kFcConvLdsLimit) continue;
+    const int sl = (2 * lds <= kFcConvLdsPerCU ? 2 : 1) * kNumCU;
+    const int lo = n > 2 ? n - 2 : 1;
+    int64_t T[2], wgs = 0;
+    bool ok = true;
+    for (int j = 0; j < 2; ++j) {
+      T[j] = ceil_div(nb[j], n);
+      if (T[j] > nb[j] / lo) ok = false;
+      wgs += B * sh[j].ntiles_n * T[j];
+    }
+    if (!ok) continue;
+    const int64_t r = ceil_div(wgs, sl);
+    const int64_t cost = r * (n + 1), best = best_rounds * (best_n + 1);
+    if (best_n && (cost > best || (cost == best && r >= best_rounds))) continue;
+    best_n = n, best_slots = sl, best_rounds = r, best_T[0] = T[0], best_T[1] = T[1];
+  }
+  if (!best_n) return 0;
+  const int lo = best_n > 2 ? best_n - 2 : 1;
+  int64_t *T = best_T, wgs = B * (sh[0].ntiles_n * T[0] + sh[1].ntiles_n * T[1]);
+  for (;;) {
+    int pick = -1;
+    for (int j = 0; j < 2; ++j) {
+      if (T[j] + 1 > nb[j] / lo || wgs + B * sh[j].ntiles_n > best_rounds * best_slots) continue;
+      if (pick < 0 || ceil_div(nb[j], T[j]) > ceil_div(nb[pick], T[pick]) ||
+          (ceil_div(nb[j], T[j]) == ceil_div(nb[pick], T[pick]) && nb[j] % T[j] > nb[pick] % T[pick]))
+        pick = j;
+    }
+    if (pick < 0) break;
+    wgs += B * sh[pick].ntiles_n;
+    ++T[pick];
+  }
+  int nmb = 0;
+  for (int j = 0; j < 2; ++j) {
+    fc_conv_set_tiling(&tl[j], nb[j], T[j], B);
+    const int h = tl[j].base + (tl[j].rem ? 1 : 0);
+    if (h > nmb) nmb = h;
+  }
+  if (rounds) *rounds = (int)best_rounds;
+  if (slots) *slots = best_slots;
+  return nmb < kFcMinRowBlocks ? kFcMinRowBlocks : nmb;
+}
+
+}
diff --git a/global_flow_local_attention_amd/csrc/fc_gemm.h b/global_flow_local_attention_amd/csrc/fc_gemm.h
--- a/global_flow_local_attention_amd/csrc/fc_gemm.h
+++ b/global_flow_local_attention_amd/csrc/fc_gemm.h
@@ -136,6 +136,17 @@
 int fc_conv_f32src(const PackedDesc &X32, const void *wk, int64_t w_split_stride, float *out, int64_t out_bs, int ldo,
                    int n_valid, int64_t B, int nch, int M, int Wv, int Wp, int k, const uint32_t *amax_x,
                    const uint32_t *amax_w, hipStream_t stream);
+struct ConvJobArgs {
+  PackedDesc X;
+  const void *wk;
+  int64_t w_split_stride;
+  float *out;
+  int64_t out_bs;
+  int ldo, n_valid, M, Wv, Wp;
+  const uint32_t *amax_x;
+};
+int fc_conv_f32src_jobs(const ConvJobArgs *jobs, int njobs, int64_t B, int nch, int k, const uint32_t *amax_w,
+                        hipStream_t stream);
 bool fc_conv_fits(int Wv, int Wp, int k, int mode);
 int fc_wgrad(const PackedDesc &X, const PackedDesc &Y, int64_t y_lead, float *dwacc, int cpad, int64_t B, int Mk,
              int Wp, int k, int mode, hipStream_t stream);
@@ -186,20 +197,6 @@
 int fc_wino_wgrad_reduce(float *part, int nsplit, float *grad_w0, int C, int c_off, int cpad, int k, hipStream_t stream);
 int fc_wino_wgrad_reduce2(float *part_s, int nsplit_s, float *part_t, int nsplit_t, float *grad_w0, int C, int cpad, int k,
                           hipStream_t stream);
-
-struct Wn16ConvJob {
-  PackedDesc X;
-  const uint32_t *U;
-  const uint32_t *amax_x;
-  float *out;
-  int64_t out_bs;
-  int ldo, n_valid, M, Wv, Wp;
-  int64_t S;
-};
-int fc_wino16_pack_weights(const float *w0, const uint32_t *amax_w, float *u_ft, float *u_fs, int C, int k, hipStream_t stream);
-bool fc_wino16_fits(int M, int Wv, int Wp, int k);
-int fc_wino16_conv_jobs(const Wn16ConvJob *jobs, int njobs, int64_t B, int nch, int k, const uint32_t *amax_w,
-                        hipStream_t stream);
 
 int fc_sample_tail_fwd(const float *gs, const float *gt, const float *flow, const float *b0, const float *w1,
                        const float *b1, float *hid, float *logits, int64_t B, int H, int W, int k, int64_t gs_bs,
diff --git a/global_flow_local_attention_amd/csrc/fc_wino16.hip b/global_flow_local_attention_amd/csrc/fc_wino16.hip
--- a/global_flow_local_attention_amd/csrc/fc_wino16.hip
+++ /dev/null
@@ -1,472 +0,0 @@
-#include "fc_wino_shared.h"
-
-namespace gfla {
-
-__global__ __launch_bounds__(256) void fc_wino16_pack_w_kernel(const float *__restrict__ w0, WnPackJobs jobs, int C,
-                                                               const uint32_t *__restrict__ amax_w) {
-  constexpr int KS = 3;
-  const WnPackJob jb = jobs.j[blockIdx.y];
-  const int nch = (jb.n_in + kFcChunk - 1) / kFcChunk, ntn = (jb.n_out + kWnN - 1) / kWnN;
-  const int64_t idx = (int64_t)blockIdx.x * 256 + threadIdx.x;
-  if (!jb.U || idx >= (int64_t)ntn * kWnN * nch * kFcChunk) return;
-  const float su = wn16_pow2(wn16_scale_exp(*amax_w, kWn16HeadW));
-  const int co = (int)(idx % (ntn * kWnN)), ci = (int)(idx / (ntn * kWnN));
-  float w[KS][KS];
-#pragma unroll
-  for (int i = 0; i < KS; ++i)
-#pragma unroll
-    for (int j = 0; j < KS; ++j) {
-      float v = 0.f;
-      if (ci < jb.n_in && co < jb.n_out) v = w0[(((int64_t)co * 2 * C + jb.c_off + ci) * KS + i) * KS + j];
-      w[i][j] = v * su;
-    }
-  float t[6][KS];
-#pragma unroll
-  for (int j = 0; j < KS; ++j) {
-    float col[KS], o[6];
-#pragma unroll
-    for (int i = 0; i < KS; ++i) col[i] = w[i][j];
-    wn_g<KS>(col, o);
-#pragma unroll
-    for (int a = 0; a < 6; ++a) t[a][j] = o[a];
-  }
-  const int ntile = co / kWnN, n = co % kWnN;
-  const int step = ci >> 3, g = (ci >> 2) & 1, c4 = ci & 3;
-  uint32_t *dst = reinterpret_cast<uint32_t *>(jb.U) + ((((int64_t)ntile * 2 * nch + step) * kWnXi * 2 + g) * kWnN + n) * 4 + c4;
-#pragma unroll
-  for (int a = 0; a < 6; ++a) {
-    float o[6];
-    wn_g<KS>(t[a], o);
-#pragma unroll
-    for (int e = 0; e < 6; ++e) dst[(int64_t)(a * 6 + e) * 2 * kWnN * 4] = wn16_split(o[e]);
-  }
-}
-
-int fc_wino16_pack_weights(const float *w0, const uint32_t *amax_w, float *u_ft, float *u_fs, int C, int k, hipStream_t stream) {
-  if (k != 3) return GFLA_ERR_UNSUPPORTED;
-  WnPackJobs jobs;
-  jobs.j[0] = WnPackJob{u_ft, 0, 0, C, kFcHidden};
-  jobs.j[1] = WnPackJob{u_fs, C, 0, C, kFcHidden};
-  const dim3 grid((unsigned)ceil_div(ceil_div(kFcHidden, kWnN) * kWnN * ceil_div(C, kFcChunk) * kFcChunk, 256), 2);
-  fc_wino16_pack_w_kernel<<<grid, 256, 0, stream>>>(w0, jobs, C, amax_w);
-  return launch_status();
-}
-
-struct Wn16KArgs {
-  PackedDesc X;
-  const uint32_t *U;
-  const uint32_t *amax_x;
-  float *out;
-  int64_t out_bs;
-  int ldo, n_valid, Ho, Wv, Wp;
-  WnGeo geo;
-  int ntn;
-  int64_t total_groups, S;
-};
-
-template <int M>
-struct WnAT;
-template <>
-struct WnAT<2> {
-  static constexpr float v[2][6] = {{1.f, 1.f, 1.f, 1.f, 1.f, 0.f}, {0.f, 1.f, -1.f, 2.f, -0.5f, 1.f}};
-};
-template <>
-struct WnAT<4> {
-  static constexpr float v[4][6] = {{1.f, 1.f, 1.f, 1.f, 1.f, 0.f},
-                                    {0.f, 1.f, -1.f, 2.f, -0.5f, 0.f},
-                                    {0.f, 1.f, 1.f, 4.f, 0.25f, 0.f},
-                                    {0.f, 1.f, -1.f, 8.f, -0.125f, 1.f}};
-};
-
-template <int PG_>
-struct PgTag { static constexpr int value = PG_; };
-
-extern unsigned long long *g_wino_stamps;
-template <int KS, bool DB = true, int DBG = 0>
-__global__ __launch_bounds__(kWnThreads, 2) void fc_wino16_conv_kernel(Wn16KArgs a0, Wn16KArgs a1, unsigned n0, int nch,
-                                                                      const uint32_t *__restrict__ amax_w,
-                                                                      unsigned long long *stamps) {
-  unsigned long long tk0 = 0, t_first = 0, t_second = 0, t_bar = 0, t_pro = 0, t_epi = 0;
-  if constexpr (DBG & 16) tk0 = __builtin_amdgcn_s_memtime();
-  auto stamp = [&](unsigned long long &slot) {
-    if constexpr (DBG & 16) {
-      __builtin_amdgcn_s_waitcnt(0);
-      const unsigned long long n = __builtin_amdgcn_s_memtime();
-      slot += n - tk0;
-      tk0 = n;
-    }
-  };
-  constexpr int M = Wn<KS>::M, PITCH = Wn<KS>::PITCH, NP = 9;
-  const bool second = blockIdx.x >= n0;
-#define GFLA_PICK(f) (second ? a1.f : a0.f)
-  PackedDesc X;
-  X.base = GFLA_PICK(X.base), X.split_stride = 0, X.batch_stride = GFLA_PICK(X.batch_stride);
-  X.chunk_stride = GFLA_PICK(X.chunk_stride), X.pix_stride = GFLA_PICK(X.pix_stride);
-  const uint32_t *__restrict__ U = GFLA_PICK(U);
-  const uint32_t *__restrict__ amax_x = GFLA_PICK(amax_x);
-  float *__restrict__ out = GFLA_PICK(out);
-  const int64_t out_bs = GFLA_PICK(out_bs), total_groups = GFLA_PICK(total_groups), S = GFLA_PICK(S);
-  const int ldo = GFLA_PICK(ldo), n_valid = GFLA_PICK(n_valid), Ho = GFLA_PICK(Ho), Wv = GFLA_PICK(Wv), Wp = GFLA_PICK(Wp);
-  const int ntn = GFLA_PICK(ntn);
-  WnGeo geo;
-  geo.TH = GFLA_PICK(geo.TH), geo.TW = GFLA_PICK(geo.TW), geo.ngroups = GFLA_PICK(geo.ngroups), geo.span = GFLA_PICK(geo.span);
-  geo.tpg = GFLA_PICK(geo.tpg);
-#undef GFLA_PICK
-  extern __shared__ __attribute__((aligned(16))) unsigned char gfla_smem[];
-  uint32_t *vbuf = reinterpret_cast<uint32_t *>(gfla_smem);
-  unsigned char *raw = gfla_smem + 2 * kWnVFloats * 4;
-  const int raw_bytes = (geo.span * PITCH + 15) & ~15;
-  const int t = threadIdx.x, lane = t & 63, wave = t >> 6, nblk = wave & 1, pg = (wave >> 1) & 3, xh = wave >> 2;
-  const int g = lane >> 5, l31 = lane & 31;
-  const int ex = wn16_scale_exp(*amax_x, kWn16HeadX), ew = wn16_scale_exp(*amax_w, kWn16HeadW);
-  const float sx = wn16_pow2(ex), inv_x = wn16_pow2(254 - ex), inv_w = wn16_pow2(254 - ew);
-  const int64_t x = blockIdx.x - (second ? n0 : 0u);
-  const int xcd = (int)(x & 7);
-  const int64_t slot = x >> 3;
-  const int ntile = (int)(slot % ntn);
-  const int64_t glin = (slot / ntn) * 8 + xcd;
-  if (glin >= total_groups) return;
-  const int64_t b = glin / geo.ngroups;
-  const int grp = (int)(glin - b * geo.ngroups);
-  const int ntiles = geo.TH * geo.TW;
-  const int tile0 = grp * geo.tpg;
-  const int ty_first = tile0 / geo.TW;
-  const int p0 = M * ty_first * Wp;
-  const int64_t avail = S - p0;
-
-  const int tl = (t & 255) >> 3, c8 = t & 7;
-  int toff;
-  {
-    const int tau = min(tile0 + min(tl, geo.tpg - 1), ntiles - 1);
-    const int ty = tau / geo.TW, tx = tau - ty * geo.TW;
-    toff = ((M * ty * Wp + M * tx) - p0) * PITCH + c8 * 4;
-  }
-  const int vpos = xh * 18 * 256 + (c8 >> 2) * 128 + tl * 4 + (c8 & 3);
-
-  const unsigned char *xg = X.base + b * X.batch_stride + (int64_t)p0 * X.pix_stride;
-
-  f32x16 acc[NP];
-#pragma unroll
-  for (int p = 0; p < NP; ++p)
-#pragma unroll
-    for (int i = 0; i < 16; ++i) acc[p][i] = 0.f;
-
-  const int npieces = geo.span * 4;
-  u32x4w pf[kWnPF];
-  auto piece_off = [&](int q) -> unsigned {
-    const int pix = q >> 2;
-    return (unsigned)min((int64_t)pix, avail - 1) * (unsigned)X.pix_stride + (unsigned)(q & 3) * 16u;
-  };
-  auto piece_store = [&](int q, u32x4w v, int cc) {
-    const int pix = q >> 2;
-    float f[4];
-#pragma unroll
-    for (int e = 0; e < 4; ++e) f[e] = pix >= avail ? 0.f : __uint_as_float(v[e]) * sx;
-    float2 *d = reinterpret_cast<float2 *>(raw + (DB ? (cc & 1) * raw_bytes : 0) + pix * PITCH + (q & 3) * 16);
-    d[0] = make_float2(f[0], f[1]);
-    d[1] = make_float2(f[2], f[3]);
-  };
-  auto prefetch = [&](int cc) {
-    const unsigned char *base = xg + (int64_t)cc * X.chunk_stride;
-#pragma unroll
-    for (int i = 0; i < kWnPF; ++i) pf[i] = *reinterpret_cast<const u32x4w *>(base + piece_off(min(t + kWnThreads * i, npieces - 1)));
-  };
-  auto commit = [&](int cc) {
-#pragma unroll
-    for (int i = 0; i < kWnPF; ++i) {
-      piece_store(min(t + kWnThreads * i, npieces - 1), pf[i], cc);
-    }
-    const unsigned char *base = xg + (int64_t)cc * X.chunk_stride;
-    for (int q = t + kWnThreads * kWnPF; q < npieces; q += kWnThreads)
-      piece_store(q, *reinterpret_cast<const u32x4w *>(base + piece_off(q)), cc);
-  };
-
-  const int nsteps = 2 * nch;
-  const unsigned ub_wave = __builtin_amdgcn_readfirstlane((unsigned)((((unsigned)ntile * nsteps) * kWnXi + NP * pg) * 2 * kWnN + nblk * 32));
-  const u32x4w *ub = reinterpret_cast<const u32x4w *>(U) + ub_wave + g * kWnN + l31;
-  u32x4w bf[NP];
-  auto load_b = [&](int step, int p) { return ub[((unsigned)step * kWnXi + p) * 2 * kWnN]; };
-
-  auto transform = [&](auto half_tag, int step) {
-    constexpr int HALF = decltype(half_tag)::value;
-    const unsigned char *src = raw + (DB ? ((step >> 1) & 1) * raw_bytes : 0) + toff + (step & 1) * 32;
-    uint32_t *dst = vbuf + (step & 1) * kWnVFloats + vpos;
-    __builtin_amdgcn_s_setprio(3);
-    float tm[3][6];
-#pragma unroll
-    for (int jp = 0; jp < 3; ++jp) {
-      f32x2v d[6], o[3];
-#pragma unroll
-      for (int i = 0; i < 6; ++i)
-        d[i] = f32x2v{*reinterpret_cast<const float *>(src + (i * Wp + 2 * jp) * PITCH),
-                      *reinterpret_cast<const float *>(src + (i * Wp + 2 * jp + 1) * PITCH)};
-      wn_bt3<HALF, f32x2v>(d, o);
-#pragma unroll
-      for (int r = 0; r < 3; ++r) tm[r][2 * jp] = o[r][0], tm[r][2 * jp + 1] = o[r][1];
-    }
-#pragma unroll
-    for (int r = 0; r < 3; ++r) {
-      float o[6];
-      wn_bt_pk(tm[r], o);
-#pragma unroll
-      for (int e = 0; e < 6; ++e) dst[(r * 6 + e) * 256] = (DBG & 32) ? (uint32_t)__float_as_uint(o[e]) : wn16_split(o[e]);
-    }
-    __builtin_amdgcn_s_setprio(0);
-  };
-
-  auto multiply = [&](int s, int sn) {
-    const u32x4w *va = reinterpret_cast<const u32x4w *>(vbuf + (s & 1) * kWnVFloats + (NP * pg) * 256 + g * 128 + l31 * 4);
-    u32x4w ra[2][2];
-    auto read_pair = [&](int p, int sl) {
-      ra[sl][0] = va[p * 64];
-      if (p + 1 < NP) ra[sl][1] = va[(p + 1) * 64];
-    };
-    auto swapped = [](u32x4w w) {
-      u32x4w r;
-#pragma unroll
-      for (int e = 0; e < 4; ++e) r[e] = __builtin_amdgcn_alignbit(w[e], w[e], 16);
-      return r;
-    };
-    read_pair(0, 0);
-#pragma unroll
-    for (int p = 0; p < NP; p += 2) {
-      const int sl = (p >> 1) & 1;
-      if (p + 2 < NP) read_pair(p + 2, sl ^ 1);
-      __builtin_amdgcn_sched_barrier(0);
-      const f16x8 a0v = __builtin_bit_cast(f16x8, ra[sl][0]);
-      const f16x8 b0v = __builtin_bit_cast(f16x8, bf[p]), b0s = __builtin_bit_cast(f16x8, swapped(bf[p]));
-      if (p + 1 < NP) {
-        const f16x8 a1v = __builtin_bit_cast(f16x8, ra[sl][1]);
-        const f16x8 b1v = __builtin_bit_cast(f16x8, bf[p + 1]), b1s = __builtin_bit_cast(f16x8, swapped(bf[p + 1]));
-        acc[p] = __builtin_amdgcn_mfma_f32_32x32x16_f16(a0v, b0v, acc[p], 0, 0, 0);
-        acc[p + 1] = __builtin_amdgcn_mfma_f32_32x32x16_f16(a1v, b1v, acc[p + 1], 0, 0, 0);
-        acc[p] = __builtin_amdgcn_mfma_f32_32x32x16_f16(a0v, b0s, acc[p], 0, 0, 0);
-        acc[p + 1] = __builtin_amdgcn_mfma_f32_32x32x16_f16(a1v, b1s, acc[p + 1], 0, 0, 0);
-        if constexpr (!(DBG & 4)) {
-          bf[p] = load_b(sn, p);
-          bf[p + 1] = load_b(sn, p + 1);
-        }
-      } else {
-        acc[p] = __builtin_amdgcn_mfma_f32_32x32x16_f16(a0v, b0v, acc[p], 0, 0, 0);
-        acc[p] = __builtin_amdgcn_mfma_f32_32x32x16_f16(a0v, b0s, acc[p], 0, 0, 0);
-        if constexpr (!(DBG & 4)) bf[p] = load_b(sn, p);
-      }
-      __builtin_amdgcn_sched_barrier(0);
-    }
-  };
-
-  prefetch(0);
-  commit(0);
-#pragma unroll
-  for (int p = 0; p < NP; ++p) bf[p] = load_b(0, p);
-  __syncthreads();
-  if (xh == 0) transform(Half0{}, 0);
-  else transform(Half1{}, 0);
-  __syncthreads();
-
-  stamp(t_pro);
-  for (int s = 0; s < nsteps; ++s) {
-    const int cc = s >> 1;
-    const int sn = min(s + 1, nsteps - 1);
-    const bool stage_next = !(s & 1) && cc + 1 < nch;
-    constexpr bool kT = !(DBG & 1), kM = !(DBG & 2), kS = !(DBG & 8);
-    if (xh == 0) {
-      if constexpr (kM) multiply(s, sn);
-      __builtin_amdgcn_sched_barrier(0);
-      stamp(t_first);
-      if (kS && stage_next) {
-        prefetch(cc + 1);
-        if constexpr (kT) transform(Half0{}, s + 1);
-        if constexpr (DB) commit(cc + 1);
-      } else {
-        if constexpr (kT) transform(Half0{}, s + 1);
-      }
-      stamp(t_second);
-    } else {
-      if (kS && stage_next) {
-        prefetch(cc + 1);
-        if constexpr (kT) transform(Half1{}, s + 1);
-        if constexpr (DB) commit(cc + 1);
-      } else {
-        if constexpr (kT) transform(Half1{}, s + 1);
-      }
-      __builtin_amdgcn_sched_barrier(0);
-      stamp(t_first);
-      if constexpr (kM) multiply(s, sn);
-      stamp(t_second);
-    }
-    __syncthreads();
-    stamp(t_bar);
-    if constexpr (!DB) {
-      if (stage_next) {
-        commit(cc + 1);
-        __syncthreads();
-      }
-    }
-  }
-
-  float4 *xch = reinterpret_cast<float4 *>(gfla_smem);
-  constexpr int MM4 = M * M / 4;
-  const int col = ntile * kWnN + nblk * 32 + l31;
-  float *ob = out + b * out_bs + col;
-  auto partial = [&](auto pg_tag, int i, float (&part)[M * M]) {
-    constexpr int PG = decltype(pg_tag)::value;
-#pragma unroll
-    for (int e = 0; e < M * M; ++e) part[e] = 0.f;
-#pragma unroll
-    for (int a = 0; a < 6; ++a) {
-      constexpr int first = NP * PG, last = NP * PG + NP - 1;
-      const int e0 = a * 6 > first ? 0 : first - a * 6, e1 = a * 6 + 5 < last ? 5 : last - a * 6;
-      if (a * 6 + 5 < first || a * 6 > last) continue;
-      float tj[M];
-#pragma unroll
-      for (int j = 0; j < M; ++j) {
-        float sacc = 0.f;
-#pragma unroll
-        for (int e = 0; e < 6; ++e)
-          if (e >= e0 && e <= e1 && WnAT<M>::v[j][e] != 0.f) sacc = fmaf(WnAT<M>::v[j][e], acc[a * 6 + e - first][i], sacc);
-        tj[j] = sacc;
-      }
-#pragma unroll
-      for (int ii = 0; ii < M; ++ii)
-        if (WnAT<M>::v[ii][a] != 0.f) {
-#pragma unroll
-          for (int j = 0; j < M; ++j) part[ii * M + j] = fmaf(WnAT<M>::v[ii][a], tj[j], part[ii * M + j]);
-        }
-    }
-  };
-  constexpr int QPR = M == 2 ? 4 : 1;
-  auto finish = [&](auto pg_tag) {
-    constexpr int PG = decltype(pg_tag)::value;
-#pragma unroll
-    for (int q0 = 0; q0 < 4; q0 += QPR) {
-      float part[QPR][4][M * M];
-#pragma unroll
-      for (int qq = 0; qq < QPR; ++qq)
-#pragma unroll
-        for (int r = 0; r < 4; ++r) partial(pg_tag, 4 * (q0 + qq) + r, part[qq][r]);
-      if constexpr (!(DBG & 256)) __syncthreads();
-#pragma unroll
-      for (int qq = 0; qq < QPR; ++qq) {
-        const int qd = q0 + qq;
-        if (PG != qd && !(DBG & 256)) {
-          const int w3 = (PG - qd - 1) & 3;
-          float4 *dst = xch + (((qq * 3 + w3) * 2 + nblk) * 4 * MM4) * 64 + lane;
-#pragma unroll
-          for (int r = 0; r < 4; ++r)
-#pragma unroll
-            for (int c4 = 0; c4 < MM4; ++c4)
-              dst[(r * MM4 + c4) * 64] = make_float4(part[qq][r][4 * c4], part[qq][r][4 * c4 + 1], part[qq][r][4 * c4 + 2],
-                                                     part[qq][r][4 * c4 + 3]);
-        }
-      }
-      if constexpr (!(DBG & 256)) __syncthreads();
-#pragma unroll
-      for (int qq = 0; qq < QPR; ++qq) {
-        const int qd = q0 + qq;
-        if (PG != qd) continue;
-#pragma unroll
-        for (int w3 = 0; w3 < ((DBG & 256) ? 0 : 3); ++w3) {
-          const float4 *srcp = xch + (((qq * 3 + w3) * 2 + nblk) * 4 * MM4) * 64 + lane;
-#pragma unroll
-          for (int r = 0; r < 4; ++r)
-#pragma unroll
-            for (int c4 = 0; c4 < MM4; ++c4) {
-              const float4 v = srcp[(r * MM4 + c4) * 64];
-              part[qq][r][4 * c4] += v.x, part[qq][r][4 * c4 + 1] += v.y, part[qq][r][4 * c4 + 2] += v.z, part[qq][r][4 * c4 + 3] += v.w;
-            }
-        }
-#pragma unroll
-        for (int r = 0; r < 4; ++r) {
-          const int slot_ = 8 * qd + 4 * g + r, tau = tile0 + slot_;
-          if (slot_ >= geo.tpg || tau >= ntiles || col >= n_valid) continue;
-          const int ty = tau / geo.TW, tx = tau - ty * geo.TW;
-#pragma unroll
-          for (int i = 0; i < M; ++i) {
-            const int yo = M * ty + i;
-            if (yo >= Ho) continue;
-#pragma unroll
-            for (int j = 0; j < M; ++j) {
-              const int xo = M * tx + j;
-              if (xo < Wv && (!(DBG & 128) || part[qq][r][i * M + j] == 1.2345f))
-                ob[(int64_t)(yo * Wv + xo) * ldo] = (part[qq][r][i * M + j] * inv_x) * inv_w;
-            }
-          }
-        }
-      }
-    }
-  };
-  if constexpr (DBG & 64) {
-    float keep = 0.f;
-#pragma unroll
-    for (int p = 0; p < NP; ++p)
-#pragma unroll
-      for (int i = 0; i < 16; ++i) keep += acc[p][i];
-    if (keep == 1.2345f) ob[0] = keep * inv_x * inv_w;
-    return;
-  }
-  if (pg == 0) finish(PgTag<0>{});
-  else if (pg == 1) finish(PgTag<1>{});
-  else if (pg == 2) finish(PgTag<2>{});
-  else finish(PgTag<3>{});
-  if constexpr (DBG & 16) {
-    stamp(t_epi);
-    if (stamps && lane == 0) {
-      unsigned long long *o = stamps + ((int64_t)blockIdx.x * 8 + wave) * 6;
-      o[0] = t_pro, o[1] = t_first, o[2] = t_second, o[3] = t_bar, o[4] = t_epi, o[5] = (unsigned long long)xh;
-    }
-  }
-}
-
-static unsigned wn16_lds_bytes(int k, const WnGeo &g, bool double_raw) {
-  const int m = k == 5 ? 2 : 4;
-  const unsigned raw = k == 5 ? wn_raw_bytes<5>(g) : wn_raw_bytes<3>(g);
-  const unsigned main_loop = (unsigned)(2 * kWnVFloats * 4) + (double_raw ? 2u : 1u) * raw;
-  const unsigned exchange = (unsigned)(3 * 2 * 4 * m * m * 64 * 4) * (m == 2 ? 4u : 1u);
-  return main_loop > exchange ? main_loop : exchange;
-}
-
-static int wn16_launch(const Wn16ConvJob *jobs, int njobs, int64_t B, int nch, const uint32_t *amax_w, hipStream_t stream) {
-  Wn16KArgs a[2];
-  int64_t wgs[2] = {0, 0};
-  bool db = tuning(21) != 1;
-  unsigned lds = 0;
-  for (int j = 0; j < njobs; ++j) db = db && wn16_lds_bytes(3, wn_geometry<3>(jobs[j].M, jobs[j].Wv, jobs[j].Wp), true) <= kWnLdsLimit;
-  for (int j = 0; j < 2; ++j) {
-    const Wn16ConvJob &J = jobs[j < njobs ? j : 0];
-    const WnGeo g = wn_geometry<3>(J.M, J.Wv, J.Wp);
-    const int ntn = (int)ceil_div(J.n_valid, kWnN);
-    const int64_t groups = B * g.ngroups;
-    a[j] = Wn16KArgs{J.X, J.U, J.amax_x, J.out, J.out_bs, J.ldo, J.n_valid, J.M / J.Wv, J.Wv, J.Wp, g, ntn, groups, J.S};
-    if (j < njobs) {
-      wgs[j] = ceil_div(groups, 8) * 8 * ntn;
-      lds = std::max(lds, wn16_lds_bytes(3, g, db));
-    }
-  }
-  if (wgs[0] + wgs[1] > 0x7fffffffLL || lds > kWnLdsLimit) return GFLA_ERR_UNSUPPORTED;
-  auto kern = db ? fc_wino16_conv_kernel<3, true> : fc_wino16_conv_kernel<3, false>;
-  (void)hipFuncSetAttribute(reinterpret_cast<const void *>(kern), hipFuncAttributeMaxDynamicSharedMemorySize, (int)lds);
-  kern<<<dim3((unsigned)(wgs[0] + wgs[1])), kWnThreads, lds, stream>>>(a[0], a[1], (unsigned)wgs[0], nch, amax_w,
-                                                                         db ? g_wino_stamps : nullptr);
-  return launch_status();
-}
-
-bool fc_wino16_fits(int M, int Wv, int Wp, int k) {
-  if (!fc_wino_fits(M, Wv, Wp, k)) return false;
-  const WnGeo g = k == 5 ? wn_geometry<5>(M, Wv, Wp) : wn_geometry<3>(M, Wv, Wp);
-  return wn16_lds_bytes(k, g, false) <= kWnLdsLimit;
-}
-
-int fc_wino16_conv_jobs(const Wn16ConvJob *jobs, int njobs, int64_t B, int nch, int k, const uint32_t *amax_w, hipStream_t stream) {
-  if (B <= 0 || njobs <= 0) return GFLA_OK;
-  if (njobs > 2 || !amax_w || k != 3) return GFLA_ERR_UNSUPPORTED;
-  for (int j = 0; j < njobs; ++j)
-    if (!jobs[j].amax_x || !fc_wino16_fits(jobs[j].M, jobs[j].Wv, jobs[j].Wp, k)) return GFLA_ERR_UNSUPPORTED;
-  if (njobs == 2 && tuning(21) == 2) {
-    const int st = fc_wino16_conv_jobs(jobs, 1, B, nch, k, amax_w, stream);
-    return st != GFLA_OK ? st : fc_wino16_conv_jobs(jobs + 1, 1, B, nch, k, amax_w, stream);
-  }
-  return wn16_launch(jobs, njobs, B, nch, amax_w, stream);
-}
-
-}
diff --git a/global_flow_local_attention_amd/fc_mfma.py b/global_flow_local_attention_amd/fc_mfma.py
--- a/global_flow_local_attention_amd/fc_mfma.py
+++ b/global_flow_local_attention_amd/fc_mfma.py
@@ -10,8 +10,8 @@
 MODE_NAMES = {0: "f32 MFMA, direct convolution", 1: "one f16 term per operand (exact for bf16 values), f32 accumulate",
               2: "two f16 terms per operand, f32 accumulate", 3: "three f16 terms per operand, f32 accumulate",
               4: "f32 MFMA, Winograd-domain convolutions F(2x2,5x5) / F(4x4,3x3)",
-              5: "two f16 terms per operand on f16 MFMA, f32 accumulate: direct kernels (k5 convolutions, data gradients) + "
-                 "Winograd domain F(2x2,5x5) / F(4x4,3x3) (k3 forward, k5 weight gradient)"}
+              5: "two f16 terms per operand on f16 MFMA, f32 accumulate: direct kernels (forward and data-gradient "
+                 "convolutions; k3: both halves per launch) + Winograd domain F(2x2,5x5) / F(4x4,3x3) (weight gradients: k5 f16, k3 f32)"}
 
 
 def supported(C, H, W, k, mode=DEFAULT_MODE):
diff --git a/include/gfla_hip.h b/include/gfla_hip.h
--- a/include/gfla_hip.h
+++ b/include/gfla_hip.h
@@ -255,6 +255,10 @@
                         const float *b0, const float *w1, const float *b1, void *workspace, float *logits,
                         int64_t B, int64_t C, int64_t H, int64_t W, int kernel_size, double slope, gfla_stream_t stream);
 int gfla_fc_geometry(int64_t H, int64_t W, int kernel_size, int is_source, int64_t *out);
+
+int gfla_fc_conv_tiling(int64_t B, int64_t C, int64_t H, int64_t W, int kernel_size, int dgrad, int64_t *out);
+
+int gfla_fc_map_offsets(int64_t B, int64_t C, int64_t H, int64_t W, int kernel_size, int mode, int64_t *out);
 int gfla_fc_conv_fwd_f32(const float *x, const float *w0, int is_source, void *workspace, float *out, int64_t B,
                          int64_t C, int64_t H, int64_t W, int kernel_size, int mode, gfla_stream_t stream);
 int gfla_fc_conv_bwd_f32(const float *z, int is_source, void *workspace, void *scratch, float *grad_x,
```

New measurement: 9837 (median of 6 runs). 1.02x the previous value.
